# SurrealAI/surreal

Hardware: AMD Instinct MI355X
Metric: env-steps/sec (learner ingest) PPO 1024 actors×128 steps, 1/2/4/8 MI355X (higher is better)
Workload: dtype f32; 1 GPU; BASELINE configs[4]: PPO synthetic 1024 actors x 128 steps x 376-dim obs per GPU, one learn() per step, batch resident in HBM; mode=adapt, B_per_gpu=1024, n_step=128, obs_dim=376, action_dim=17, epochs=10 policy + 10 value, KL early exit disabled, hip_graph=True, parallelism=dp1, epoch_kernels=fused row-block, graph_segments=False

## Files before the change

include/surreal_amd.h:

```cpp
#ifndef SURREAL_AMD_H
#define SURREAL_AMD_H

#include <stddef.h>
#include <stdint.h>

#ifdef __cplusplus
extern "C" {
#endif

typedef void* smx_stream_t;

enum {
    SMX_OK = 0,
    SMX_E_NULL = -1,
    SMX_E_SHAPE = -2,
    SMX_E_UNSUPPORTED = -3,
    SMX_E_WORKSPACE = -4,
    SMX_E_ALIGN = -5
};

enum { SMX_ACT_NONE = 0, SMX_ACT_RELU = 1, SMX_ACT_TANH = 2 };
enum { SMX_PPO_CLIP = 0, SMX_PPO_ADAPT = 1 };

int smx_abi_version(void);
// ... 139 lines not shown
int smx_ppo_learn_epilogue_f32(const smx_learn_epilogue_t* args, smx_stream_t stream);
int smx_moments_f32(const float* x, int64_t n, float* moments, smx_stream_t stream);
int smx_moments_merge_f32(const float* parts, int32_t k, float* out, smx_stream_t stream);
int smx_adv_normalize_f32(float* x, int64_t n, const float* moments, float min_std,
                          smx_stream_t stream);

typedef struct {
    float lr_actor, lr_critic;
    float beta, eta;
    float clip_eps;
    float kl_target;
    float actor_max_norm, critic_max_norm;
    float actor_weight_decay, critic_weight_decay;
    int32_t adam_step_actor, adam_step_critic;
    int32_t stop_flag;
    int32_t epochs_done;
    int32_t reserved[2];
} smx_ppo_ctrl_t;

enum {
    SMX_PS_SURR = 0,
    SMX_PS_LOSS = 1,
    SMX_PS_ENTROPY = 2,
    SMX_PS_KL = 3,
    SMX_PS_GRADNORM = 4,
    SMX_PS_LB = 5,
    SMX_PS_ISW = 6,
    SMX_PS_REFBEH = 7,
    SMX_PS_STRIDE = 8
};
enum { SMX_VS_LOSS = 0, SMX_VS_EXPVAR = 1, SMX_VS_GRADNORM = 2, SMX_VS_STRIDE = 4 };

int32_t smx_ppo_loss_blocks(int64_t rows);
int32_t smx_ppo_loss_partial_stride(int32_t A);
int smx_ppo_policy_loss_f32(int32_t mode, const float* mean, const float* log_var,
                            const float* actions, int32_t ld_act, const float* behave,
                            int32_t ld_beh, const float* ref, int32_t ld_ref,
                            const float* adv, int64_t rows, int32_t A,
                            const smx_ppo_ctrl_t* ctrl, float* g_surr, float* g_kl,
                            float* row_partials, smx_stream_t stream);
int smx_ppo_partials_fold_f32(const float* row_partials, int32_t nblk, int32_t stride, float* out, int32_t nout,
                              const smx_ppo_ctrl_t* ctrl, smx_stream_t stream);
int smx_ppo_loss_finalize_f32(int32_t mode, const float* row_partials, int32_t nblk,
                              const float* g_surr, const float* g_kl, const float* log_var,
                              int64_t rows, int64_t n_total, int32_t A, smx_ppo_ctrl_t* ctrl,
                              int32_t check_stop, int32_t will_update, float* dz3,
                              float* dz3_t, int64_t ld_t, float* dlogvar, float* dlogvar_sumsq,
                              float* stats, smx_stream_t stream);

int32_t smx_value_loss_blocks(int64_t rows);
int smx_value_loss_f32(const float* values, const float* returns, int64_t rows,
                       int64_t n_total, float* dz3, float* partials, smx_ppo_ctrl_t* ctrl,
                       int32_t will_update, smx_stream_t stream);
typedef struct smx_ppo_losses {
    int32_t mode, A;
    const float* mean;
    const float* log_var;
    const float* actions;
    const float* behave;
    const float* ref;
    const float* adv;
    int32_t ld_act, ld_beh, ld_ref, check_stop;
    int64_t rows;
    float* g_surr;
    float* g_kl;
    float* row_partials;
    float* dz3;
    float* dz3_t;
    int64_t ld_t;
    float* dlogvar;
    float* dlogvar_sumsq;
    float* stats;
    const float* values;
    const float* returns;
    float* v_dz3;
    float* v_partials;
    int32_t will_update, v_will_update;
} smx_ppo_losses_t;
int smx_ppo_epoch_losses_f32(const smx_ppo_losses_t* args, smx_ppo_ctrl_t* ctrl,
                             smx_stream_t stream);
int smx_ppo_epoch_losses_dp_f32(const smx_ppo_losses_t* args, int64_t n_total, float* g_surr_t,
                                float* g_kl_t, smx_ppo_ctrl_t* ctrl, smx_stream_t stream);
typedef struct smx_ppo_combine {
    int32_t mode, A;
    const float* row_partials;
    int32_t nblk;
    int32_t check_stop;
    int64_t n_total;
    const float* log_var;
    float* stats;
    float* grads_a;
    const float* grads_kl;
    int64_t n_mlp, n_a;
    float* sumsq_a;
    const float* grads_c;
    int64_t n_c;
    float* sumsq_c;
    int32_t will_update, reserved;
} smx_ppo_combine_t;
int smx_ppo_epoch_combine_f32(const smx_ppo_combine_t* args, smx_ppo_ctrl_t* ctrl,
                              smx_stream_t stream);
int smx_mlp3_wgrad_multi_f32(const smx_mlp3_job_t* jobs, int32_t njobs, smx_stream_t stream);

enum { SMX_EPOCH_LOSS_NONE = 0, SMX_EPOCH_LOSS_POLICY = 1, SMX_EPOCH_LOSS_VALUE = 2, SMX_EPOCH_RHS_SURR = 3,
       SMX_EPOCH_RHS_KL = 4 };
typedef struct smx_epoch_job {
    const smx_mlp3_t* net;
    const float* x;
    int64_t rows;
    float* h1T;
    float* h2T;
    int64_t ldT;
    float* out;
    int32_t out_ld;
    int32_t out_act;
    int32_t loss;
    int32_t reserved;
    const int32_t* stop_flag;
    const float* dz3;
    float* dz3T;
    float* dz2T;
    float* dz1T;
    const float* packed;
} smx_epoch_job_t;
typedef struct smx_epoch_pack {
    const smx_mlp3_t* net;
    float* packed;
} smx_epoch_pack_t;
int64_t smx_epoch_packed_floats(int32_t D, int32_t H1, int32_t H2, int32_t OUT);
int smx_epoch_pack_f32(const smx_epoch_pack_t* items, int32_t n, smx_stream_t stream);
typedef struct smx_epoch_prep {
    const float* obs0; int64_t ld_obs0; int64_t rows; int32_t D; int32_t A;
    const float* zmean; const float* zstd;
    float* xn; float* xnT; int64_t ldT;
    const float* ref_sum; const float* ref_sumsq; const float* ref_count; float ref_eps; int32_t ref_filter;
    float* xr;
    const float* obs_next; int64_t ld_next; float* xnext;
    const float* ref_log_var; float* ref_std; int64_t ld_ref;
    int32_t* zero_words; int32_t n_zero; int32_t n_pack;
    smx_epoch_pack_t pack[4];
} smx_epoch_prep_t;
int smx_epoch_prepare_f32(const smx_epoch_prep_t* args, smx_stream_t stream);
struct smx_ppo_losses;
int32_t smx_epoch_blocks(int64_t rows);
int32_t smx_epoch_supported(int32_t D, int32_t H1, int32_t H2, int32_t OUT);
int smx_epoch_forward_f32(const smx_epoch_job_t* jobs, int32_t njobs, const struct smx_ppo_losses* loss,
                          smx_ppo_ctrl_t* ctrl, int64_t n_total, smx_stream_t stream);
int smx_epoch_backward_f32(const smx_epoch_job_t* jobs, int32_t njobs, const struct smx_ppo_losses* loss,
                           smx_ppo_ctrl_t* ctrl, int64_t n_total, smx_stream_t stream);
int32_t smx_epoch_fwdbwd_supported(int32_t D, int32_t H1, int32_t H2, int32_t OUT);
int smx_epoch_fwdbwd_f32(const smx_epoch_job_t* jobs, int32_t njobs, const struct smx_ppo_losses* loss,
                         smx_ppo_ctrl_t* ctrl, int64_t n_total, int32_t* sync_word, uint64_t* kl_slots,
                         smx_stream_t stream);
int smx_device_occupy(int32_t blocks, int64_t microseconds, smx_stream_t stream);

int smx_diaggauss_sample_f32(const float* mean, int64_t ld_mean, const float* log_var,
                             const float* noise_scale, const float* eps, int64_t ld_eps,
                             int64_t rows, int32_t A, float* actions, int64_t ld_act, float* pd,
                             int64_t ld_pd, smx_stream_t stream);
int smx_ppo_final_stats_f32(const float* log_var, int32_t A, const float* running_sum,
                            const float* running_sumsq, const float* count, int32_t D, float* out4,
                            smx_stream_t stream);
int smx_value_loss_finalize_f32(const float* partials, int32_t count, int32_t nblk,
                                float* stats, int32_t stats_stride, smx_stream_t stream);

int smx_clip_adam_step_f32(float* theta, const float* grads, float* exp_avg,
                           float* exp_avg_sq, int64_t n, const float* sumsq_partials,
                           int32_t npart, const smx_ppo_ctrl_t* ctrl, int32_t which,
                           int32_t honour_stop, float* grad_norm_out, smx_stream_t stream);
typedef struct smx_adam_group {
    float* theta;
    const float* grads;
    float* exp_avg;
    float* exp_avg_sq;
    int64_t n;
    const float* sumsq_partials;
    int32_t npart;
    int32_t honour_stop;
    float* grad_norm_out;
    const smx_mlp3_t* pack_net;
    float* packed;
} smx_adam_group_t;
int smx_clip_adam_step_group_f32(const smx_adam_group_t* group, int32_t which, const smx_ppo_ctrl_t* ctrl,
                                 smx_stream_t stream);
int smx_clip_adam_step_pair_f32(const smx_adam_group_t* actor, const smx_adam_group_t* critic,
                                const smx_ppo_ctrl_t* ctrl, smx_stream_t stream);
int32_t smx_sumsq_blocks(int64_t n);
int smx_sumsq_partials_f32(const float* x, int64_t n, float* partials, smx_stream_t stream);

int smx_ring_insert_f32(float* table, int64_t capacity, int32_t width, int64_t cursor,
                        const float* src, int64_t n, smx_stream_t stream);
int smx_gather_rows_f32(const float* table, int64_t capacity, int32_t width,
                        const int64_t* idx, int64_t n, float* dst, smx_stream_t stream);
int smx_uniform_indices(int64_t* idx, int64_t n, int64_t len, uint64_t seed,
                        uint64_t offset, smx_stream_t stream);
int smx_philox4x32_10(const uint32_t* ctr_key, int64_t n, uint32_t* out, smx_stream_t stream);
typedef struct {
    const void* table;
    void* dst;
    int64_t row_bytes;
} smx_gather_job_t;
int smx_uniform_gather_multi(const smx_gather_job_t* jobs, int32_t njobs, int64_t capacity, int64_t rows,
                             const int64_t* idx, int64_t len, uint64_t seed, uint64_t offset, int64_t* idx_out,
                             smx_stream_t stream);

int smx_ring_insert_bytes(void* table, int64_t capacity, int64_t row_bytes, int64_t cursor,
                          const void* src, int64_t n, smx_stream_t stream);
int smx_gather_rows_bytes(const void* table, int64_t capacity, int64_t row_bytes, const int64_t* idx,
                          int64_t n, void* dst, smx_stream_t stream);

int smx_window_emit_f32(const float* src, int32_t actors, int32_t T, int32_t width,
                        int32_t start, int32_t n_step, int32_t stride, int32_t W, float* dst,
                        smx_stream_t stream);
int smx_window_emit_bytes(const void* src, int32_t actors, int32_t T, int64_t row_bytes, int32_t start,
                          int32_t n_step, int32_t stride, int32_t W, void* dst, smx_stream_t stream);

int smx_frame_stack_u8(const void* frames, int32_t actors, int32_t R, int64_t frame_bytes, int32_t n_stack,
                       const int32_t* episode_first, int32_t start, int32_t n_step, int32_t stride, int32_t W,
                       void* dst, smx_stream_t stream);
int smx_synth_frame_u8(const float* s0, int64_t ld_s0, int32_t n, int32_t C, int32_t H, int32_t W, int32_t t,
                       void* dst, int64_t ld_dst, smx_stream_t stream);


struct smx_episode_monitor {
    double* ep_reward;
    int32_t* ep_steps;
    int64_t* ep_count;
    double* done_reward;
    int32_t* done_steps;
    int32_t capacity, reserved;
};

struct smx_noise_stream {
    uint64_t seed;
    int64_t actor_base;
    int64_t step;
    int32_t enabled, reserved;
};
int smx_noise_fill_f32(const struct smx_noise_stream* noise, int32_t steps, int32_t n, int32_t A, float* out,
                       smx_stream_t stream);

int smx_synth_env_step_f32(float* state, const float* init_state, const float* actions,
                           int32_t n, int32_t D, int32_t A, int32_t t, int32_t episode_len,
                           int32_t slot, int32_t T, float* obs_roll, float* act_roll,
                           float* rew_roll, float* done_roll, const struct smx_episode_monitor* mon,
                           smx_stream_t stream);

typedef struct smx_synth_act_step {
    float* state;
    const float* init_state;
    const float* mean;
    const float* log_var;
    const float* noise_scale;
    const float* eps;
    int64_t ld_mean, ld_eps;
    int32_t n, D, A, t, episode_len, slot, T, reserved;
    float* obs_roll;
    float* act_roll;
    float* rew_roll;
    float* done_roll;
    float* pd_roll;
    const float* zsum;
    const float* zsumsq;
    const float* zcount;
    float zeps, reserved_f;
    float* xn_out;
    struct smx_noise_stream noise;
    struct smx_episode_monitor mon;
} smx_synth_act_step_t;
int smx_synth_act_env_step_f32(const smx_synth_act_step_t* args, smx_stream_t stream);
int smx_synth_act_env_step_head_f32(const smx_synth_act_step_t* args, const float* W3, const float* b3,
                                    const float* h2, int64_t ld_h2, int32_t H2, int32_t out_act,
                                    smx_stream_t stream);


int smx_ddpg_critic_loss_f32(const float* q, const float* q_next_target, const float* rewards,
                             const float* dones, float gamma_n, int64_t rows, float* y,
                             float* dz3, smx_stream_t stream);
int smx_tanh_backward_f32(const float* da, const float* a, int64_t n, float* out,
                          smx_stream_t stream);
int smx_fill_f32(float* x, int64_t n, float value, smx_stream_t stream);
int smx_layernorm_forward_f32(const float* x, int64_t ldx, int64_t rows, int32_t F, const float* gamma, const float* beta,
                              float eps, float* y, int64_t ldy, float* mean, float* rstd, smx_stream_t stream);
int64_t smx_layernorm_backward_ws_floats(int64_t rows, int32_t F);
int smx_layernorm_backward_f32(const float* dy, int64_t lddy, const float* x, int64_t ldx, const float* mean,
                               const float* rstd, const float* gamma, int64_t rows, int32_t F, int32_t relu_mask, float* dx,
                               int64_t lddx, float* dgamma, float* dbeta, float* ws, int64_t ws_floats, smx_stream_t stream);
int smx_adam_step_f32(float* theta, const float* grads, float* exp_avg, float* exp_avg_sq,
                      int64_t n, double lr, int32_t step, double weight_decay,
                      double clip_value, smx_stream_t stream);
int smx_ddpg_critic_loss_step_f32(const float* q, const float* q_next_target, const float* rewards,
                                  const float* dones, float gamma_n, int64_t rows, float* y,
                                  float* dz3, int32_t* step_counter, smx_stream_t stream);
int smx_adam_step_dev_f32(float* theta, const float* grads, float* exp_avg, float* exp_avg_sq,
                          int64_t n, const float* lr, const int32_t* step, double weight_decay,
                          double clip_value, smx_stream_t stream);
int smx_hard_update_every_f32(float* target, const float* source, int64_t n, const int32_t* step,
                              int32_t interval, smx_stream_t stream);
int smx_soft_update_f32(float* target, const float* source, float tau, int64_t n,
                        smx_stream_t stream);
int smx_ddpg_stats_f32(const float* q, const float* y, const float* rewards,
                       const float* actions, int32_t ld_act, int32_t A, const float* q_actor,
                       int64_t rows, float* stats, smx_stream_t stream);

typedef struct smx_ddpg_net {
    const float *W1, *b1, *W2, *b2, *W3, *b3;
// ... 323 lines not shown
```

surreal_amd/_lib.py:

```python
import ctypes
import os
from ctypes import (POINTER, Structure, c_char_p, c_double, c_float, c_int32, c_int64, c_size_t,
                    c_uint64, c_void_p)

_HERE = os.path.dirname(os.path.abspath(__file__))
LIB_PATH = os.environ.get('SMX_LIB_PATH') or os.path.join(_HERE, 'libsurreal_amd.so')

SMX_ACT_NONE, SMX_ACT_RELU, SMX_ACT_TANH = 0, 1, 2
SMX_PPO_CLIP, SMX_PPO_ADAPT = 0, 1
SMX_E_UNSUPPORTED = -3
PS_SURR, PS_LOSS, PS_ENTROPY, PS_KL, PS_GRADNORM, PS_LB, PS_ISW, PS_REFBEH, PS_STRIDE = range(9)
VS_LOSS, VS_EXPVAR, VS_GRADNORM = 0, 1, 2
VS_STRIDE = 4


class Mlp3(Structure):
    _fields_ = [('W1', c_void_p), ('b1', c_void_p), ('W2', c_void_p), ('b2', c_void_p),
                ('W3', c_void_p), ('b3', c_void_p),
                ('D', c_int32), ('H1', c_int32), ('H2', c_int32), ('OUT', c_int32)]


class Mlp3Job(Structure):
    _fields_ = [('net', POINTER(Mlp3)), ('x', c_void_p), ('rows', c_int64), ('h1', c_void_p),
                ('h2', c_void_p), ('out', c_void_p), ('out_act', c_int32), ('out_ld', c_int32),
# ... 104 lines not shown
                [(n, c_void_p) for n in ('c_a1', 'cm1', 'cr1', 'c_a2', 'cm2', 'cr2', 'dn2', 'dz1c', 'a1', 'am1', 'ar1', 'a2',
                                         'am2', 'ar2', 'dn2a', 'dn1a')] + [('second', POINTER(DdpgRowsLnSecond))])


class DdpgRows(Structure):
    _fields_ = ([('rows', c_int64)] + [(n, c_int32) for n in ('D', 'A', 'H1', 'H2', 'c1', 'c2')] +
                [(n, DdpgNet) for n in ('actor', 'critic', 'target_actor', 'target_critic')] +
                [(n, c_void_p) for n in ('packed', 'x', 'x_next', 'actions', 'rewards', 'dones')] +
                [('gamma_n', c_float)] +
                [(n, c_void_p) for n in ('xcat', 'h2c', 'q', 'q_next', 'y', 'dz3', 'dz2', 'dxcat', 'h1a', 'h2a', 'act',
                                         'q_actor', 'dz3a', 'dz2a', 'dz1a', 'step')] +
                [('second', POINTER(DdpgRowsSecond)), ('ln', POINTER(DdpgRowsLn))])


class GatherJob(Structure):
    _fields_ = [('table', c_void_p), ('dst', c_void_p), ('row_bytes', c_int64)]


class EpisodeMonitor(Structure):
    _fields_ = [('ep_reward', c_void_p), ('ep_steps', c_void_p), ('ep_count', c_void_p), ('done_reward', c_void_p),
                ('done_steps', c_void_p), ('capacity', c_int32), ('reserved', c_int32)]


class NoiseStream(Structure):
    _fields_ = [('seed', c_uint64), ('actor_base', c_int64), ('step', c_int64), ('enabled', c_int32),
                ('reserved', c_int32)]


class SynthRollout(Structure):
    _fields_ = [('net', POINTER(Mlp3)), ('packed', c_void_p), ('out_act', c_int32), ('n', c_int32),
                ('log_var', c_void_p), ('noise_scale', c_void_p), ('eps', c_void_p), ('zsum', c_void_p),
                ('zsumsq', c_void_p), ('zcount', c_void_p), ('zeps', c_float), ('t', c_int32),
                ('episode_len', c_int32), ('steps', c_int32), ('rows_per_actor', c_int32), ('slot', c_int32),
                ('state', c_void_p), ('init_state', c_void_p), ('obs_roll', c_void_p), ('act_roll', c_void_p),
                ('rew_roll', c_void_p), ('done_roll', c_void_p), ('pd_roll', c_void_p), ('obs_last', c_void_p),
                ('actors_per_workgroup', c_int32), ('noise', NoiseStream), ('mon', EpisodeMonitor)]


class SynthLstmRollout(Structure):
    _fields_ = [('roll', SynthRollout), ('lstm', POINTER(Lstm)), ('lstm_packed', c_void_p), ('hidden', c_int32),
                ('reserved', c_int32), ('h0', c_void_p), ('c0', c_void_p), ('hN', c_void_p), ('cN', c_void_p),
                ('h_before', c_void_p), ('c_before', c_void_p), ('cell_roll', c_void_p)]


class SynthPpoWindowRollout(Structure):
    _fields_ = [('base', SynthLstmRollout), ('n_step', c_int32), ('advance', c_int32), ('carry_obs', c_void_p),
                ('carry_act', c_void_p), ('carry_rew', c_void_p), ('carry_pd', c_void_p), ('carry_cells', c_void_p),
                ('obs', c_void_p), ('obs_next', c_void_p), ('actions', c_void_p), ('rewards', c_void_p),
                ('dones', c_void_p), ('pds', c_void_p), ('cells', c_void_p), ('cursor', c_int64),
                ('capacity', c_int64)]


class DdpgRollout(Structure):
    _fields_ = [('net', POINTER(Mlp3)), ('packed', c_void_p), ('n', c_int32), ('D', c_int32), ('A', c_int32),
                ('steps', c_int32), ('t', c_int32), ('episode_len', c_int32), ('n_step', c_int32),
                ('noise_type', c_int32), ('actors_per_workgroup', c_int32), ('reserved', c_int32),
                ('eps', c_void_p), ('sigmas', c_void_p), ('theta', c_double), ('dt', c_double), ('root_dt', c_double),
                ('gpow', c_void_p), ('ou', c_void_p), ('state', c_void_p), ('init_state', c_void_p),
                ('carry_obs', c_void_p), ('carry_act', c_void_p), ('carry_rew', c_void_p), ('obs', c_void_p),
                ('obs_next', c_void_p), ('actions', c_void_p), ('rewards', c_void_p), ('dones', c_void_p),
                ('cursor', c_int64), ('capacity', c_int64), ('noise', NoiseStream), ('mon', EpisodeMonitor)]


class DdpgActorVariant(Structure):
    _fields_ = [('ln', c_void_p), ('ln_eps', c_float), ('reserved', c_int32), ('packed_pop', c_void_p),
                ('packed_stride', c_int64), ('actors_per_agent', c_int32), ('agents', c_int32),
                ('measure_step', c_int32), ('reserved2', c_int32), ('dist', c_void_p)]


class ParamNoise(Structure):
    _fields_ = [('net', POINTER(Mlp3)), ('seed', c_uint64), ('agent_base', c_int64), ('generation', c_int64),
                ('agents', c_int32), ('adaptive', c_int32), ('acts', c_int64), ('alpha', c_double), ('target', c_double),
                ('sigma', c_void_p), ('dist', c_void_p), ('packed_pop', c_void_p), ('packed_stride', c_int64),
                ('ln', c_void_p)]


class DdpgPixelStep(Structure):
    _fields_ = [('base', DdpgRollout), ('C', c_int32), ('H', c_int32), ('W', c_int32), ('frame_stacks', c_int32),
                ('hist_len', c_int32), ('hist_pos', c_int32), ('hist', c_void_p), ('pixel', c_void_p),
                ('pixel_next', c_void_p), ('obs_pixel', c_void_p)]


class SynthPpoPixelWindowStep(Structure):
    _fields_ = ([(n, c_int32) for n in ('n', 'D', 'A', 'hidden', 't', 'episode_len', 'n_step', 'advance')] +
                [(n, c_void_p) for n in ('log_var', 'noise_scale', 'eps', 'state', 'init_state', 'h_before', 'c_before',
                                         'carry_obs', 'carry_act', 'carry_rew', 'carry_pd', 'carry_cells', 'obs',
                                         'obs_next', 'actions', 'rewards', 'dones', 'pds', 'cells')] +
                [('cursor', c_int64), ('capacity', c_int64)] +
                [(n, c_int32) for n in ('C', 'H', 'W', 'frame_stacks', 'hist_len', 'hist_pos', 'copy_workgroups',
                                        'reserved')] +
                [(n, c_void_p) for n in ('hist', 'pixel', 'pixel_next', 'obs_pixel')] + [('noise', NoiseStream),
                                                                                   ('mon', EpisodeMonitor)])


SMX_DDPG_NOISE_NONE, SMX_DDPG_NOISE_GAUSSIAN, SMX_DDPG_NOISE_OU = 0, 1, 2
SMX_PPO_PIXEL_STEP_MAX_A = 64


class Xchg(Structure):
    _fields_ = [('world', c_int32), ('rank', c_int32), ('capacity', c_int64), ('peer', c_void_p * 8)]


class SynthActStep(Structure):
    _fields_ = [('state', c_void_p), ('init_state', c_void_p), ('mean', c_void_p), ('log_var', c_void_p),
                ('noise_scale', c_void_p), ('eps', c_void_p), ('ld_mean', c_int64), ('ld_eps', c_int64),
                ('n', c_int32), ('D', c_int32), ('A', c_int32), ('t', c_int32), ('episode_len', c_int32),
                ('slot', c_int32), ('T', c_int32), ('reserved', c_int32),
                ('obs_roll', c_void_p), ('act_roll', c_void_p), ('rew_roll', c_void_p),
                ('done_roll', c_void_p), ('pd_roll', c_void_p), ('zsum', c_void_p), ('zsumsq', c_void_p),
                ('zcount', c_void_p), ('zeps', c_float), ('reserved_f', c_float), ('xn_out', c_void_p),
                ('noise', NoiseStream), ('mon', EpisodeMonitor)]


CTRL_WORDS = 16
(C_LR_ACTOR, C_LR_CRITIC, C_BETA, C_ETA, C_CLIP_EPS, C_KL_TARGET, C_ACTOR_MAX_NORM,
 C_CRITIC_MAX_NORM, C_ACTOR_WD, C_CRITIC_WD, C_STEP_ACTOR, C_STEP_CRITIC, C_STOP,
 C_EPOCHS_DONE) = range(14)
C_XCHG_ERR = 14
C_SYNC_ERR = 15

_P = c_void_p
_SIGS = {
    'smx_abi_version': (c_int32, []),
    'smx_error_string': (c_char_p, [c_int32]),
    'smx_zfilter_stats_f32': (c_int32, [_P, _P, _P, c_int32, c_float, _P, _P, _P]),
    'smx_zfilter_forward_f32': (c_int32, [_P, c_int64, c_int64, c_int32, _P, _P, _P, _P]),
    'smx_zfilter_forward_sums_f32': (c_int32, [_P, c_int64, c_int64, c_int32, _P, _P, _P, c_float, _P, _P]),
    'smx_diaggauss_sample_f32': (c_int32, [_P, c_int64, _P, _P, _P, c_int64, c_int64, c_int32, _P,
                                           c_int64, _P, c_int64, _P]),
    'smx_zfilter_update_f32': (c_int32, [_P, c_int64, c_int64, c_int32, _P, _P, _P, c_float, _P]),
    'smx_mlp3_packed_bytes': (c_size_t, [c_int32, c_int32, c_int32, c_int32]),
    'smx_mlp3_pack_f32': (c_int32, [POINTER(Mlp3), _P, c_size_t, _P]),
    'smx_mlp3_pack_zstats_f32': (c_int32, [POINTER(Mlp3), _P, c_size_t, _P, _P, _P, c_int32, c_float, _P, _P, _P]),
    'smx_mlp3_fused_exact_zfilter': (c_int32, [c_int32]),
    'smx_mlp3_forward_fused_f32': (c_int32, [_P, c_int32, c_int32, c_int32, c_int32, _P, _P,
                                             c_int64, c_int32, c_int32, _P, _P, _P, c_int32, _P]),
    'smx_linear_f32': (c_int32, [_P, c_int32, c_int32, _P, c_int32, c_int32, _P, _P, c_int32,
                                 c_int32, c_int32, c_int32, c_int32, _P, _P, _P]),
    'smx_linear_wgrad_f32': (c_int32, [_P, c_int32, _P, c_int32, _P, c_int32, _P, c_int32, c_int32,
                                       c_int32, _P]),
    'smx_mlp3_forward_f32': (c_int32, [POINTER(Mlp3), _P, c_int64, _P, _P, _P, c_int32, _P, _P]),
    'smx_mlp3_forward_multi_f32': (c_int32, [POINTER(Mlp3Job), c_int32, _P]),
    'smx_mlp3_backward_multi_f32': (c_int32, [POINTER(Mlp3Job), c_int32, _P]),
    'smx_mlp3_wgrad_multi_f32': (c_int32, [POINTER(Mlp3Job), c_int32, _P]),
    'smx_epoch_blocks': (c_int32, [c_int64]),
    'smx_epoch_supported': (c_int32, [c_int32, c_int32, c_int32, c_int32]),
    'smx_epoch_packed_floats': (c_int64, [c_int32, c_int32, c_int32, c_int32]),
    'smx_epoch_pack_f32': (c_int32, [POINTER(EpochPack), c_int32, _P]),
    'smx_epoch_prepare_f32': (c_int32, [POINTER(EpochPrep), _P]),
    'smx_epoch_forward_f32': (c_int32, [POINTER(EpochJob), c_int32, POINTER(PpoLosses), _P, c_int64, _P]),
    'smx_epoch_backward_f32': (c_int32, [POINTER(EpochJob), c_int32, POINTER(PpoLosses), _P, c_int64, _P]),
    'smx_epoch_fwdbwd_supported': (c_int32, [c_int32, c_int32, c_int32, c_int32]),
    'smx_epoch_fwdbwd_f32': (c_int32, [POINTER(EpochJob), c_int32, POINTER(PpoLosses), _P, c_int64, _P, _P, _P]),
    'smx_device_occupy': (c_int32, [c_int32, c_int64, _P]),
    'smx_layernorm_forward_f32': (c_int32, [_P, c_int64, c_int64, c_int32, _P, _P, c_float, _P, c_int64, _P, _P, _P]),
    'smx_layernorm_backward_ws_floats': (c_int64, [c_int64, c_int32]),
    'smx_layernorm_backward_f32': (c_int32, [_P, c_int64, _P, c_int64, _P, _P, _P, c_int64, c_int32, c_int32, _P, c_int64, _P, _P,
                                             _P, c_int64, _P]),
    'smx_zfilter_update_ws_floats': (c_int64, [c_int64, c_int32]),
    'smx_zfilter_update_ws_f32': (c_int32, [_P, c_int64, c_int64, c_int32, _P, _P, _P, c_float, _P, c_int64, _P]),
    'smx_ppo_partials_fold_f32': (c_int32, [_P, c_int32, c_int32, _P, c_int32, _P, _P]),
    'smx_mlp3_forward_rows_supported': (c_int32, [c_int32, c_int32, c_int32, c_int32]),
    'smx_mlp3_forward_rows_f32': (c_int32, [POINTER(Mlp3), _P, c_int64, _P, _P, _P, c_int32, c_int32, _P, c_size_t, _P, _P]),
    'smx_mlp3_backward_partials': (c_int32, [c_int32, c_int32, c_int32, c_int32]),
    'smx_mlp3_backward_f32': (c_int32, [POINTER(Mlp3), _P, _P, _P, _P, c_int64, _P, _P, _P, _P,
                                        _P, _P]),
    'smx_mlp3_backward_ws_floats': (c_int64, [c_int32, c_int32, c_int32, c_int32, c_int64]),
    'smx_mlp3_backward_splitk_f32': (c_int32, [POINTER(Mlp3), _P, _P, _P, _P, c_int64, _P, _P, _P, _P, c_int64, _P, _P]),
    'smx_mlp3_dgrad_rows_supported': (c_int32, [c_int32, c_int32, c_int32, c_int32]),
    'smx_mlp3_dgrad_rows_ws_floats': (c_int64, [c_int32, c_int32, c_int32, c_int32]),
    'smx_mlp3_backward_rows_f32': (c_int32, [POINTER(Mlp3), _P, _P, _P, _P, c_int64, _P, _P, _P, _P, _P, c_int64, _P, c_int64,
                                             _P, _P]),
    'smx_windowed_gae_returns_f32': (c_int32, [_P, _P, _P, _P, _P, _P, c_float, c_float, c_int32,
                                               c_int32, c_int32, _P, _P, _P]),
    'smx_windowed_gae_norm_f32': (c_int32, [_P, _P, _P, _P, _P, _P, c_float, c_float, c_int32, c_int32, c_int32, _P, _P, _P,
                                            c_float, _P, _P]),
    'smx_ppo_learn_epilogue_f32': (c_int32, [POINTER(LearnEpilogue), _P]),
    'smx_reward_filter_f32': (c_int32, [_P, c_int64, c_float, c_int32, _P, c_float, c_int32, _P, _P, _P, _P, _P]),
    'smx_reward_filter_partials': (c_int32, []),
    'smx_moments_f32': (c_int32, [_P, c_int64, _P, _P]),
    'smx_moments_merge_f32': (c_int32, [_P, c_int32, _P, _P]),
    'smx_adv_normalize_f32': (c_int32, [_P, c_int64, _P, c_float, _P]),
    'smx_ppo_loss_blocks': (c_int32, [c_int64]),
    'smx_ppo_loss_partial_stride': (c_int32, [c_int32]),
    'smx_ppo_policy_loss_f32': (c_int32, [c_int32, _P, _P, _P, c_int32, _P, c_int32, _P, c_int32,
                                          _P, c_int64, c_int32, _P, _P, _P, _P, _P]),
    'smx_ppo_loss_finalize_f32': (c_int32, [c_int32, _P, c_int32, _P, _P, _P, c_int64, c_int64,
                                            c_int32, _P, c_int32, c_int32, _P, _P, c_int64, _P, _P,
                                            _P, _P]),
    'smx_ppo_epoch_losses_f32': (c_int32, [POINTER(PpoLosses), _P, _P]),
    'smx_ppo_epoch_losses_dp_f32': (c_int32, [POINTER(PpoLosses), c_int64, _P, _P, _P, _P]),
    'smx_ppo_epoch_combine_f32': (c_int32, [POINTER(PpoCombine), _P, _P]),
    'smx_ppo_final_stats_f32': (c_int32, [_P, c_int32, _P, _P, _P, c_int32, _P, _P]),
    'smx_value_loss_blocks': (c_int32, [c_int64]),
    'smx_value_loss_f32': (c_int32, [_P, _P, c_int64, c_int64, _P, _P, _P, c_int32, _P]),
    'smx_value_loss_finalize_f32': (c_int32, [_P, c_int32, c_int32, _P, c_int32, _P]),
    'smx_clip_adam_step_f32': (c_int32, [_P, _P, _P, _P, c_int64, _P, c_int32, _P, c_int32,
                                         c_int32, _P, _P]),
    'smx_clip_adam_step_group_f32': (c_int32, [POINTER(AdamGroup), c_int32, _P, _P]),
    'smx_clip_adam_step_pair_f32': (c_int32, [POINTER(AdamGroup), POINTER(AdamGroup), _P, _P]),
    'smx_sumsq_blocks': (c_int32, [c_int64]),
    'smx_sumsq_partials_f32': (c_int32, [_P, c_int64, _P, _P]),
    'smx_synth_act_env_step_head_f32': (c_int32, [POINTER(SynthActStep), _P, _P, _P, c_int64, c_int32, c_int32, _P]),
    'smx_conv_u8_forward_f32': (c_int32, [_P, c_int64, c_int32, c_int32, c_int32, c_int32, c_int32, _P, _P, c_int32,
                                          _P, _P, _P]),
    'smx_conv_u8_wgrad_ws_floats': (c_int64, [c_int32, c_int32]),
    'smx_conv_u8_wgrad_f32': (c_int32, [_P, c_int64, c_int32, c_int32, c_int32, c_int32, c_int32, _P, c_int32, _P, _P, _P,
                                        c_int64, _P, _P]),
    'smx_conv_cl_forward_f32': (c_int32, [_P, c_int64, c_int32, c_int32, c_int32, c_int32, c_int32, _P, _P, c_int32,
                                          _P, _P, _P]),
    'smx_conv_cl_wgrad_ws_floats': (c_int64, [c_int32, c_int32]),
    'smx_conv_cl_wgrad_f32': (c_int32, [_P, c_int64, c_int32, c_int32, c_int32, c_int32, c_int32, _P, c_int32, _P, _P, _P,
                                        c_int64, _P, _P]),
    'smx_conv_cl_dgrad_f32': (c_int32, [_P, c_int64, c_int32, c_int32, c_int32, c_int32, c_int32, _P, c_int32, _P, _P,
                                        _P, _P]),
    'smx_ring_insert_bytes': (c_int32, [_P, c_int64, c_int64, c_int64, _P, c_int64, _P]),
    'smx_gather_rows_bytes': (c_int32, [_P, c_int64, c_int64, _P, c_int64, _P, _P]),
    'smx_window_emit_bytes': (c_int32, [_P, c_int32, c_int32, c_int64, c_int32, c_int32, c_int32, c_int32, _P, _P]),
    'smx_ring_insert_f32': (c_int32, [_P, c_int64, c_int32, c_int64, _P, c_int64, _P]),
    'smx_gather_rows_f32': (c_int32, [_P, c_int64, c_int32, _P, c_int64, _P, _P]),
    'smx_philox4x32_10': (c_int32, [_P, c_int64, _P, _P]),
    'smx_noise_fill_f32': (c_int32, [POINTER(NoiseStream), c_int32, c_int32, c_int32, _P, _P]),
    'smx_uniform_indices': (c_int32, [_P, c_int64, c_int64, c_uint64, c_uint64, _P]),
    'smx_uniform_gather_multi': (c_int32, [POINTER(GatherJob), c_int32, c_int64, c_int64, _P, c_int64, c_uint64, c_uint64,
                                           _P, _P]),
    'smx_window_emit_f32': (c_int32, [_P, c_int32, c_int32, c_int32, c_int32, c_int32, c_int32,
                                      c_int32, _P, _P]),
    'smx_synth_act_env_step_f32': (c_int32, [POINTER(SynthActStep), _P]),
    'smx_synth_env_step_f32': (c_int32, [_P, _P, _P, c_int32, c_int32, c_int32, c_int32, c_int32,
                                         c_int32, c_int32, _P, _P, _P, _P, POINTER(EpisodeMonitor), _P]),
    'smx_ddpg_critic_loss_f32': (c_int32, [_P, _P, _P, _P, c_float, c_int64, _P, _P, _P]),
    'smx_tanh_backward_f32': (c_int32, [_P, _P, c_int64, _P, _P]),
    'smx_fill_f32': (c_int32, [_P, c_int64, c_float, _P]),
    'smx_adam_step_f32': (c_int32, [_P, _P, _P, _P, c_int64, c_double, c_int32, c_double, c_double,
                                    _P]),
    'smx_soft_update_f32': (c_int32, [_P, _P, c_float, c_int64, _P]),
    'smx_ddpg_critic_loss_step_f32': (c_int32, [_P, _P, _P, _P, c_float, c_int64, _P, _P, _P, _P]),
    'smx_adam_step_dev_f32': (c_int32, [_P, _P, _P, _P, c_int64, _P, _P, c_double, c_double, _P]),
    'smx_hard_update_every_f32': (c_int32, [_P, _P, c_int64, _P, c_int32, _P]),
    'smx_ddpg_rows_supported': (c_int32, [c_int32] * 6),
    'smx_ddpg_rows_supported_at': (c_int32, [c_int32] * 6 + [c_int64]),
    'smx_ddpg_rows_packed_floats': (c_int64, [c_int32] * 6),
    'smx_ddpg_rows_pack_f32': (c_int32, [_P, c_int32, _P]),
    'smx_ddpg_rows_critic_f32': (c_int32, [_P, _P]),
    'smx_ddpg_rows_actor_f32': (c_int32, [_P, _P]),
    'smx_ddpg_rows_second_supported': (c_int32, [c_int32] * 6 + [c_int64]),
    'smx_ddpg_rows_second_packed_floats': (c_int64, [c_int32] * 6),
    'smx_ddpg_rows_critic_td3_f32': (c_int32, [_P, _P]),
    'smx_ddpg_rows_ln_supported': (c_int32, [c_int32] * 6 + [c_int64]),
    'smx_ddpg_rows_ln_second_supported': (c_int32, [c_int32] * 6 + [c_int64]),
    'smx_ddpg_rows_update_f32': (c_int32, [_P, c_int32, _P, _P]),
    'smx_ddpg_rows_wgrad_update_f32': (c_int32, [_P, c_int32, _P, _P]),
    'smx_ddpg_stats_f32': (c_int32, [_P, _P, _P, _P, c_int32, c_int32, _P, c_int64, _P, _P]),
    'smx_lstm_param_count': (c_int64, [c_int32, c_int32]),
    'smx_lstm_forward_f32': (c_int32, [POINTER(Lstm), _P, c_int64, c_int32, _P, _P, _P, _P, _P, _P,
                                       _P, _P, _P, _P]),
    'smx_lstm_backward_f32': (c_int32, [POINTER(Lstm), _P, c_int64, c_int32, _P, _P, _P, _P, _P, _P,
                                        _P, _P, _P, c_int64, _P]),
    'smx_lstm_backward_ws_floats': (c_int64, [c_int32, c_int32, c_int64, c_int32]),
    'smx_linear_wgrad_ws_floats': (c_int64, [c_int32, c_int32, c_int32]),
    'smx_linear_wgrad_splitk_f32': (c_int32, [_P, c_int32, _P, c_int32, _P, c_int32, _P, c_int32,
                                              c_int32, c_int32, _P, c_int64, _P]),
    'smx_linear_wgrad_splitk_pair_f32': (c_int32, [_P, c_int32, c_int32, c_int32, _P, c_int32, _P, _P, c_int32, _P,
                                                    c_int32, _P, _P, c_int32, _P, c_int64, _P]),
    'smx_im2col_f32': (c_int32, [_P, c_int32, c_int32, c_int64, c_int32, c_int32, c_int32, c_int32,
                                 c_int32, c_int32, c_float, _P, _P]),
    'smx_col2im_f32': (c_int32, [_P, c_int64, c_int32, c_int32, c_int32, c_int32, c_int32, c_int32,
                                 _P, _P, _P]),
    'smx_flatten_order_f32': (c_int32, [_P, c_int32, c_int32, c_int32, c_int32, _P, _P]),
    'smx_linear_multi_f32': (c_int32, [POINTER(LinearJob), c_int32, _P]),
    'smx_frame_stack_u8': (c_int32, [_P, c_int32, c_int32, c_int64, c_int32, _P, c_int32, c_int32, c_int32, c_int32, _P, _P]),
    'smx_synth_frame_u8': (c_int32, [_P, c_int64, c_int32, c_int32, c_int32, c_int32, c_int32, _P, c_int64, _P]),
    'smx_synth_rollout_supported': (c_int32, [c_int32, c_int32, c_int32, c_int32]),
    'smx_synth_rollout_f32': (c_int32, [POINTER(SynthRollout), _P]),
    'smx_synth_lstm_rollout_supported': (c_int32, [c_int32] * 5),
    'smx_lstm_rollout_packed_floats': (c_int64, [c_int32, c_int32]),
    'smx_lstm_rollout_pack_f32': (c_int32, [POINTER(Lstm), _P, _P]),
    'smx_synth_lstm_rollout_f32': (c_int32, [POINTER(SynthLstmRollout), _P]),
    'smx_synth_ppo_window_rollout_supported': (c_int32, [c_int32] * 5),
    'smx_synth_ppo_window_rollout_f32': (c_int32, [POINTER(SynthPpoWindowRollout), _P]),
    'smx_synth_ddpg_rollout_supported': (c_int32, [c_int32, c_int32, c_int32, c_int32, c_int32]),
    'smx_synth_ddpg_rollout_f32': (c_int32, [POINTER(DdpgRollout), POINTER(DdpgActorVariant), _P]),
    'smx_synth_ddpg_population_block': (c_int32, [c_int32, c_int32, c_int32]),
    'smx_synth_ddpg_step_f32': (c_int32, [POINTER(DdpgRollout), _P, c_int64, _P]),
    'smx_synth_ddpg_pixel_step': (c_int32, [POINTER(DdpgPixelStep), _P, c_int64, _P]),
    'smx_param_noise_copy_floats': (c_int64, [c_int32, c_int32, c_int32, c_int32, c_int32]),
    'smx_param_noise_fill_f32': (c_int32, [POINTER(ParamNoise), c_int32, _P, _P]),
    'smx_param_noise_refresh_f32': (c_int32, [POINTER(ParamNoise), _P]),
    'smx_synth_ppo_pixel_window_step': (c_int32, [POINTER(SynthPpoPixelWindowStep), _P, c_int64, _P]),
    'smx_xchg_bytes': (c_int64, [c_int64, c_int32]),
    'smx_xchg_alloc': (c_int32, [c_int64, c_double, POINTER(c_void_p), POINTER(c_int32), _P]),
    'smx_xchg_free': (c_int32, [_P]),
    'smx_xchg_export': (c_int32, [_P, _P]),
    'smx_xchg_open': (c_int32, [_P, POINTER(c_void_p)]),
    'smx_xchg_close': (c_int32, [_P]),
    'smx_xchg_allreduce_f32': (c_int32, [POINTER(Xchg), _P, _P, c_int64, _P, _P]),
    'smx_xchg_allgather_f32': (c_int32, [POINTER(Xchg), _P, c_int64, _P, _P, _P]),
    'smx_xchg_status': (c_int32, [POINTER(Xchg), _P, _P]),
}

EXPORTED_SYMBOLS = tuple(sorted(_SIGS))


class SmxError(RuntimeError):
    pass

# ... 58 lines not shown
```

surreal_amd/csrc/smx_epoch.hip:

```cpp
#include "smx_common.h"
#include <string.h>

#define SMX_LDS_BARRIER() asm volatile("s_waitcnt lgkmcnt(0)\n\ts_barrier" ::: "memory")

namespace {
#include "smx_ppo_loss.inc.h"
#include "smx_epoch_pack.inc.h"
#include "smx_epoch_mma.inc.h"

constexpr int TB = 3;
constexpr int MAX_EJOBS = 4;
constexpr int XV = 7;
constexpr int LIN = 6;
constexpr int LINF = 3;
constexpr int EXCLUSIVE_LDS = 84 * 1024;
constexpr int LDZ = 68;
constexpr int LDO = 36;
static_assert(ER == LOSS_ROWS_PER_BLOCK, "a row block is a loss block");
static_assert(NTH == 256, "the shared loss code strides by 256 threads");

#ifdef SMX_EPOCH_TIMING
#define TSTAMP(i) do { if (G.tbuf && threadIdx.x == 0) G.tbuf[(size_t)ts_blk * 32 + (i)] = (long long)__builtin_readcyclecounter(); } while (0)
#else
#define TSTAMP(i) do { } while (0)
#endif
struct EJob {
    const float *W1, *b1, *W2, *b2, *W3, *b3;
    int D, H1, H2, OUT;
    const float* x;
    int rows;
    float *h1T, *h2T;
    long ldT;
    float* out;
    int out_ld, out_act, loss, blk_base;
    const int* stop;
    const float* dz3;
    float *dz3T, *dz2T, *dz1T;
    const float *P1, *P2, *P3, *P2T, *P3T;
};

struct PolArgs {
    int mode, A;
    const float *log_var, *actions, *behave, *ref, *adv;
    int ld_act, ld_beh, ld_ref, check_stop, will_update;
    float *g_surr, *g_kl, *row_partials;
    float *dlogvar, *dlogvar_sumsq, *stats;
};

struct ValArgs {
    const float* returns;
    float *v_dz3, *v_partials;
    int will_update;
};

struct EArgs {
    EJob j[MAX_EJOBS];
    int n;
    PolArgs pl;
    ValArgs vl;
    long n_total;
    int ldx, ldh1, ldh2, off_h1, off_h2, off_out, off_red, off_loss;
    int off_g;
    int* sync;
    int nb_pol;
    const int* pol_stop;
    unsigned long long* kl_slots;
    int fsplit;
    int xsplit;
    long long* tbuf;
};

__device__ __forceinline__ int xcd_job_order(const EArgs& G, int raw) {
    const int nb = G.xsplit;
    if (nb == 0) return raw;
    const int xcd = raw & 7, slot = raw >> 3;
    return (xcd >> 2) * nb + slot * 4 + (xcd & 3);
}

__device__ __forceinline__ EJob select_job(const EArgs& G, int bid) {
    int pi = 0;
#pragma unroll
    for (int k = 1; k < MAX_EJOBS; ++k) pi += (k < G.n && bid >= G.j[k].blk_base) ? 1 : 0;
    EJob J = G.j[pi];
    asm volatile("" :: "s"(J.W1), "s"(J.b1), "s"(J.W2), "s"(J.b2), "s"(J.W3), "s"(J.b3), "s"(J.D), "s"(J.H1),
                 "s"(J.H2), "s"(J.OUT), "s"(J.x), "s"(J.rows), "s"(J.h1T), "s"(J.h2T), "s"(J.ldT), "s"(J.out),
                 "s"(J.out_ld), "s"(J.out_act), "s"(J.loss), "s"(J.blk_base), "s"(J.stop), "s"(J.dz3),
                 "s"(J.dz3T), "s"(J.dz2T), "s"(J.dz1T));
    return J;
}

constexpr int FNWV = 8;
constexpr int FNTH = 64 * FNWV;
constexpr int FTG = 3;

__device__ __forceinline__ void fb_reduce_partials(const float* __restrict__ partials, int nblk, int stride, float* S,
                                                   float* buf) {
    const int tid = threadIdx.x;
    float t0 = 0.f, t1 = 0.f, t2 = 0.f, t3 = 0.f;
    for (int b0 = 0; b0 < nblk; b0 += FIN_CH) {
        const int nb = min(FIN_CH, nblk - b0);
        const int cnt = nb * stride;
        const float* src = partials + (size_t)b0 * stride;
        for (int i0 = tid; i0 < cnt; i0 += 8 * FNTH) {
            float v[8];
#pragma unroll
            for (int u = 0; u < 8; ++u)
                v[u] = __hip_atomic_load(src + min(i0 + FNTH * u, cnt - 1), __ATOMIC_RELAXED, __HIP_MEMORY_SCOPE_AGENT);
#pragma unroll
            for (int u = 0; u < 8; ++u)
                if (i0 + FNTH * u < cnt) buf[i0 + FNTH * u] = v[u];
        }
        SMX_LDS_BARRIER();
        if (tid < stride) {
            int b = 0;
            for (; b + 4 <= nb; b += 4) {
                t0 += buf[b * stride + tid];
                t1 += buf[(b + 1) * stride + tid];
                t2 += buf[(b + 2) * stride + tid];
                t3 += buf[(b + 3) * stride + tid];
            }
            for (; b < nb; ++b) t0 += buf[b * stride + tid];
        }
        SMX_LDS_BARRIER();
    }
    if (tid < stride) S[tid] = (t0 + t1) + (t2 + t3);
    SMX_LDS_BARRIER();
}

template <bool FB>
__device__ __forceinline__ void epoch_fwd_body(const EArgs& G, smx_ppo_ctrl_t* __restrict__ ctrl) {
    extern __shared__ float sm[];
    const int bid = xcd_job_order(G, (int)blockIdx.x);
    const int ts_blk = bid;
    (void)ts_blk;
    TSTAMP(0);
    const EJob J = select_job(G, bid);
    const int stopv = J.stop ? __builtin_nontemporal_load(J.stop) : 0;
    const int blk = bid - J.blk_base;
    const long row0 = (long)blk * ER;
    int nrows = J.rows - (int)row0;
    if (nrows > ER) nrows = ER;
    const int tid = threadIdx.x, lane = tid & 63;
    const int wv = __builtin_amdgcn_readfirstlane(tid >> 6);
    const int fm = lane & 15, kq = lane >> 4;
    TSTAMP(12);

    float* xs = sm;
    float* h1s = sm + G.off_h1;
    float* h2s = sm + G.off_h2;
    float* outs = sm + G.off_out;
    const int ldx = G.ldx, ldh1 = G.ldh1, ldh2 = G.ldh2;

    const rsrc_t rx = make_rsrc(J.x, (unsigned)J.rows * (unsigned)J.D * 4u);
    const bool lo = tid < NTH;
    const int xr = (tid & (NTH - 1)) >> 4, xj = tid & 15;
    const unsigned xrow = (unsigned)(row0 + xr) * (unsigned)J.D * 4u;
    const bool xvec = (J.D & 3) == 0;
    float4 xv[XV];
    if (xvec) {
#pragma unroll
        for (int i = 0; i < XV; ++i) {
            const int k = 4 * (xj + 16 * i);
            xv[i] = ld16(rx, (lo && k < J.D && xr < nrows) ? xrow + 4u * k : OOB);
        }
    }
    const PolArgs& pa = G.pl;
    const int LW = 5 * pa.A + 1;
    float lin[LINF];
    float vret = 0.f;
    unsigned lin_ok = 0u;
    auto loss_word = [&](int n, int c, bool& ok) -> float {
        const int A = pa.A;
        ok = n < nrows;
        n = ok ? n : 0;
        const long gr = row0 + n;
        const float* q = c < A ? pa.actions + gr * pa.ld_act + c
                       : c < 3 * A ? pa.behave + gr * pa.ld_beh + (c - A)
                       : c < 5 * A ? pa.ref + gr * pa.ld_ref + (c - 3 * A) : pa.adv + gr;
        return *q;
    };
    if (J.loss == SMX_EPOCH_LOSS_POLICY) {
        const int lq = FNTH / LW, lr = FNTH - lq * LW;
        int n = tid / LW, c = tid - n * LW;
#pragma unroll
        for (int i = 0; i < LINF; ++i) {
            const bool in = tid + FNTH * i < ER * LW;
            bool ok;
            lin[i] = loss_word(in ? n : 0, in ? c : 0, ok);
            lin_ok |= (ok && in) ? (1u << i) : 0u;
            n += lq;
            c += lr;
            if (c >= LW) { c -= LW; ++n; }
        }
    } else if (lo && J.loss == SMX_EPOCH_LOSS_VALUE && tid < nrows) {
        vret = G.vl.returns[row0 + tid];
    }
    TSTAMP(13);
    for (int idx = tid; idx < (G.off_red - G.off_h1) >> 2; idx += FNTH)
        *(float4*)(h1s + 4 * idx) = make_float4(0.f, 0.f, 0.f, 0.f);
    TSTAMP(14);
    if (xvec && lo) {
#pragma unroll
        for (int i = 0; i < XV; ++i) {
            const int k = 4 * (xj + 16 * i);
            if (k < ldx) *(float4*)(xs + xr * ldx + k) = xv[i];
        }
        for (int k = 4 * (xj + 16 * XV); k < ldx; k += 64) {
            const float4 v = ld16(rx, (k < J.D && xr < nrows) ? xrow + 4u * k : OOB);
            *(float4*)(xs + xr * ldx + k) = v;
        }
    } else if (!xvec) {
        for (int idx = tid; idx < ER * ldx; idx += FNTH) {
            const int n = idx / ldx, j = idx - n * ldx;
            xs[idx] = (j < J.D && n < nrows) ? J.x[(size_t)(row0 + n) * J.D + j] : 0.f;
        }
    }
    TSTAMP(15);
    float* lin_s = sm + G.off_loss + loss_scratch_floats(pa.A);
    if (J.loss == SMX_EPOCH_LOSS_POLICY) {
#pragma unroll
        for (int i = 0; i < LINF; ++i) {
            const int idx = tid + FNTH * i;
            if (idx < ER * LW) lin_s[idx] = ((lin_ok >> i) & 1u) ? lin[i] : 0.f;
        }
        for (int idx = tid + FNTH * LINF; idx < ER * LW; idx += FNTH) {
            const int n = idx / LW;
            bool ok;
            const float v = loss_word(n, idx - n * LW, ok);
            lin_s[idx] = ok ? v : 0.f;
        }
    }
    if (__builtin_amdgcn_readfirstlane(stopv) != 0) return;
    TSTAMP(1);
    SMX_LDS_BARRIER();
    TSTAMP(2);

#pragma unroll 1
    for (int l = 0; l < 3; ++l) {
        const float* Wp = l == 0 ? J.P1 : (l == 1 ? J.P2 : J.P3);
        const float* bias = l == 0 ? J.b1 : (l == 1 ? J.b2 : J.b3);
        const int H = l == 0 ? J.H1 : (l == 1 ? J.H2 : J.OUT);
        const int K = l == 0 ? J.D : (l == 1 ? J.H1 : J.H2);
        const float* in_lds = l == 0 ? xs : (l == 1 ? h1s : h2s);
        const int ldi = l == 0 ? ldx : (l == 1 ? ldh1 : ldh2);
        float* out_lds = l == 0 ? h1s : (l == 1 ? h2s : outs);
        const int ldo = l == 0 ? ldh1 : (l == 1 ? ldh2 : LDO);
        float* hT = l == 0 ? J.h1T : (l == 1 ? J.h2T : nullptr);
        const int tiles = (H + 15) >> 4;
        const int C2 = (((K + 31) >> 5) + 1) & ~1;
        const rsrc_t rw = make_rsrc(Wp, (unsigned)tiles * (unsigned)C2 * 2048u);
        const rsrc_t rbias = make_rsrc(bias, (unsigned)H * 4u);
        float* stp = l == 2 ? J.out : hT;
        const bool st_ok = stp != nullptr;
        const rsrc_t rst = make_rsrc(stp ? stp : Wp, l == 2 ? (unsigned)J.rows * (unsigned)J.out_ld * 4u
                                                             : (unsigned)H * (unsigned)J.ldT * 4u);
#pragma unroll 1
        for (int tb = 0; tb < tiles; tb += FNWV * FTG) {
            const int t0 = tb + wv;
            int nt = (tiles - t0 + FNWV - 1) / FNWV;
            nt = nt < 0 ? 0 : (nt > FTG ? FTG : nt);
            float bs[FTG][4];
#pragma unroll
            for (int g = 0; g < FTG; ++g) {
                const int f0 = 16 * (t0 + FNWV * g) + 4 * kq;
#pragma unroll
                for (int r = 0; r < 4; ++r) bs[g][r] = ld4(rbias, (g < nt) ? (unsigned)(f0 + r) * 4u : OOB);
            }
            f32x4 acc[TG];
#pragma unroll
            for (int g = 0; g < TG; ++g) acc[g] = (f32x4){0.f, 0.f, 0.f, 0.f};
            TSTAMP(16 + 4 * l);
            if (nt > 2) fwd_tiles<3>(acc, rw, tiles, C2, in_lds, ldi, t0, FNWV, lane);
            else if (nt > 1) fwd_tiles<2>(acc, rw, tiles, C2, in_lds, ldi, t0, FNWV, lane);
            else if (nt > 0) fwd_tiles<1>(acc, rw, tiles, C2, in_lds, ldi, t0, FNWV, lane);
            TSTAMP(17 + 4 * l);
            const unsigned sstep = l == 2 ? 4u : (unsigned)J.ldT * 4u;
            const unsigned srow = l == 2 ? (unsigned)(row0 + fm) * (unsigned)J.out_ld * 4u
                                         : (unsigned)(row0 + fm) * 4u;
#pragma unroll
            for (int g = 0; g < FTG; ++g) {
                if (g < nt) {
                    const int f0 = 16 * (t0 + FNWV * g) + 4 * kq;
                    float v[4];
#pragma unroll
                    for (int r = 0; r < 4; ++r) {
                        float z = acc[g][r] + bs[g][r];
                        if (g == 0 && l == 2) z = act_f(z, J.out_act);
                        else z = (z < 0.f) ? 0.f : z;
                        v[r] = (f0 + r < H) ? z : 0.f;
                    }
                    *(float4*)(out_lds + fm * ldo + f0) = make_float4(v[0], v[1], v[2], v[3]);
#pragma unroll
                    for (int r = 0; r < 4; ++r) {
                        const bool ok = st_ok && fm < nrows && f0 + r < H;
                        __builtin_amdgcn_raw_buffer_store_b32(__float_as_uint(v[r]), rst,
                                                              ok ? srow + (unsigned)(f0 + r) * sstep : OOB, 0, 0);
                    }
                }
            }
        }
        TSTAMP(18 + 4 * l);
        SMX_LDS_BARRIER();
        TSTAMP(3 + l);
    }

    if constexpr (!FB) {
    if (!lo) return;
    if (J.loss == SMX_EPOCH_LOSS_POLICY) {
        const PolArgs& p = G.pl;
        policy_loss_body(blk, sm + G.off_loss, p.mode, outs, LDO, p.log_var, lin_s, LW, lin_s + p.A, LW,
                         lin_s + 3 * p.A, LW, lin_s + 5 * p.A, (long)J.rows, p.A, ctrl, p.g_surr, p.g_kl,
                         p.row_partials, 1.0f, false, nullptr, nullptr, 0, row0, LW);
    } else if (J.loss == SMX_EPOCH_LOSS_VALUE && tid < 64) {
        const ValArgs& q = G.vl;
        const bool ok = tid < nrows;
        const float v = ok ? outs[tid * LDO] : 0.f, g = ok ? vret : 0.f;
        const float d = g - v, e = v - g;
        if (ok) q.v_dz3[row0 + tid] = (2.0f * e) / (float)G.n_total;
        const float cnt = (float)nrows;
        const float md = smx_wave_sum(ok ? d : 0.f) / cnt;
        const float mg = smx_wave_sum(ok ? g : 0.f) / cnt;
        const float m2d = smx_wave_sum(ok ? (d - md) * (d - md) : 0.f);
        const float m2g = smx_wave_sum(ok ? (g - mg) * (g - mg) : 0.f);
        const float sq = smx_wave_sum(ok ? e * e : 0.f);
        if (tid == 0) {
            float* P = q.v_partials + (size_t)blk * 8;
            P[0] = cnt; P[1] = md; P[2] = m2d; P[3] = mg; P[4] = m2g; P[5] = sq; P[6] = 0.f; P[7] = 0.f;
            if (blk == 0 && q.will_update) ctrl->adam_step_critic += 1;
        }
    }
    TSTAMP(6);
    } else {
    __shared__ __attribute__((aligned(16))) float S[8 + 2 * MAX_A + 8];
    float& s_kl = S[8 + 2 * MAX_A];
    int& wait_ok = *(int*)&S[8 + 2 * MAX_A + 1];
    static_assert(sizeof(S) % 16 == 0, "static LDS is a multiple of 16 bytes");
    const PolArgs& p = G.pl;
    const bool policy = J.loss == SMX_EPOCH_LOSS_POLICY;
    const bool adapt = policy && p.mode == SMX_PPO_ADAPT;
    const int A = p.A;
    const int pstride = 8 + 2 * A;
    float* gss = sm + G.off_g;
    float* gks = gss + ER * LDZ;
    float* dz2s = gks + ER * LDZ;
    const float nf = (float)G.n_total;
    const float inv_n = 1.0f / nf;
    const int pol_stopped = (G.pol_stop && blockIdx.x == gridDim.x - 1) ? __builtin_nontemporal_load(G.pol_stop) : 0;
    const int tiles2 = (J.H2 + 15) >> 4;
    float4 wa[FTG], wb[FTG];
    {
        const rsrc_t rw3 = make_rsrc(J.P3T, (unsigned)tiles2 * (unsigned)pack_chunks(J.OUT) * 2048u);
#pragma unroll
        for (int g = 0; g < FTG; ++g) {
            const int t = wv + FNWV * g;
            const unsigned o = t < tiles2 ? ((unsigned)t * (unsigned)pack_chunks(J.OUT) * 512u + (unsigned)lane * 4u) * 4u : OOB;
            wa[g] = ld16(rw3, o);
            wb[g] = ld16(rw3, t < tiles2 ? o + 1024u : OOB);
        }
    }
    if (policy) {
        if (lo) {
            policy_loss_body<true>(blk, sm + G.off_loss, p.mode, outs, LDO, p.log_var, lin_s, LW, lin_s + p.A, LW,
                                   lin_s + 3 * p.A, LW, lin_s + 5 * p.A, (long)J.rows, p.A, ctrl, nullptr, nullptr,
                                   p.row_partials, 1.0f, false, nullptr, nullptr, 0, row0, LW, G.kl_slots);
        } else {
#pragma unroll
            for (int i = 0; i < POLICY_LOSS_BARRIERS; ++i) SMX_LDS_BARRIER();
        }
    } else if (tid < 64) {
        const ValArgs& q = G.vl;
        const bool ok = tid < nrows;
        const float v = ok ? outs[tid * LDO] : 0.f, g = ok ? vret : 0.f;
        const float d = g - v, e = v - g;
        const float dz = (2.0f * e) / nf;
        if (ok) q.v_dz3[row0 + tid] = dz;
        if (tid < ER) gss[tid * LDZ] = ok ? dz : 0.f;
        const float cnt = (float)nrows;
        const float md = smx_wave_sum(ok ? d : 0.f) / cnt;
        const float mg = smx_wave_sum(ok ? g : 0.f) / cnt;
        const float m2d = smx_wave_sum(ok ? (d - md) * (d - md) : 0.f);
        const float m2g = smx_wave_sum(ok ? (g - mg) * (g - mg) : 0.f);
        const float sq = smx_wave_sum(ok ? e * e : 0.f);
        if (tid == 0) {
            float* P = q.v_partials + (size_t)blk * 8;
            P[0] = cnt; P[1] = md; P[2] = m2d; P[3] = mg; P[4] = m2g; P[5] = sq; P[6] = 0.f; P[7] = 0.f;
            if (blk == 0 && q.will_update) ctrl->adam_step_critic += 1;
        }
    }
    SMX_LDS_BARRIER();
    TSTAMP(6);
    if (policy) {
        const float* sc = sm + G.off_loss;
        const float* e_dmu = loss_elem_dmu(sc, A);
        const float* e_dkl = loss_elem_dkl(sc, A);
        const float* r_dll = loss_row_dll(sc, A);
        for (int idx = tid; idx < ER * 32; idx += FNTH) {
            const int n = idx >> 5, a = idx & 31;
            const bool ok = n < nrows && a < A;
            const int i = ok ? n * A + a : 0;
            const float gs = r_dll[ok ? n : 0] * e_dmu[i];
            gss[n * LDZ + a] = ok ? gs * inv_n : 0.f;
            if (adapt) gks[n * LDZ + a] = ok ? e_dkl[i] * inv_n : 0.f;
        }
    }
    SMX_LDS_BARRIER();
    f32x4 aS[FTG], aK[FTG];
#pragma unroll
    for (int g = 0; g < FTG; ++g) { aS[g] = (f32x4){0.f, 0.f, 0.f, 0.f}; aK[g] = (f32x4){0.f, 0.f, 0.f, 0.f}; }
    {
        const float* bs = gss + (lane & 15) * LDZ + 8 * (lane >> 4);
        const float4 s0 = *(const float4*)bs, s1 = *(const float4*)(bs + 4);
        float4 k0 = make_float4(0.f, 0.f, 0.f, 0.f), k1 = k0;
        if (adapt) {
            const float* bk = gks + (lane & 15) * LDZ + 8 * (lane >> 4);
            k0 = *(const float4*)bk; k1 = *(const float4*)(bk + 4);
        }
#pragma unroll
        for (int g = 0; g < FTG; ++g) {
            if (wv + FNWV * g < tiles2) {
                aS[g] = MFMA16(wa[g].x, s0.x, aS[g]); aS[g] = MFMA16(wa[g].y, s0.y, aS[g]);
                aS[g] = MFMA16(wa[g].z, s0.z, aS[g]); aS[g] = MFMA16(wa[g].w, s0.w, aS[g]);
                aS[g] = MFMA16(wb[g].x, s1.x, aS[g]); aS[g] = MFMA16(wb[g].y, s1.y, aS[g]);
                aS[g] = MFMA16(wb[g].z, s1.z, aS[g]); aS[g] = MFMA16(wb[g].w, s1.w, aS[g]);
                if (adapt) {
                    aK[g] = MFMA16(wa[g].x, k0.x, aK[g]); aK[g] = MFMA16(wa[g].y, k0.y, aK[g]);
                    aK[g] = MFMA16(wa[g].z, k0.z, aK[g]); aK[g] = MFMA16(wa[g].w, k0.w, aK[g]);
                    aK[g] = MFMA16(wb[g].x, k1.x, aK[g]); aK[g] = MFMA16(wb[g].y, k1.y, aK[g]);
                    aK[g] = MFMA16(wb[g].z, k1.z, aK[g]); aK[g] = MFMA16(wb[g].w, k1.w, aK[g]);
                }
            }
        }
    }
    TSTAMP(7);
    const int nbp = G.nb_pol;
    auto wait_count = [&]() {
        if (tid == 0) {
            const long long t0 = (long long)wall_clock64();
            int okw = 1;
            while (__hip_atomic_load(G.sync, __ATOMIC_RELAXED, __HIP_MEMORY_SCOPE_AGENT) < nbp) {
                if ((long long)wall_clock64() - t0 > 25000000LL) { okw = 0; break; }
                __builtin_amdgcn_s_sleep(1);
            }
            wait_ok = wait_ok & okw;
            if (!okw) atomicOr(&ctrl->reserved[1], 1);
        }
        __syncthreads();
    };
    auto kl_total = [&]() -> float {
        if (tid < 64) {
            float t = 0.f;
            int okw = 1;
            const long long t0 = (long long)wall_clock64();
            for (int b = tid; b < nbp; b += 64) {
                unsigned long long w;
                while (((w = __hip_atomic_load(G.kl_slots + b, __ATOMIC_RELAXED, __HIP_MEMORY_SCOPE_AGENT)) >> 32) == 0ull) {
                    if ((long long)wall_clock64() - t0 > 25000000LL) { okw = 0; break; }
                    __builtin_amdgcn_s_sleep(1);
                }
                t += __uint_as_float((unsigned)w);
            }
            t = smx_wave_sum(t);
            okw = __all(okw);
            if (tid == 0) {
                s_kl = t;
                wait_ok = wait_ok & okw;
                if (!okw) atomicOr(&ctrl->reserved[1], 1);
            }
        }
        SMX_LDS_BARRIER();
        return s_kl;
    };
    auto kl_coef = [&](float klsum, float& ck, bool& stop) {
        float S3[3] = {0.f, 0.f, klsum}, ls;
        loss_and_kl_coef(p.mode, S3, nf, ctrl, ls, ck);
        stop = (p.check_stop && (double)(klsum / nf) > 4.0 * (double)ctrl->kl_target) || wait_ok == 0;
    };
    float c_kl = 0.f;
    bool stop_now = false;
    if (tid == 0) wait_ok = 1;
    if (adapt) kl_coef(kl_total(), c_kl, stop_now);
    if (policy && tid < 128) asm volatile("s_waitcnt vmcnt(0)" ::: "memory");
    SMX_LDS_BARRIER();
    if (policy && tid == 0) __hip_atomic_fetch_add(G.sync, 1, __ATOMIC_RELAXED, __HIP_MEMORY_SCOPE_AGENT);
    TSTAMP(8);
    if (!stop_now) {
        {
            const rsrc_t rout = make_rsrc(J.dz2T, (unsigned)J.H2 * (unsigned)J.ldT * 4u);
#pragma unroll
            for (int g = 0; g < FTG; ++g) {
                const int t = wv + FNWV * g;
                if (t < tiles2) {
                    const int f0 = 16 * t + 4 * kq;
                    const float4 m = *(const float4*)(h2s + fm * ldh2 + f0);
                    float4 v;
                    v.x = (m.x > 0.f) ? aS[g][0] + c_kl * aK[g][0] : 0.f;
                    v.y = (m.y > 0.f) ? aS[g][1] + c_kl * aK[g][1] : 0.f;
                    v.z = (m.z > 0.f) ? aS[g][2] + c_kl * aK[g][2] : 0.f;
                    v.w = (m.w > 0.f) ? aS[g][3] + c_kl * aK[g][3] : 0.f;
                    *(float4*)(dz2s + fm * ldh2 + f0) = v;
                    const bool ok = fm < nrows;
                    const unsigned o = ((unsigned)f0 * (unsigned)J.ldT + (unsigned)(row0 + fm)) * 4u, st = (unsigned)J.ldT * 4u;
                    __builtin_amdgcn_raw_buffer_store_b32(__float_as_uint(v.x), rout, ok && f0 < J.H2 ? o : OOB, 0, 0);
                    __builtin_amdgcn_raw_buffer_store_b32(__float_as_uint(v.y), rout, ok && f0 + 1 < J.H2 ? o + st : OOB, 0, 0);
                    __builtin_amdgcn_raw_buffer_store_b32(__float_as_uint(v.z), rout, ok && f0 + 2 < J.H2 ? o + 2 * st : OOB, 0, 0);
                    __builtin_amdgcn_raw_buffer_store_b32(__float_as_uint(v.w), rout, ok && f0 + 3 < J.H2 ? o + 3 * st : OOB, 0, 0);
                }
            }
        }
        if (policy) {
            for (int idx = tid; idx < ER * A; idx += FNTH) {
                const int a = idx / ER, n = idx - a * ER;
                const float v = gss[n * LDZ + a] + c_kl * gks[n * LDZ + a];
                if (n < nrows) J.dz3T[(size_t)a * J.ldT + row0 + n] = v;
            }
        }
        SMX_LDS_BARRIER();
        TSTAMP(9);
        {
            const int tiles1 = (J.H1 + 15) >> 4;
            const int C2h = pack_chunks(J.H2);
            const rsrc_t rw2 = make_rsrc(J.P2T, (unsigned)tiles1 * (unsigned)C2h * 2048u);
            const rsrc_t rout = make_rsrc(J.dz1T, (unsigned)J.H1 * (unsigned)J.ldT * 4u);
#pragma unroll 1
            for (int tb = 0; tb < tiles1; tb += FNWV * FTG) {
                const int t0 = tb + wv;
                int nt = (tiles1 - t0 + FNWV - 1) / FNWV;
                nt = nt < 0 ? 0 : (nt > FTG ? FTG : nt);
                f32x4 acc[TG];
#pragma unroll
                for (int g = 0; g < TG; ++g) acc[g] = (f32x4){0.f, 0.f, 0.f, 0.f};
                if (nt > 2) fwd_tiles<3>(acc, rw2, tiles1, C2h, dz2s, ldh2, t0, FNWV, lane);
                else fwd_tiles<2>(acc, rw2, tiles1, C2h, dz2s, ldh2, t0, FNWV, lane);
#pragma unroll
                for (int g = 0; g < FTG; ++g) {
                    if (g < nt) {
                        const int f0 = 16 * (t0 + FNWV * g) + 4 * kq;
                        const float4 m = *(const float4*)(h1s + fm * ldh1 + f0);
                        const float vx = (m.x > 0.f) ? acc[g][0] : 0.f, vy = (m.y > 0.f) ? acc[g][1] : 0.f;
                        const float vz = (m.z > 0.f) ? acc[g][2] : 0.f, vw = (m.w > 0.f) ? acc[g][3] : 0.f;
                        const bool ok = fm < nrows;
                        const unsigned o = ((unsigned)f0 * (unsigned)J.ldT + (unsigned)(row0 + fm)) * 4u, st = (unsigned)J.ldT * 4u;
                        __builtin_amdgcn_raw_buffer_store_b32(__float_as_uint(vx), rout, ok && f0 < J.H1 ? o : OOB, 0, 0);
                        __builtin_amdgcn_raw_buffer_store_b32(__float_as_uint(vy), rout, ok && f0 + 1 < J.H1 ? o + st : OOB, 0, 0);
                        __builtin_amdgcn_raw_buffer_store_b32(__float_as_uint(vz), rout, ok && f0 + 2 < J.H1 ? o + 2 * st : OOB, 0, 0);
                        __builtin_amdgcn_raw_buffer_store_b32(__float_as_uint(vw), rout, ok && f0 + 3 < J.H1 ? o + 3 * st : OOB, 0, 0);
                    }
                }
            }
        }
    }
    TSTAMP(10);
    if (nbp > 0 && blockIdx.x == gridDim.x - 1 && pol_stopped == 0) {
        wait_count();
        fb_reduce_partials(p.row_partials, nbp, pstride, S, sm + G.off_loss);
        const float klsum = kl_total();
        float loss = 0.f, ck = 0.f;
        if (tid == 0) S[2] = klsum;
        SMX_LDS_BARRIER();
        loss_and_kl_coef(p.mode, S, nf, ctrl, loss, ck);
        for (int a = tid; a < A; a += FNTH) p.dlogvar[a] = (S[8 + a] + ck * S[8 + A + a]) * inv_n;
        if (tid == 0 && wait_ok)
            write_policy_scalars(S, nf, loss, ck, p.log_var, A, ctrl, p.check_stop, p.will_update, p.dlogvar_sumsq,
                                 p.stats);
    }
    TSTAMP(11);
    }
}

__global__ __launch_bounds__(FNTH) void epoch_fwd_kernel(EArgs G, smx_ppo_ctrl_t* __restrict__ ctrl) {
    epoch_fwd_body<false>(G, ctrl);
}

__global__ __launch_bounds__(FNTH) void epoch_fb_kernel(EArgs G, smx_ppo_ctrl_t* __restrict__ ctrl) {
    epoch_fwd_body<true>(G, ctrl);
}

__global__ __launch_bounds__(NTH) void epoch_bwd_kernel(EArgs G, smx_ppo_ctrl_t* __restrict__ ctrl) {
    extern __shared__ float sm[];
    __shared__ float S[8 + 2 * MAX_A];
    const int ts_blk = blockIdx.x;
    (void)ts_blk;
    TSTAMP(0);
    const EJob J = select_job(G, (int)blockIdx.x);
    const int fs = G.fsplit;
    const int wg = blockIdx.x - J.blk_base;
    const int nb = (J.rows + ER - 1) / ER;
    int blk, half;
    if ((nb & 7) == 0 && (J.blk_base & 7) == 0) {
        const int s = wg >> 3;
        half = s % fs;
        blk = (s / fs) * 8 + (wg & 7);
    } else {
        blk = wg / fs;
        half = wg - blk * fs;
    }
    const long row0 = (long)blk * ER;
    int nrows = J.rows - (int)row0;
    if (nrows > ER) nrows = ER;
    const int tid = threadIdx.x, lane = tid & 63;
    const int wv = __builtin_amdgcn_readfirstlane(tid >> 6);
    const int fm = lane & 15, kq = lane >> 4;
    float* dz3s = sm;
    float* dz2s = sm + G.off_h2;
    const int ldh2 = G.ldh2;
    const bool policy = J.loss == SMX_EPOCH_LOSS_POLICY;
    const bool dp_surr = J.loss == SMX_EPOCH_RHS_SURR, dp_kl = J.loss == SMX_EPOCH_RHS_KL;
    const bool actor = policy || dp_surr || dp_kl;
    const PolArgs& p = G.pl;

    const int A = p.A;
    float gs0 = 0.f, gk0 = 0.f, gs1 = 0.f, gk1 = 0.f, vd = 0.f;
    if (actor) {
        const int last = ER * A - 1;
        const int i0 = tid < last ? tid : last, i1 = tid + NTH < last ? tid + NTH : last;
        const int a0 = i0 / ER, n0 = i0 - a0 * ER, a1 = i1 / ER, n1 = i1 - a1 * ER;
        const size_t e0 = (size_t)(row0 + (n0 < nrows ? n0 : 0)) * A + a0;
        const size_t e1 = (size_t)(row0 + (n1 < nrows ? n1 : 0)) * A + a1;
        gs0 = p.g_surr[e0]; gk0 = p.g_kl[e0];
        gs1 = p.g_surr[e1]; gk1 = p.g_kl[e1];
    } else {
        vd = J.dz3[row0 + (tid < nrows ? tid : 0)];
    }
    for (int idx = tid; idx < (G.off_red >> 2); idx += NTH) *(float4*)(sm + 4 * idx) = make_float4(0.f, 0.f, 0.f, 0.f);
    if (tid == 0) S[0] = (actor && ctrl->stop_flag) ? 1.f : 0.f;
    SMX_LDS_BARRIER();
    const bool stopped = S[0] != 0.f;
    SMX_LDS_BARRIER();
    if (stopped) return;
    TSTAMP(1);

    if (policy) {
        const int nblk = nb;
        reduce_row_partials(p.row_partials, nblk, 8 + 2 * A, S, sm + G.off_loss);
        const float n = (float)G.n_total;
        float c_kl, loss;
        loss_and_kl_coef(p.mode, S, n, ctrl, loss, c_kl);
        const float inv_n = 1.0f / n;
        const bool stop_now = p.check_stop && (double)(S[2] / n) > 4.0 * (double)ctrl->kl_target;
        if (wg == 0) {
            for (int a = tid; a < A; a += NTH) p.dlogvar[a] = (S[8 + a] + c_kl * S[8 + A + a]) * inv_n;
            if (tid == 0)
                write_policy_scalars(S, n, loss, c_kl, p.log_var, A, ctrl, p.check_stop, p.will_update,
                                     p.dlogvar_sumsq, p.stats);
        }
        TSTAMP(2);
        if (stop_now || !p.will_update) return;
#pragma unroll
        for (int i = 0; i < 2; ++i) {
            const int idx = tid + NTH * i;
            if (idx < ER * A) {
                const int a = idx / ER, nn = idx - a * ER;
                const float v = nn < nrows ? ((i ? gs1 : gs0) + c_kl * (i ? gk1 : gk0)) * inv_n : 0.f;
                if (nn < nrows && half == 0 && J.dz3T) J.dz3T[(size_t)a * J.ldT + row0 + nn] = v;
                dz3s[nn * LDZ + a] = v;
            }
        }
    } else if (actor) {
        const float inv_n = 1.0f / (float)G.n_total;
#pragma unroll
        for (int i = 0; i < 2; ++i) {
            const int idx = tid + NTH * i;
            if (idx < ER * A) {
                const int a = idx / ER, nn = idx - a * ER;
                const float v = nn < nrows ? (dp_surr ? (i ? gs1 : gs0) : (i ? gk1 : gk0)) * inv_n : 0.f;
                if (nn < nrows && half == 0 && J.dz3T) J.dz3T[(size_t)a * J.ldT + row0 + nn] = v;
                dz3s[nn * LDZ + a] = v;
            }
        }
    } else {
        if (tid < ER) dz3s[tid * LDZ] = tid < nrows ? vd : 0.f;
    }
    SMX_LDS_BARRIER();
    TSTAMP(3);
#pragma unroll 1
    for (int l = 0; l < 2; ++l) {
        const float* Wp = l == 0 ? J.P3T : J.P2T;
        const int M = l == 0 ? J.H2 : J.H1, K = l == 0 ? J.OUT : J.H2;
        const float* in_lds = l == 0 ? dz3s : dz2s;
        const int ldi = l == 0 ? LDZ : ldh2;
        const float* hT = l == 0 ? J.h2T : J.h1T;
        float* out_lds = l == 0 ? dz2s : nullptr;
        float* outT = l == 0 ? (half == 0 ? J.dz2T : nullptr) : J.dz1T;
        const int first = l == 0 ? 0 : half, step = l == 0 ? 1 : fs;
        const int tiles = (M + 15) >> 4;
        const int C2 = (((K + 31) >> 5) + 1) & ~1;
        const rsrc_t rw = make_rsrc(Wp, (unsigned)tiles * (unsigned)C2 * 2048u);
        const rsrc_t rmask = make_rsrc(hT, (unsigned)M * (unsigned)J.ldT * 4u);
        const rsrc_t rout = make_rsrc(outT ? outT : hT, (unsigned)M * (unsigned)J.ldT * 4u);
#pragma unroll 1
        for (int tb = first; tb < tiles; tb += step * NWV * TB) {
            const int t0 = tb + step * wv, ts = step * NWV;
            int nt = (tiles - t0 + ts - 1) / ts;
            nt = nt < 0 ? 0 : (nt > TB ? TB : nt);
            float mk[TB][4];
#pragma unroll
            for (int g = 0; g < TB; ++g) {
                const int f0 = 16 * (t0 + ts * g) + 4 * kq;
                const bool ok = g < nt && f0 < M && fm < nrows;
#pragma unroll
                for (int r = 0; r < 4; ++r)
                    mk[g][r] = ld4(rmask, ok ? ((unsigned)(f0 + r) * (unsigned)J.ldT + (unsigned)(row0 + fm)) * 4u : OOB);
            }
            f32x4 acc[TG];
#pragma unroll
            for (int g = 0; g < TG; ++g) acc[g] = (f32x4){0.f, 0.f, 0.f, 0.f};
            TSTAMP(8 + 4 * l);
            if (nt > 1) fwd_tiles<TB>(acc, rw, tiles, C2, in_lds, ldi, t0, ts, lane);
            else if (nt > 0) fwd_tiles<1>(acc, rw, tiles, C2, in_lds, ldi, t0, ts, lane);
            TSTAMP(9 + 4 * l);
#pragma unroll
            for (int g = 0; g < TB; ++g) {
                if (g < nt) {
                    const int f0 = 16 * (t0 + ts * g) + 4 * kq;
                    float4 v;
                    v.x = (mk[g][0] > 0.f) ? acc[g][0] : 0.f;
                    v.y = (mk[g][1] > 0.f) ? acc[g][1] : 0.f;
                    v.z = (mk[g][2] > 0.f) ? acc[g][2] : 0.f;
                    v.w = (mk[g][3] > 0.f) ? acc[g][3] : 0.f;
                    if (out_lds) *(float4*)(out_lds + fm * ldh2 + f0) = v;
                    const bool ok = outT != nullptr && f0 < M && fm < nrows;
                    const unsigned o = ((unsigned)f0 * (unsigned)J.ldT + (unsigned)(row0 + fm)) * 4u, st = (unsigned)J.ldT * 4u;
                    __builtin_amdgcn_raw_buffer_store_b32(__float_as_uint(v.x), rout, ok ? o : OOB, 0, 0);
                    __builtin_amdgcn_raw_buffer_store_b32(__float_as_uint(v.y), rout, ok ? o + st : OOB, 0, 0);
                    __builtin_amdgcn_raw_buffer_store_b32(__float_as_uint(v.z), rout, ok ? o + 2 * st : OOB, 0, 0);
                    __builtin_amdgcn_raw_buffer_store_b32(__float_as_uint(v.w), rout, ok ? o + 3 * st : OOB, 0, 0);
                }
            }
// ... 145 lines not shown
    SMX_REQUIRE((a->zmean == nullptr) == (a->zstd == nullptr), SMX_E_NULL);
    SMX_REQUIRE(!a->xnT || a->ldT >= a->rows, SMX_E_SHAPE);
    SMX_REQUIRE(!a->ref_filter || (a->ref_sum && a->ref_sumsq && a->ref_count), SMX_E_NULL);
    SMX_REQUIRE(!a->xnext || (a->obs_next && a->ld_next >= a->D), SMX_E_SHAPE);
    SMX_REQUIRE(!a->ref_std || (a->ref_log_var && a->A > 0 && a->ld_ref >= a->A), SMX_E_SHAPE);
    SMX_REQUIRE(a->n_zero >= 0 && a->n_zero <= (1 << 20) && (a->n_zero == 0 || a->zero_words), SMX_E_SHAPE);
    PrepArgs P;
    memset(&P, 0, sizeof(P));
    P.obs0 = a->obs0; P.ld_obs0 = (long)a->ld_obs0; P.rows = (long)a->rows; P.D = a->D;
    P.zmean = a->zmean; P.zstd = a->zstd; P.xn = a->xn; P.xnT = a->xnT; P.ldT = (long)a->ldT;
    P.rsum = a->ref_sum; P.rsumsq = a->ref_sumsq; P.rcount = a->ref_count; P.reps = a->ref_eps;
    P.ref_filter = a->ref_filter; P.xr = a->xr;
    P.obs_next = a->obs_next; P.ld_next = (long)a->ld_next; P.xnext = a->xnext;
    P.ref_log_var = a->ref_log_var; P.A = a->A; P.ref_std = a->ref_std; P.ld_ref = (long)a->ld_ref;
    P.zero_words = a->zero_words; P.n_zero = a->n_zero;
    P.n_x = P.rows * P.D;
    P.n_std = a->ref_std ? P.rows * a->A : 0;
    P.pack.count = 0; P.pack.total = 0;
    if (a->n_pack > 0) {
        const int rc = fill_pack(P.pack, a->pack, a->n_pack);
        if (rc) return rc;
    }
    const long total = 2 * P.n_x + (P.xnext ? P.n_x : 0) + P.n_std + P.pack.total;
    long blocks = (total + 255) / 256;
    if (blocks > 4096) blocks = 4096;
    hipLaunchKernelGGL(epoch_prepare_kernel, dim3((unsigned)blocks), dim3(256), 0, smx_s(stream), P);
    SMX_LAUNCH_CHECK();
    return SMX_OK;
}

extern "C" void smx_epoch_debug_tbuf(void* p) { g_tbuf = (long long*)p; }

extern "C" int32_t smx_epoch_blocks(int64_t rows) { return (int32_t)((rows + ER - 1) / ER); }

static int fwd_lds_bytes(int D, int H1, int H2, int A) {
    const int floats = ER * (r64(D) + 4) + ER * (r64(H1) + 4) + ER * (r64(H2) + 4) + ER * LDO + NWV * 2 * 256 +
                       loss_scratch_floats(A) + ER * (5 * A + 1);
    return floats * (int)sizeof(float);
}
static int fb_loss_floats(int A) {
    const int a = loss_scratch_floats(A) + ER * (5 * A + 1), b = FIN_CH * (8 + 2 * A);
    return a > b ? a : b;
}
static int fb_lds_bytes(int D, int H1, int H2, int A) {
    const int floats = ER * (r64(D) + 4) + ER * (r64(H1) + 4) + ER * (r64(H2) + 4) + ER * LDO + 2 * ER * LDZ +
                       ER * (r64(H2) + 4) + NWV * 2 * 256 + fb_loss_floats(A);
    return floats * (int)sizeof(float);
}
constexpr int MAX_LDS = 128 * 1024;

extern "C" int32_t smx_epoch_supported(int32_t D, int32_t H1, int32_t H2, int32_t OUT) {
    return D > 0 && H1 > 0 && H2 > 0 && OUT > 0 && H1 % 4 == 0 && H2 % 4 == 0 && OUT <= 32 &&
           D <= 2048 && H1 <= 16 * NWV * TG * 2 && H2 <= 16 * NWV * TG * 2 &&
           fwd_lds_bytes(D, H1, H2, OUT) <= MAX_LDS;
}

extern "C" int32_t smx_epoch_fwdbwd_supported(int32_t D, int32_t H1, int32_t H2, int32_t OUT) {
    return smx_epoch_supported(D, H1, H2, OUT) && H2 <= 16 * FNWV * FTG && fb_lds_bytes(D, H1, H2, OUT) <= MAX_LDS;
}

enum { KIND_FWD = 0, KIND_BWD = 1, KIND_FB = 2 };

static int fill_args(EArgs& G, const smx_epoch_job_t* jobs, int32_t njobs, const smx_ppo_losses_t* loss,
                     int64_t n_total, int fsplit, int kind) {
    const bool backward = kind == KIND_BWD;
    SMX_REQUIRE(jobs, SMX_E_NULL);
    SMX_REQUIRE(njobs >= 1 && njobs <= MAX_EJOBS, SMX_E_SHAPE);
    memset(&G, 0, sizeof(G));
    G.n = njobs;
    G.n_total = n_total;
    G.fsplit = fsplit;
    G.tbuf = g_tbuf;
    int base = 0, maxD = 0, maxH1 = 0, maxH2 = 0, A = 0;
    for (int k = 0; k < njobs; ++k) {
        const smx_epoch_job_t& s = jobs[k];
        SMX_REQUIRE(s.net && s.x, SMX_E_NULL);
        const smx_mlp3_t& n = *s.net;
        SMX_REQUIRE(smx_epoch_supported(n.D, n.H1, n.H2, n.OUT), SMX_E_UNSUPPORTED);
        SMX_REQUIRE(s.rows > 0 && s.rows < (1 << 30), SMX_E_SHAPE);
        SMX_REQUIRE(((n.D & 3) || ((uintptr_t)s.x & 15) == 0) && ((uintptr_t)n.W1 & 3) == 0 &&
                        ((uintptr_t)n.W2 & 15) == 0 && ((uintptr_t)n.W3 & 15) == 0 && ((uintptr_t)n.b1 & 15) == 0 &&
                        ((uintptr_t)n.b2 & 15) == 0,
                    SMX_E_ALIGN);
        SMX_REQUIRE((!s.h1T && !s.h2T) || (s.h1T && s.h2T && s.ldT >= s.rows), SMX_E_SHAPE);
        EJob& J = G.j[k];
        J.W1 = n.W1; J.b1 = n.b1; J.W2 = n.W2; J.b2 = n.b2; J.W3 = n.W3; J.b3 = n.b3;
        J.D = n.D; J.H1 = n.H1; J.H2 = n.H2; J.OUT = n.OUT;
        J.x = s.x; J.rows = (int)s.rows; J.h1T = s.h1T; J.h2T = s.h2T; J.ldT = (long)s.ldT;
        J.out = s.out; J.out_ld = s.out_ld ? s.out_ld : n.OUT; J.out_act = s.out_act; J.loss = s.loss;
        J.stop = s.stop_flag;
        J.dz3 = s.dz3; J.dz3T = s.dz3T; J.dz2T = s.dz2T; J.dz1T = s.dz1T;

        {
            SMX_REQUIRE(s.packed, SMX_E_NULL);
            SMX_REQUIRE(((uintptr_t)s.packed & 15) == 0, SMX_E_ALIGN);
            J.P1 = s.packed;
            J.P2 = s.packed + 4 * pack_off(n.D, n.H1, n.H2, n.OUT, 1);
            J.P3 = s.packed + 4 * pack_off(n.D, n.H1, n.H2, n.OUT, 2);
            J.P2T = s.packed + 4 * pack_off(n.D, n.H1, n.H2, n.OUT, 3);
            J.P3T = s.packed + 4 * pack_off(n.D, n.H1, n.H2, n.OUT, 4);
        }
        J.blk_base = base;
        base += smx_epoch_blocks(s.rows) * fsplit;
        if (s.loss == SMX_EPOCH_RHS_SURR || s.loss == SMX_EPOCH_RHS_KL) {
            SMX_REQUIRE(backward, SMX_E_UNSUPPORTED);
            SMX_REQUIRE(loss && loss->g_surr && loss->g_kl && s.dz3T, SMX_E_NULL);
        }
        if (s.loss == SMX_EPOCH_LOSS_POLICY || s.loss == SMX_EPOCH_RHS_SURR || s.loss == SMX_EPOCH_RHS_KL) {
            SMX_REQUIRE(loss, SMX_E_NULL);
            SMX_REQUIRE(loss->A == n.OUT && loss->A <= MAX_A, SMX_E_SHAPE);
            SMX_REQUIRE(loss->rows == s.rows, SMX_E_SHAPE);
            A = loss->A;
        }
        if (s.loss == SMX_EPOCH_LOSS_VALUE) {
            SMX_REQUIRE(loss && n.OUT == 1, SMX_E_SHAPE);
            SMX_REQUIRE(backward ? s.dz3 != nullptr : (loss->returns && loss->v_dz3 && loss->v_partials), SMX_E_NULL);
        }
        if (backward || kind == KIND_FB) SMX_REQUIRE(s.h1T && s.h2T && s.dz2T && s.dz1T, SMX_E_NULL);
        if (kind == KIND_FB) {
            SMX_REQUIRE(s.loss == SMX_EPOCH_LOSS_POLICY || s.loss == SMX_EPOCH_LOSS_VALUE, SMX_E_UNSUPPORTED);
            SMX_REQUIRE(smx_epoch_fwdbwd_supported(n.D, n.H1, n.H2, n.OUT), SMX_E_UNSUPPORTED);
            SMX_REQUIRE(s.loss != SMX_EPOCH_LOSS_POLICY || s.dz3T, SMX_E_NULL);
        }
        maxD = n.D > maxD ? n.D : maxD; maxH1 = n.H1 > maxH1 ? n.H1 : maxH1; maxH2 = n.H2 > maxH2 ? n.H2 : maxH2;
    }
    if (loss) {
        const smx_ppo_losses_t& a = *loss;
        G.pl.mode = a.mode; G.pl.A = a.A; G.pl.log_var = a.log_var; G.pl.actions = a.actions; G.pl.behave = a.behave;
        G.pl.ref = a.ref; G.pl.adv = a.adv; G.pl.ld_act = a.ld_act; G.pl.ld_beh = a.ld_beh; G.pl.ld_ref = a.ld_ref;
        G.pl.check_stop = a.check_stop; G.pl.will_update = a.will_update; G.pl.g_surr = a.g_surr; G.pl.g_kl = a.g_kl;
        G.pl.row_partials = a.row_partials; G.pl.dlogvar = a.dlogvar; G.pl.dlogvar_sumsq = a.dlogvar_sumsq;
        G.pl.stats = a.stats;
        G.vl.returns = a.returns; G.vl.v_dz3 = a.v_dz3; G.vl.v_partials = a.v_partials;
        G.vl.will_update = a.v_will_update;
    }
    if (!backward && njobs == 2 && fsplit == 1) {
        const int nb0 = smx_epoch_blocks(jobs[0].rows), nb1 = smx_epoch_blocks(jobs[1].rows);
        if (nb0 == nb1 && (nb0 & 3) == 0) G.xsplit = nb0;
    }
    G.ldx = r64(maxD) + 4; G.ldh1 = r64(maxH1) + 4; G.ldh2 = r64(maxH2) + 4;
    if (backward) { G.ldx = 0; G.ldh1 = 0; }
    G.off_h1 = backward ? ER * LDZ : ER * G.ldx;
    G.off_h2 = G.off_h1 + ER * G.ldh1;
    G.off_out = G.off_h2 + ER * G.ldh2;
    G.off_g = G.off_out + ER * LDO;
    G.off_red = G.off_out + (backward ? 0 : ER * LDO) + (kind == KIND_FB ? 2 * ER * LDZ + ER * G.ldh2 : 0);
    G.off_loss = G.off_red + (backward ? 0 : NWV * 2 * 256);
    const int loss_floats = backward ? FIN_CH * (8 + 2 * MAX_A)
                                     : (kind == KIND_FB ? fb_loss_floats(A) : loss_scratch_floats(A) + ER * (5 * A + 1));
    const int bytes = (G.off_loss + loss_floats) * (int)sizeof(float);
    return bytes > EXCLUSIVE_LDS ? bytes : EXCLUSIVE_LDS;
}

extern "C" int smx_epoch_forward_f32(const smx_epoch_job_t* jobs, int32_t njobs, const smx_ppo_losses_t* loss,
                                     smx_ppo_ctrl_t* ctrl, int64_t n_total, smx_stream_t stream) {
    EArgs G;
    const int lds = fill_args(G, jobs, njobs, loss, n_total, 1, KIND_FWD);
    if (lds < 0) return lds;
    SMX_REQUIRE(ctrl, SMX_E_NULL);
    if (loss && loss->mode != SMX_PPO_CLIP && loss->mode != SMX_PPO_ADAPT) return SMX_E_UNSUPPORTED;
    for (int k = 0; k < njobs; ++k)
        if (jobs[k].loss == SMX_EPOCH_LOSS_POLICY)
            SMX_REQUIRE(loss->log_var && loss->actions && loss->behave && loss->ref && loss->adv && loss->g_surr &&
                            loss->g_kl && loss->row_partials, SMX_E_NULL);
    const EJob& Lj = G.j[njobs - 1];
    const int blocks = Lj.blk_base + smx_epoch_blocks(Lj.rows);
    SMX_REQUIRE(lds <= MAX_LDS, SMX_E_UNSUPPORTED);
    static bool attr_set = false;
    if (!attr_set) {
        (void)hipFuncSetAttribute((const void*)epoch_fwd_kernel, hipFuncAttributeMaxDynamicSharedMemorySize, 128 * 1024);
        attr_set = true;
    }
    hipLaunchKernelGGL(epoch_fwd_kernel, dim3(blocks), dim3(FNTH), lds, smx_s(stream), G, ctrl);
    SMX_LAUNCH_CHECK();
    return SMX_OK;
}

extern "C" int smx_epoch_backward_f32(const smx_epoch_job_t* jobs, int32_t njobs, const smx_ppo_losses_t* loss,
                                      smx_ppo_ctrl_t* ctrl, int64_t n_total, smx_stream_t stream);

extern "C" int smx_epoch_fwdbwd_f32(const smx_epoch_job_t* jobs, int32_t njobs, const smx_ppo_losses_t* loss,
                                    smx_ppo_ctrl_t* ctrl, int64_t n_total, int32_t* sync_word, uint64_t* kl_slots,
                                    smx_stream_t stream) {
    EArgs G;
    SMX_REQUIRE(loss && ctrl, SMX_E_NULL);
    const int lds = fill_args(G, jobs, njobs, loss, n_total, 1, KIND_FB);
    if (lds < 0) return lds;
    if (loss->mode != SMX_PPO_CLIP && loss->mode != SMX_PPO_ADAPT) return SMX_E_UNSUPPORTED;
    int n_policy = 0;
    for (int k = 0; k < njobs; ++k)
        if (jobs[k].loss == SMX_EPOCH_LOSS_POLICY) {
            SMX_REQUIRE(loss->will_update, SMX_E_UNSUPPORTED);
            SMX_REQUIRE(loss->log_var && loss->actions && loss->behave && loss->ref && loss->adv && loss->g_surr &&
                            loss->g_kl && loss->row_partials && loss->dlogvar && loss->stats && sync_word && kl_slots,
                        SMX_E_NULL);
            SMX_REQUIRE(((uintptr_t)kl_slots & 7) == 0, SMX_E_ALIGN);
            ++n_policy;
        }
    SMX_REQUIRE(n_policy <= 1, SMX_E_SHAPE);
    {
        const int n_cu = smx_cu_count();
        const EJob& Lj0 = G.j[njobs - 1];
        const int blocks0 = Lj0.blk_base + smx_epoch_blocks(Lj0.rows);
        if (n_policy && loss->mode == SMX_PPO_ADAPT && blocks0 > n_cu) {
            const int rc = smx_epoch_forward_f32(jobs, njobs, loss, ctrl, n_total, stream);
            if (rc) return rc;
            return smx_epoch_backward_f32(jobs, njobs, loss, ctrl, n_total, stream);
        }
    }
    G.sync = (int*)sync_word;
    G.kl_slots = (unsigned long long*)kl_slots;
    for (int k = 0; k < njobs; ++k)
        if (jobs[k].loss == SMX_EPOCH_LOSS_POLICY) {
            G.nb_pol = smx_epoch_blocks(jobs[k].rows);
            G.pol_stop = jobs[k].stop_flag;
        }
    const EJob& Lj = G.j[njobs - 1];
    const int blocks = Lj.blk_base + smx_epoch_blocks(Lj.rows);
    SMX_REQUIRE(lds <= MAX_LDS, SMX_E_UNSUPPORTED);
    static bool attr_set_fb = false;
    if (!attr_set_fb) {
        (void)hipFuncSetAttribute((const void*)epoch_fb_kernel, hipFuncAttributeMaxDynamicSharedMemorySize, 128 * 1024);
        attr_set_fb = true;
    }
    hipLaunchKernelGGL(epoch_fb_kernel, dim3(blocks), dim3(FNTH), lds, smx_s(stream), G, ctrl);
    SMX_LAUNCH_CHECK();
    return SMX_OK;
}

extern "C" int smx_epoch_backward_f32(const smx_epoch_job_t* jobs, int32_t njobs, const smx_ppo_losses_t* loss,
                                      smx_ppo_ctrl_t* ctrl, int64_t n_total, smx_stream_t stream) {
    EArgs G;
    bool update = true;
    for (int k = 0; k < njobs && jobs; ++k)
        if (jobs[k].loss == SMX_EPOCH_LOSS_POLICY && loss && !loss->will_update) update = false;
    const int fs = 2;
    const int lds = fill_args(G, jobs, njobs, loss, n_total, fs, KIND_BWD);
    if (lds < 0) return lds;
    SMX_REQUIRE(ctrl, SMX_E_NULL);
    for (int k = 0; k < njobs; ++k)
        if (jobs[k].loss == SMX_EPOCH_LOSS_POLICY) {
            SMX_REQUIRE(loss->log_var && loss->g_surr && loss->g_kl && loss->row_partials && loss->dlogvar &&
                            loss->stats, SMX_E_NULL);
            SMX_REQUIRE(!update || jobs[k].dz3T, SMX_E_NULL);
        }
    const EJob& Lj = G.j[njobs - 1];
    int blocks = Lj.blk_base + smx_epoch_blocks(Lj.rows) * fs;
    if (!update) {
        SMX_REQUIRE(njobs == 1, SMX_E_SHAPE);
        blocks = 1;
    }
    static bool attr_set_b = false;
    if (!attr_set_b) {
        (void)hipFuncSetAttribute((const void*)epoch_bwd_kernel, hipFuncAttributeMaxDynamicSharedMemorySize, 128 * 1024);
        attr_set_b = true;
    }
    hipLaunchKernelGGL(epoch_bwd_kernel, dim3(blocks), dim3(NTH), lds, smx_s(stream), G, ctrl);
    SMX_LAUNCH_CHECK();
    return SMX_OK;
}

__global__ void occupy_kernel(long long ticks, int* sink) {
    extern __shared__ float occ[];
    const long long t0 = (long long)wall_clock64();
    float acc = 0.f;
    while ((long long)wall_clock64() - t0 < ticks) {
        occ[threadIdx.x] = acc;
        acc += occ[(threadIdx.x + 1) & 63];
        __builtin_amdgcn_s_sleep(8);
    }
    if (acc == 12345.678f && sink) *sink = 1;
}

extern "C" int smx_device_occupy(int32_t blocks, int64_t microseconds, smx_stream_t stream) {
    SMX_REQUIRE(blocks > 0 && blocks <= 4096 && microseconds >= 0 && microseconds <= 2000000, SMX_E_SHAPE);
    static bool attr_set_o = false;
    if (!attr_set_o) {
        (void)hipFuncSetAttribute((const void*)occupy_kernel, hipFuncAttributeMaxDynamicSharedMemorySize, 128 * 1024);
        attr_set_o = true;
    }
    hipLaunchKernelGGL(occupy_kernel, dim3(blocks), dim3(64), EXCLUSIVE_LDS, smx_s(stream), (long long)microseconds * 100LL,
                       (int*)nullptr);
    SMX_LAUNCH_CHECK();
    return SMX_OK;
}
```

surreal_amd/csrc/smx_ppo_loss.inc.h:

```cpp
#pragma once

#ifndef SMX_LDS_BARRIER
#define SMX_LDS_BARRIER() __syncthreads()
#endif

constexpr int LOSS_ROWS_PER_BLOCK = 16;
constexpr int MAX_A = 32;

__host__ __device__ constexpr int loss_scratch_floats(int A) { return LOSS_ROWS_PER_BLOCK * (8 * A + 1) + 2 * MAX_A; }
__device__ __forceinline__ const float* loss_elem_dmu(const float* sm, int A) { return sm + 5 * LOSS_ROWS_PER_BLOCK * A; }
__device__ __forceinline__ const float* loss_elem_dkl(const float* sm, int A) { return sm + 6 * LOSS_ROWS_PER_BLOCK * A; }
__device__ __forceinline__ const float* loss_row_dll(const float* sm, int A) { return sm + 8 * LOSS_ROWS_PER_BLOCK * A; }
constexpr int POLICY_LOSS_BARRIERS = 3;

__device__ __forceinline__ float clamp_min_nan(float x, float lo) {
    return (x == x) ? fmaxf(x, lo) : x;
}

template <bool COH>
__device__ __forceinline__ void partial_store(float* p, float v) {
    if constexpr (COH) __hip_atomic_store(p, v, __ATOMIC_RELAXED, __HIP_MEMORY_SCOPE_AGENT);
    else *p = v;
}

template <bool COH = false>
__device__ __forceinline__ void policy_loss_body(
    const int blk, float* sm,
    int mode, const float* __restrict__ mean_blk, const int ld_mean, const float* __restrict__ log_var,
    const float* __restrict__ g_actions, int ld_act, const float* __restrict__ g_behave, int ld_beh,
    const float* __restrict__ g_ref, int ld_ref, const float* __restrict__ adv, long rows, int A,
    const smx_ppo_ctrl_t* __restrict__ ctrl, float* __restrict__ g_surr, float* __restrict__ g_kl,
    float* __restrict__ partials, const float gscale = 1.0f, const bool scaled = false,
    float* __restrict__ g_surr_t = nullptr, float* __restrict__ g_kl_t = nullptr, const long ld_t = 0,
    const long in_row0 = 0 ,
    const int ld_adv = 1,
    unsigned long long* __restrict__ kl_slot = nullptr ) {
    const int R = LOSS_ROWS_PER_BLOCK;
    float* e_z2 = sm;
    float* e_zb2 = e_z2 + R * A;
    float* e_lsb = e_zb2 + R * A;
    float* e_kl = e_lsb + R * A;
    float* e_klb = e_kl + R * A;
    float* e_dmu = e_klb + R * A;
    float* e_dkl = e_dmu + R * A;
    float* e_gk = e_dkl + R * A;
    float* r_dll = e_gk + R * A;
    float* s_sig = r_dll + R;
    float* s_lsig = s_sig + MAX_A;
    const long row0 = (long)blk * R;
    long nrows = rows - row0;
    if (nrows > R) nrows = R;
    const int tid = threadIdx.x;
    const int stride = 8 + 2 * A;
    float* P = partials + (size_t)blk * stride;

    if (tid < A) {
        const float sg = expf(log_var[tid]);
        s_sig[tid] = sg;
        s_lsig[tid] = logf(sg);
    }
    SMX_LDS_BARRIER();
    const int n_el = (int)nrows * A;
    for (int i0 = tid; i0 < n_el; i0 += 512) {
        float o_z2[2], o_zb2[2], o_lsb[2], o_kl[2], o_klb[2], o_dmu[2], o_dkl[2], o_gk[2];
#pragma unroll
        for (int u = 0; u < 2; ++u) {
            const int i = min(i0 + 256 * u, n_el - 1);
            const int rr = i / A, a = i - rr * A;
            const long gr = row0 + rr - in_row0;
            const float sig = s_sig[a];
            const float mu = mean_blk[rr * ld_mean + a];
            const float ac = g_actions[gr * ld_act + a];
            const float mb = g_behave[gr * ld_beh + a], sb = g_behave[gr * ld_beh + A + a];
            const float mr = g_ref[gr * ld_ref + a], sr = g_ref[gr * ld_ref + A + a];
            const float z = (ac - mu) / sig;
            const float zb = (ac - mb) / sb;
            const float s2 = sig * sig;
            const float dt = 1.0f - mu * mu;
            const float num = sr * sr + (mr - mu) * (mr - mu);
            o_z2[u] = z * z;
            o_zb2[u] = zb * zb;
            o_lsb[u] = logf(sb);
            o_kl[u] = logf(sig / sr) + num / (2.0f * s2);
            o_klb[u] = logf(sb / sr) + (sr * sr + (mr - mb) * (mr - mb)) / (2.0f * (sb * sb));
            o_dmu[u] = ((ac - mu) / s2) * dt;
            o_dkl[u] = ((mu - mr) / s2) * dt;
            o_gk[u] = 1.0f - num / s2;
        }
#pragma unroll
        for (int u = 0; u < 2; ++u) {
            const int i = i0 + 256 * u;
            if (i < n_el) {
                e_z2[i] = o_z2[u]; e_zb2[i] = o_zb2[u]; e_lsb[i] = o_lsb[u]; e_kl[i] = o_kl[u];
                e_klb[i] = o_klb[u]; e_dmu[i] = o_dmu[u]; e_dkl[i] = o_dkl[u]; e_gk[i] = o_gk[u];
            }
        }
    }
    SMX_LDS_BARRIER();

    if (tid < 64) {
        const int r = tid >> 2, q = tid & 3;
        const bool ok = r < nrows;
        const float c_ll = (float)(0.5 * 1.8378770664093453  * (double)A);
        const float half_d = (float)(0.5 * (double)A);
        float s1 = 0.f, s2 = 0.f, sb1 = 0.f, sb2 = 0.f, klr = 0.f, klbr = 0.f;
        if (ok) {
            for (int a = q; a < A; a += 4) {
                s1 += e_z2[r * A + a];
                s2 += s_lsig[a];
                sb1 += e_zb2[r * A + a];
                sb2 += e_lsb[r * A + a];
                klr += e_kl[r * A + a];
                klbr += e_klb[r * A + a];
            }
        }
#pragma unroll
        for (int off = 1; off <= 2; off <<= 1) {
            s1 += __shfl_xor(s1, off, 64);
            s2 += __shfl_xor(s2, off, 64);
            sb1 += __shfl_xor(sb1, off, 64);
            sb2 += __shfl_xor(sb2, off, 64);
            klr += __shfl_xor(klr, off, 64);
            klbr += __shfl_xor(klbr, off, 64);
        }
        const float ll = ((-0.5f * s1) - c_ll) - s2;
        const float llb = ((-0.5f * sb1) - c_ll) - sb2;
        const float el = expf(ll);
        const float Ll = clamp_min_nan(el, 1e-5f);
        const float Lb = clamp_min_nan(expf(llb), 1e-5f);
        const float kl = klr - half_d;
        const float klb = klbr - half_d;
        const float ad = ok ? adv[(row0 + r - in_row0) * ld_adv] : 0.f;
        float surr, loss_r, dLl;
        if (mode == SMX_PPO_CLIP) {
            const float eps = ctrl->clip_eps;
            const float lo = (float)(1.0 - (double)eps), hi = (float)(1.0 + (double)eps);
            const float ratio = Ll / Lb;
            float cr = ratio;
            if (cr == cr) cr = fminf(fmaxf(cr, lo), hi);
            surr = -ratio * ad;
            const float cs = -cr * ad;
            loss_r = (surr >= cs) ? surr : cs;
            dLl = (surr >= cs) ? (-ad / Lb) : 0.f;
        } else {
            const float Lbc = clamp_min_nan(Lb, 1e-2f);
            surr = -(ad * (Ll / Lbc));
            loss_r = surr;
            dLl = -ad / Lbc;
        }
        const float dll = (el >= 1e-5f) ? dLl * el : 0.f;
        if (q == 0) r_dll[r] = ok ? dll : 0.f;
        const float isw = Ll / (Lb + 1e-4f);
        const bool one = ok && q == 0;
        const float v0 = smx_wave_sum(one ? surr : 0.f);
        const float v1 = smx_wave_sum(one ? loss_r : 0.f);
        const float v2 = smx_wave_sum(one ? kl : 0.f);
        const float v3 = smx_wave_sum(one ? Lb : 0.f);
        const float v4 = smx_wave_sum(one ? isw : 0.f);
        const float v5 = smx_wave_sum(one ? klb : 0.f);
        if (tid == 0) {
            if (COH && kl_slot)
                __hip_atomic_store(kl_slot + blk, (unsigned long long)__float_as_uint(v2) | (1ull << 32), __ATOMIC_RELAXED,
                                   __HIP_MEMORY_SCOPE_AGENT);
            partial_store<COH>(P + 0, v0); partial_store<COH>(P + 1, v1); partial_store<COH>(P + 2, v2);
            partial_store<COH>(P + 3, v3); partial_store<COH>(P + 4, v4); partial_store<COH>(P + 5, v5);
            partial_store<COH>(P + 6, 0.f); partial_store<COH>(P + 7, 0.f);
        }
    }
    SMX_LDS_BARRIER();

    if (g_surr) {
        for (int i = tid; i < (int)nrows * A; i += 256) {
            const int rr = i / A;
            float gs = r_dll[rr] * e_dmu[i], gk = e_dkl[i];
            if (scaled) { gs *= gscale; gk *= gscale; }
            g_surr[row0 * A + i] = gs;
            g_kl[row0 * A + i] = gk;
            if (g_surr_t) {
                const long at = (long)(i - rr * A) * ld_t + row0 + rr;
                g_surr_t[at] = gs;
                if (g_kl_t) g_kl_t[at] = gk;
            }
        }
    }
    if (tid < 4 * A) {
        const int a = tid >> 2, q = tid & 3;
        float gs = 0.f, gk = 0.f;
        for (int rr = q; rr < (int)nrows; rr += 4) {
            gs += r_dll[rr] * (e_z2[rr * A + a] - 1.0f);
            gk += e_gk[rr * A + a];
        }
#pragma unroll
        for (int off = 1; off <= 2; off <<= 1) {
            gs += __shfl_xor(gs, off, 64);
            gk += __shfl_xor(gk, off, 64);
        }
        if (q == 0) {
            partial_store<COH>(P + 8 + a, gs);
            partial_store<COH>(P + 8 + A + a, gk);
        }
    }
}

constexpr int FIN_CH = 64;
__device__ __forceinline__ void reduce_row_partials(const float* __restrict__ partials, int nblk,
                                                    int stride, float* S, float* buf) {
    const int Q = 256 / stride;
    const int q = (int)threadIdx.x / stride, c = (int)threadIdx.x - q * stride;
    float t = 0.f;
    for (int b0 = 0; b0 < nblk; b0 += FIN_CH) {
        const int nb = min(FIN_CH, nblk - b0);
        const int cnt = nb * stride;
        const float* src = partials + (size_t)b0 * stride;
        for (int i0 = threadIdx.x; i0 < cnt; i0 += 8 * 256) {
            float v[8];
#pragma unroll
            for (int u = 0; u < 8; ++u) v[u] = src[min(i0 + 256 * u, cnt - 1)];
#pragma unroll
            for (int u = 0; u < 8; ++u)
                if (i0 + 256 * u < cnt) buf[i0 + 256 * u] = v[u];
        }
        SMX_LDS_BARRIER();
        if (q < Q)
            for (int b = q; b < nb; b += Q) t += buf[b * stride + c];
        SMX_LDS_BARRIER();
    }
    if (q < Q) buf[q * stride + c] = t;
    SMX_LDS_BARRIER();
    if ((int)threadIdx.x < stride) {
        float s = buf[threadIdx.x];
        for (int k = 1; k < Q; ++k) s += buf[k * stride + threadIdx.x];
        S[threadIdx.x] = s;
    }
    SMX_LDS_BARRIER();
}

__device__ __forceinline__ void loss_and_kl_coef(int mode, const float* S, float n,
                                                 const smx_ppo_ctrl_t* __restrict__ ctrl,
                                                 float& loss, float& c_kl) {
    const float surr_mean = S[0] / n;
    const float kl_mean = S[2] / n;
    c_kl = 0.f;
    if (mode == SMX_PPO_CLIP) {
        loss = S[1] / n;
    } else {
        const float beta = ctrl->beta, eta = ctrl->eta;
        const double kt2 = 2.0 * (double)ctrl->kl_target;
        loss = surr_mean + beta * kl_mean;
        c_kl = beta;
        if ((double)kl_mean - kt2 > 0.0) {
            const float d = kl_mean - (float)kt2;
            loss += eta * (d * d);
            c_kl += 2.0f * eta * d;
        }
    }
}

__device__ __forceinline__ void write_policy_scalars(const float* S, float n, float loss, float c_kl,
                                                     const float* __restrict__ log_var, int A,
                                                     smx_ppo_ctrl_t* __restrict__ ctrl,
                                                     int check_stop, int will_update,
                                                     float* __restrict__ dlogvar_sumsq,
                                                     float* __restrict__ stats) {
    const float inv_n = 1.0f / n;
    const float kl_mean = S[2] / n;
    float ls = 0.f, dq = 0.f;
    for (int a = 0; a < A; ++a) {
        ls += logf(expf(log_var[a]));
        const float g = (S[8 + a] + c_kl * S[8 + A + a]) * inv_n;
        dq += g * g;
    }
    if (dlogvar_sumsq) *dlogvar_sumsq = dq;
    stats[SMX_PS_SURR] = S[0] / n;
    stats[SMX_PS_LOSS] = loss;
    stats[SMX_PS_ENTROPY] = 0.5f * ls + (float)(0.5 * 2.8378770664093453 * (double)A);
    stats[SMX_PS_KL] = kl_mean;
    stats[SMX_PS_LB] = S[3] / n;
    stats[SMX_PS_ISW] = S[4] / n;
    stats[SMX_PS_REFBEH] = S[5] / n;
    int stop = 0;
    if (check_stop && (double)kl_mean > 4.0 * (double)ctrl->kl_target) stop = 1;
    if (stop) {
        ctrl->stop_flag = 1;
    } else if (will_update) {
        ctrl->adam_step_actor += 1;
        ctrl->epochs_done += 1;
    }
}
```

surreal_amd/kernels.py:

```python
import ctypes

import torch

from surreal_amd import _lib as L


def _row_stride(view, width):
    assert view.dim() == 2 and view.shape[1] == width and (width == 1 or view.stride(1) == 1), \
        (tuple(view.shape), view.stride())
    return view.stride(0) if view.shape[0] > 1 else max(view.stride(0), width)


def ddpg_rows_ln(kernels):
    return bool(getattr(kernels, 'ddpg_rows_ln', False))


def ddpg_rows_ln_td3(kernels):
    return bool(getattr(kernels, 'ddpg_rows_ln_td3', False))


def ddpg_rows_td3(kernels):
    return bool(getattr(kernels, 'ddpg_rows_td3', False))


# ... 81 lines not shown
            ld = 0 if out.dim() < 2 or out.stride(0) == out.shape[1] else out.stride(0)
            rc = L.load().smx_mlp3_forward_rows_f32(ctypes.byref(net.desc), L.ptr(x), x.shape[0], L.ptr(h1), L.ptr(h2),
                                                    L.ptr(out), act, ld, L.ptr(pack), pack.numel() * 4, L.ptr(stop), self._st())
            if rc != L.SMX_E_UNSUPPORTED:
                L.check(rc, 'smx_mlp3_forward_rows_f32')
                return
        L.call('smx_mlp3_forward_f32', ctypes.byref(net.desc), L.ptr(x), x.shape[0], L.ptr(h1),
               L.ptr(h2), L.ptr(out), act, L.ptr(stop), self._st())

    def _jobs(self, jobs):
        arr = (L.Mlp3Job * len(jobs))()
        for k, j in enumerate(jobs):
            g = lambda name: L.ptr(j.get(name)) if j.get(name) is not None else None
            arr[k].net = ctypes.pointer(j['net'].desc)
            arr[k].x = g('x')
            arr[k].rows = j['x'].shape[0]
            arr[k].h1, arr[k].h2, arr[k].out = g('h1'), g('h2'), g('out')
            arr[k].out_act = int(j.get('act', 0))
            out = j.get('out')
            arr[k].out_ld = 0 if out is None or out.dim() < 2 or out.stride(0) == out.shape[1] \
                else out.stride(0)
            arr[k].dz3, arr[k].dz2, arr[k].dz1 = g('dz3'), g('dz2'), g('dz1')
            arr[k].grads, arr[k].sumsq_partials = g('grads'), g('sumsq')
            arr[k].stop_flag = g('stop')
            arr[k].h1T, arr[k].h2T, arr[k].xT = g('h1T'), g('h2T'), g('xT')
            arr[k].dz3T, arr[k].dz2T, arr[k].dz1T = g('dz3T'), g('dz2T'), g('dz1T')
            tv = j.get('h1T')
            arr[k].ldT = 0 if tv is None else (tv.stride(0) if tv.shape[0] > 1 else tv.shape[1])
        return arr

    def mlp3_forward_multi(self, jobs):
        L.call('smx_mlp3_forward_multi_f32', self._jobs(jobs), len(jobs), self._st())

    def mlp3_backward_multi(self, jobs):
        L.call('smx_mlp3_backward_multi_f32', self._jobs(jobs), len(jobs), self._st())

    def mlp3_backward_partials(self, net):
        return self.lib.smx_mlp3_backward_partials(net.D, net.H1, net.H2, net.OUT)

    def mlp3_backward(self, net, x, h1, h2, dz3, dz2, dz1, grads, sumsq, stop=None, ws=None, packT=None, dx=None):
        if ws is not None and sumsq is None and packT is not None and x.shape[0] >= self.FUSED_ROWS_MIN and \
                dz2.is_contiguous() and dz1.is_contiguous() and (dx is None or dx.is_contiguous()):
            rc = L.load().smx_mlp3_backward_rows_f32(
                ctypes.byref(net.desc), L.ptr(x), L.ptr(h1), L.ptr(h2), L.ptr(dz3), x.shape[0], L.ptr(dz2), L.ptr(dz1),
                L.ptr(dx), L.ptr(grads), L.ptr(ws), ws.numel(), L.ptr(packT), packT.numel(), L.ptr(stop), self._st())
            if rc != L.SMX_E_UNSUPPORTED:
                L.check(rc, 'smx_mlp3_backward_rows_f32')
                return dx is not None
        if ws is not None and sumsq is None:
            L.call('smx_mlp3_backward_splitk_f32', ctypes.byref(net.desc), L.ptr(x), L.ptr(h1), L.ptr(h2),
                   L.ptr(dz3), x.shape[0], L.ptr(dz2), L.ptr(dz1), L.ptr(grads), L.ptr(ws), ws.numel(),
                   L.ptr(stop), self._st())
            return False
        L.call('smx_mlp3_backward_f32', ctypes.byref(net.desc), L.ptr(x), L.ptr(h1), L.ptr(h2),
               L.ptr(dz3), x.shape[0], L.ptr(dz2), L.ptr(dz1), L.ptr(grads), L.ptr(sumsq),
               L.ptr(stop), self._st())

    def mlp3_backward_ws_floats(self, net, rows):
        return int(self.lib.smx_mlp3_backward_ws_floats(net.D, net.H1, net.H2, net.OUT, int(rows)))

    def mlp3_dgrad_rows_ws_floats(self, net):
        return int(self.lib.smx_mlp3_dgrad_rows_ws_floats(net.D, net.H1, net.H2, net.OUT))

    def epoch_supported(self, *nets):
        ok = all(self.lib.smx_epoch_supported(n.D, n.H1, n.H2, n.OUT) for n in nets)
        return bool(ok and self.lib.smx_epoch_supported(max(n.D for n in nets), max(n.H1 for n in nets),
                                                        max(n.H2 for n in nets), max(n.OUT for n in nets)))

    def epoch_blocks(self, rows):
        return self.lib.smx_epoch_blocks(rows)

    def epoch_packed_numel(self, net):
        return self.lib.smx_epoch_packed_floats(net.D, net.H1, net.H2, net.OUT)

    def epoch_pack(self, items):
        arr = (L.EpochPack * len(items))()
        for k, (net, packed) in enumerate(items):
            arr[k].net = ctypes.pointer(net.desc)
            arr[k].packed = L.ptr(packed)
        L.call('smx_epoch_pack_f32', arr, len(items), self._st())

    def epoch_prepare(self, obs0, xn, xnT, xr, zmean=None, zstd=None, ref_filter=None, obs_next=None, xnext=None,
                      ref_log_var=None, ref_std=None, pack=(), zero_words=None):
        rows, D = obs0.shape
        a = L.EpochPrep()
        a.obs0, a.ld_obs0, a.rows, a.D = L.ptr(obs0), _row_stride(obs0, D), rows, D
        a.zmean, a.zstd = L.ptr(zmean), L.ptr(zstd)
        a.xn, a.xnT = L.ptr(xn), L.ptr(xnT)
        a.ldT = 0 if xnT is None else (xnT.stride(0) if xnT.shape[0] > 1 else xnT.shape[1])
        if ref_filter is not None:
            a.ref_sum, a.ref_sumsq, a.ref_count = L.ptr(ref_filter.running_sum), L.ptr(ref_filter.running_sumsq), \
                L.ptr(ref_filter.count)
            a.ref_eps, a.ref_filter = float(ref_filter.eps), 1
        a.xr = L.ptr(xr)
        if xnext is not None:
            a.obs_next, a.ld_next, a.xnext = L.ptr(obs_next), _row_stride(obs_next, D), L.ptr(xnext)
        if ref_std is not None:
            A = ref_std.shape[1]
            a.A, a.ref_log_var, a.ref_std, a.ld_ref = A, L.ptr(ref_log_var), L.ptr(ref_std), _row_stride(ref_std, A)
        if zero_words is not None:
            a.zero_words, a.n_zero = L.ptr(zero_words), zero_words.numel()
        a.n_pack = len(pack)
        for k, (net, packed) in enumerate(pack):
            a.pack[k].net = ctypes.pointer(net.desc)
            a.pack[k].packed = L.ptr(packed)
        L.call('smx_epoch_prepare_f32', ctypes.byref(a), self._st())

    _EPOCH_LOSS = {None: L.EPOCH_LOSS_NONE, 'policy': L.EPOCH_LOSS_POLICY, 'value': L.EPOCH_LOSS_VALUE,
                   'rhs_surr': L.EPOCH_RHS_SURR, 'rhs_kl': L.EPOCH_RHS_KL}

    def _epoch_jobs(self, jobs):
        arr = (L.EpochJob * len(jobs))()
        for k, j in enumerate(jobs):
            g = lambda name: L.ptr(j.get(name)) if j.get(name) is not None else None
            x = j['x']
            assert x.is_contiguous()
            arr[k].net = ctypes.pointer(j['net'].desc)
            arr[k].x, arr[k].rows = L.ptr(x), x.shape[0]
            arr[k].h1T, arr[k].h2T = g('h1T'), g('h2T')
            tv = j.get('h1T')
            arr[k].ldT = 0 if tv is None else (tv.stride(0) if tv.shape[0] > 1 else tv.shape[1])
            out = j.get('out')
            arr[k].out = g('out')
            arr[k].out_ld = 0 if out is None or out.dim() < 2 or out.stride(0) == out.shape[1] else out.stride(0)
            arr[k].out_act = int(j.get('act', 0))
            arr[k].loss = self._EPOCH_LOSS[j.get('loss')]
            arr[k].stop_flag = g('stop')
            arr[k].dz3, arr[k].dz3T, arr[k].dz2T, arr[k].dz1T = g('dz3'), g('dz3T'), g('dz2T'), g('dz1T')
            arr[k].packed = g('packed')
        return arr

    @staticmethod
    def _epoch_loss(loss):
        if loss is None:
            return None
        a = L.PpoLosses()
        g = lambda name: L.ptr(loss.get(name)) if loss.get(name) is not None else None
        a.mode = int(loss.get('mode', 0))
        if loss.get('log_var') is not None:
            A = loss['log_var'].numel()
            a.A, a.rows = A, int(loss['rows'])
            a.log_var, a.adv = g('log_var'), g('adv')
            if loss.get('actions') is not None:
                a.actions, a.ld_act = g('actions'), _row_stride(loss['actions'], A)
                a.behave, a.ld_beh = g('behave'), _row_stride(loss['behave'], 2 * A)
                a.ref, a.ld_ref = g('ref'), _row_stride(loss['ref'], 2 * A)
            a.g_surr, a.g_kl, a.row_partials = g('g_surr'), g('g_kl'), g('partials')
            a.check_stop, a.will_update = int(loss.get('check_stop', 0)), int(loss.get('will_update', 0))
            a.dlogvar, a.dlogvar_sumsq, a.stats = g('dlogvar'), g('dlogvar_sumsq'), g('stats')
        a.returns, a.v_dz3, a.v_partials = g('returns'), g('v_dz3'), g('v_partials')
        a.v_will_update = int(loss.get('v_will_update', 0))
        return ctypes.byref(a)

    def epoch_forward(self, jobs, loss=None, ctrl=None, n_total=0):
        L.call('smx_epoch_forward_f32', self._epoch_jobs(jobs), len(jobs), self._epoch_loss(loss),
               L.ptr(ctrl), int(n_total), self._st())

    def epoch_backward(self, jobs, loss, ctrl, n_total):
        L.call('smx_epoch_backward_f32', self._epoch_jobs(jobs), len(jobs), self._epoch_loss(loss),
               L.ptr(ctrl), int(n_total), self._st())

    def epoch_fwdbwd_supported(self, *nets):
        return bool(all(self.lib.smx_epoch_fwdbwd_supported(n.D, n.H1, n.H2, n.OUT) for n in nets) and
                    self.lib.smx_epoch_fwdbwd_supported(max(n.D for n in nets), max(n.H1 for n in nets),
                                                        max(n.H2 for n in nets), max(n.OUT for n in nets)))

    def epoch_fwdbwd(self, jobs, loss, ctrl, n_total, sync_word, kl_slots):
        L.call('smx_epoch_fwdbwd_f32', self._epoch_jobs(jobs), len(jobs), self._epoch_loss(loss),
               L.ptr(ctrl), int(n_total), L.ptr(sync_word), L.ptr(kl_slots), self._st())

    def layernorm_forward(self, x, gamma, beta, eps, y, mean=None, rstd=None):
        rows, F = x.shape
        L.call('smx_layernorm_forward_f32', L.ptr(x), x.stride(0), rows, F, L.ptr(gamma), L.ptr(beta), float(eps), L.ptr(y),
               y.stride(0), L.ptr(mean), L.ptr(rstd), self._st())

    def layernorm_backward_ws_floats(self, rows, F):
        return int(self.lib.smx_layernorm_backward_ws_floats(int(rows), int(F)))

    def layernorm_backward(self, dy, x, mean, rstd, gamma, dx, dgamma, dbeta, ws, relu_mask=False):
        rows, F = x.shape
        L.call('smx_layernorm_backward_f32', L.ptr(dy), dy.stride(0), L.ptr(x), x.stride(0), L.ptr(mean), L.ptr(rstd),
               L.ptr(gamma), rows, F, int(bool(relu_mask)), L.ptr(dx), dx.stride(0), L.ptr(dgamma), L.ptr(dbeta), L.ptr(ws),
               ws.numel(), self._st())

    def device_occupy(self, blocks, microseconds):
        L.call('smx_device_occupy', int(blocks), int(microseconds), self._st())

    def mlp3_wgrad_multi(self, jobs):
        L.call('smx_mlp3_wgrad_multi_f32', self._jobs(jobs), len(jobs), self._st())

    def gae(self, values, rewards, dones, gpow, lpow, gamma, gamma_H, B, N, H, adv, ret,
            values_tail=None):
        L.call('smx_windowed_gae_returns_f32', L.ptr(values), L.ptr(values_tail), L.ptr(rewards),
               L.ptr(dones),
               L.ptr(gpow), L.ptr(lpow), float(gamma), float(gamma_H), B, N, H, L.ptr(adv),
               L.ptr(ret), self._st())

    def gae_norm(self, values, rewards, dones, gpow, lpow, gamma, gamma_H, B, N, H, adv, ret, adv_mom, min_std, ticket,
                 values_tail=None):
        L.call('smx_windowed_gae_norm_f32', L.ptr(values), L.ptr(values_tail), L.ptr(rewards), L.ptr(dones),
               L.ptr(gpow), L.ptr(lpow), float(gamma), float(gamma_H), B, N, H, L.ptr(adv), L.ptr(ret), L.ptr(adv_mom),
               float(min_std), L.ptr(ticket), self._st())

    def reward_filter_partials(self):
        return int(self.lib.smx_reward_filter_partials())

    def reward_filter(self, rewards, scale, state, eps, out, partials, ticket, use_filter=True, update=True, sums=None):
        L.call('smx_reward_filter_f32', L.ptr(rewards), rewards.numel(), float(scale), int(use_filter), L.ptr(state),
               float(eps), int(update), L.ptr(out), L.ptr(sums), L.ptr(partials), L.ptr(ticket), self._st())

    def learn_epilogue(self, ret, ret_mom, log_var, out4, ticket, zfilter=None, x=None, count_rows=0, v_partials=None,
                       n_epochs=0, nblk=0, v_stats=None, stats_stride=0):
        a = L.LearnEpilogue()
        if zfilter is not None:
            rows, D = x.shape
            a.x, a.ldx, a.rows, a.D = L.ptr(x), _row_stride(x, D), rows, D
            a.running_sum, a.running_sumsq, a.count = L.ptr(zfilter.running_sum), L.ptr(zfilter.running_sumsq), \
                L.ptr(zfilter.count)
            a.count_rows = float(count_rows)
        a.A = log_var.numel()
        a.ret, a.n_ret, a.ret_moments = L.ptr(ret), ret.numel(), L.ptr(ret_mom)
        a.v_partials, a.n_epochs, a.nblk, a.v_stats, a.stats_stride = L.ptr(v_partials), n_epochs, nblk, L.ptr(v_stats), \
            stats_stride
        a.log_var, a.out4, a.ticket = L.ptr(log_var), L.ptr(out4), L.ptr(ticket)
        L.call('smx_ppo_learn_epilogue_f32', ctypes.byref(a), self._st())

    def moments(self, x, out):
        L.call('smx_moments_f32', L.ptr(x), x.numel(), L.ptr(out), self._st())

    def moments_merge(self, parts, out):
        L.call('smx_moments_merge_f32', L.ptr(parts), parts.numel() // 3, L.ptr(out), self._st())

    def adv_normalize(self, x, mom, min_std):
        L.call('smx_adv_normalize_f32', L.ptr(x), x.numel(), L.ptr(mom), float(min_std), self._st())

    def loss_blocks(self, rows):
        return self.lib.smx_ppo_loss_blocks(rows)

    def policy_loss(self, mode, mean, log_var, actions, behave, ref, adv, ctrl, g_surr, g_kl,
                    partials):
        rows, A = mean.shape
        L.call('smx_ppo_policy_loss_f32', mode, L.ptr(mean), L.ptr(log_var), L.ptr(actions),
               _row_stride(actions, A), L.ptr(behave), _row_stride(behave, 2 * A), L.ptr(ref),
               _row_stride(ref, 2 * A), L.ptr(adv), rows, A, L.ptr(ctrl), L.ptr(g_surr),
               L.ptr(g_kl), L.ptr(partials), self._st())

    def partials_fold(self, partials, nblk, out, ctrl=None):
        L.call('smx_ppo_partials_fold_f32', L.ptr(partials), int(nblk), partials.stride(0), L.ptr(out), out.shape[0],
               L.ptr(ctrl), self._st())

    def policy_finalize(self, mode, partials, nblk, g_surr, g_kl, log_var, n_total, ctrl,
                        check_stop, will_update, dz3, dlogvar, dlogvar_sumsq, stats, dz3_t=None):
        rows, A = g_surr.shape
        L.call('smx_ppo_loss_finalize_f32', mode, L.ptr(partials), nblk, L.ptr(g_surr),
               L.ptr(g_kl), L.ptr(log_var), rows, n_total, A, L.ptr(ctrl), int(check_stop),
               int(will_update), L.ptr(dz3), L.ptr(dz3_t),
               0 if dz3_t is None else dz3_t.stride(0), L.ptr(dlogvar), L.ptr(dlogvar_sumsq),
               L.ptr(stats), self._st())

    def _losses_args(self, mode, mean, log_var, actions, behave, ref, adv, g_surr, g_kl, partials,
                     check_stop, will_update, values, returns, v_dz3, v_partials, v_will_update):
        rows, A = mean.shape
        a = L.PpoLosses()
        a.mode, a.A, a.rows = mode, A, rows
        a.mean, a.log_var, a.adv = L.ptr(mean), L.ptr(log_var), L.ptr(adv)
        a.actions, a.ld_act = L.ptr(actions), _row_stride(actions, A)
        a.behave, a.ld_beh = L.ptr(behave), _row_stride(behave, 2 * A)
        a.ref, a.ld_ref = L.ptr(ref), _row_stride(ref, 2 * A)
        a.g_surr, a.g_kl, a.row_partials = L.ptr(g_surr), L.ptr(g_kl), L.ptr(partials)
        a.check_stop, a.will_update = int(check_stop), int(will_update)
        a.values, a.returns = L.ptr(values), L.ptr(returns)
        a.v_dz3, a.v_partials, a.v_will_update = L.ptr(v_dz3), L.ptr(v_partials), int(v_will_update)
        return a

    def epoch_losses(self, mode, mean, log_var, actions, behave, ref, adv, ctrl, g_surr, g_kl,
                     partials, check_stop, will_update, dz3, dlogvar, dlogvar_sumsq, stats, dz3_t=None,
                     values=None, returns=None, v_dz3=None, v_partials=None, v_will_update=True):
        a = self._losses_args(mode, mean, log_var, actions, behave, ref, adv, g_surr, g_kl, partials,
                              check_stop, will_update, values, returns, v_dz3, v_partials, v_will_update)
        a.dz3, a.dz3_t = L.ptr(dz3), L.ptr(dz3_t)
        a.ld_t = 0 if dz3_t is None else (dz3_t.stride(0) if dz3_t.shape[0] > 1 else dz3_t.shape[1])
        a.dlogvar, a.dlogvar_sumsq, a.stats = L.ptr(dlogvar), L.ptr(dlogvar_sumsq), L.ptr(stats)
        L.call('smx_ppo_epoch_losses_f32', ctypes.byref(a), L.ptr(ctrl), self._st())

    def epoch_losses_dp(self, mode, mean, log_var, actions, behave, ref, adv, ctrl, g_surr, g_kl,
                        partials, n_total, g_surr_t=None, g_kl_t=None, values=None, returns=None,
                        v_dz3=None, v_partials=None, v_will_update=True):
        a = self._losses_args(mode, mean, log_var, actions, behave, ref, adv, g_surr, g_kl, partials,
                              False, False, values, returns, v_dz3, v_partials, v_will_update)
        t = g_surr_t
        a.ld_t = 0 if t is None else (t.stride(0) if t.shape[0] > 1 else t.shape[1])
        L.call('smx_ppo_epoch_losses_dp_f32', ctypes.byref(a), int(n_total), L.ptr(g_surr_t),
               L.ptr(g_kl_t), L.ptr(ctrl), self._st())

    def epoch_combine(self, mode, partials, nblk, n_total, log_var, ctrl, check_stop, will_update,
                      stats, grads_a, grads_kl, n_mlp, sumsq_a, grads_c=None, sumsq_c=None):
        a = L.PpoCombine()
        a.mode, a.A, a.nblk, a.n_total = mode, log_var.numel(), nblk, int(n_total)
        a.row_partials, a.log_var, a.stats = L.ptr(partials), L.ptr(log_var), L.ptr(stats)
        a.check_stop, a.will_update = int(check_stop), int(will_update)
        a.grads_a, a.grads_kl = L.ptr(grads_a), L.ptr(grads_kl)
        a.n_mlp, a.n_a, a.sumsq_a = int(n_mlp), grads_a.numel(), L.ptr(sumsq_a)
        a.grads_c, a.sumsq_c = L.ptr(grads_c), L.ptr(sumsq_c)
        a.n_c = 0 if grads_c is None else grads_c.numel()
        L.call('smx_ppo_epoch_combine_f32', ctypes.byref(a), L.ptr(ctrl), self._st())

    def final_stats(self, log_var, zfilter, out4):
        zf = zfilter
        L.call('smx_ppo_final_stats_f32', L.ptr(log_var), log_var.numel(),
               L.ptr(zf.running_sum) if zf is not None else None,
               L.ptr(zf.running_sumsq) if zf is not None else None,
               L.ptr(zf.count) if zf is not None else None,
               zf.running_sum.numel() if zf is not None else 0, L.ptr(out4), self._st())

    def value_loss_blocks(self, rows):
        return self.lib.smx_value_loss_blocks(rows)

    def value_loss(self, values, returns, n_total, dz3, partials, ctrl, will_update):
        L.call('smx_value_loss_f32', L.ptr(values), L.ptr(returns), values.numel(), n_total,
               L.ptr(dz3), L.ptr(partials), L.ptr(ctrl), int(will_update), self._st())
# ... 696 lines not shown
```

surreal_amd/learner/ppo.py:

```python
import gc
import types

import numpy as np
import torch

from surreal_amd import _lib as L
from surreal_amd import kernels as KN
from surreal_amd.learner.aggregator import MultistepAggregatorWithInfo
from surreal_amd.learner.base import Learner, DeferredStats
from surreal_amd.learner.dist import _SegmentedGraph, _dist_info, setup_peer_exchange
from surreal_amd.model.ppo_net import DiagGauss, PPOModel


class LinearWithMinLR(object):

    def __init__(self, initial_lr, num_updates, update_freq=1, min_lr=0.0):
        self.initial_lr = float(initial_lr)
        self.num_updates = max(int(num_updates), 1)
        self.update_freq = max(int(update_freq), 1)
        self.min_lr = float(min_lr)
        self.n = 0
        self.lr = float(initial_lr)

    def get_lr(self):
        return [self.lr]

    def step(self):
        self.n += 1
        if self.n % self.update_freq == 0:
            frac = max(0.0, 1.0 - self.n / self.num_updates)
            self.lr = max(self.min_lr, self.initial_lr * frac)

    def state_dict(self):
        return {'n': self.n, 'lr': self.lr}

    def load_state_dict(self, sd):
        self.n, self.lr = int(sd['n']), float(sd['lr'])


def _stats_layout(Ep, Ev, n_sync):
    lay, o = types.SimpleNamespace(), 0
    for name, n in (('ctrl', L.CTRL_WORDS), ('pstats', (Ep + 1) * L.PS_STRIDE), ('sync', n_sync),
                    ('vstats', Ev * L.VS_STRIDE), ('adv_mom', 3), ('ret_mom', 3), ('spare', 2), ('fin', 4),
                    ('rf_state', 3), ('spare_end', 1)):
        setattr(lay, name, slice(o, o + n))
        o += n
    lay.total = o
    return lay


class PPOLearner(Learner):
    def __init__(self, learner_config, env_config, session_config):
        super().__init__(learner_config, env_config, session_config)
        self.K = KN.default_kernels()
        self.device = KN.default_device()
        self._dist, self.world_size, self.rank = _dist_info()
        self._pending_stats, self._trace, self._epochs_executed, self._kl_record = None, None, 0, []
        self.lazy_stats = self.device != 'cpu' and bool(self.session_config.learner.get('lazy_stats', True))

        self.current_iteration = 0
        self.global_step = 0
        self.gpu_option = 'cuda:all'
        self.use_cuda = True

        algo = self.learner_config.algo
        self.gamma = algo.gamma
        self.lam = algo.advantage.lam
        self.n_step = algo.n_step
        self.use_z_filter = algo.use_z_filter
        self.use_r_filter = algo.use_r_filter
        self.norm_adv = algo.advantage.norm_adv
        self.batch_size = self.learner_config.replay.batch_size
        self.action_dim = self.env_config.action_spec.dim[0]
        self.obs_spec = self.env_config.obs_spec
        self.init_log_sig = algo.consts.init_log_sig
        self.ppo_mode = algo.ppo_mode
        self.if_rnn_policy = algo.rnn.if_rnn_policy
        self.horizon = algo.rnn.horizon
        self.lr_actor = algo.network.lr_actor
        self.lr_critic = algo.network.lr_critic
        self.epoch_policy = algo.consts.epoch_policy
        self.epoch_baseline = algo.consts.epoch_baseline
        self.kl_target = algo.consts.kl_target
        self.adjust_threshold = algo.consts.adjust_threshold
        self.reward_scale = algo.advantage.reward_scale
        self.kl_cutoff_coeff = algo.adapt_consts.kl_cutoff_coeff
        self.beta_init = algo.adapt_consts.beta_init
        self.beta_range = algo.adapt_consts.beta_range
        self.clip_range = algo.clip_consts.clip_range
        self.clip_epsilon_init = algo.clip_consts.clip_epsilon_init
        if self.ppo_mode == 'adapt':
            self.beta = self.beta_init
            self.eta = self.kl_cutoff_coeff
            self.beta_upper = self.beta_range[1]
            self.beta_lower = self.beta_range[0]
            self.beta_adjust_threshold = self.adjust_threshold
        elif self.ppo_mode == 'clip':
            self.clip_epsilon = self.clip_epsilon_init
            self.clip_adjust_threshold = self.adjust_threshold
            self.clip_upper = self.clip_range[1]
            self.clip_lower = self.clip_range[0]
        else:
            raise ValueError('ppo_mode must be "adapt" or "clip", got %r' % (self.ppo_mode,))
        self._mode = L.SMX_PPO_CLIP if self.ppo_mode == 'clip' else L.SMX_PPO_ADAPT
        anneal = algo.network.anneal
        self.min_lr = anneal.min_lr
        self.lr_update_frequency = anneal.lr_update_frequency
        self.frames_to_anneal = anneal.frames_to_anneal
        num_updates = int(self.frames_to_anneal / self.learner_config.parameter_publish.exp_interval)
        if anneal.lr_scheduler != 'LinearWithMinLR':
            raise ValueError('unknown lr_scheduler %r' % (anneal.lr_scheduler,))

        self.exp_counter = 0
        self.kl_record = []

        mk = dict(obs_spec=self.obs_spec, action_dim=self.action_dim,
                  model_config=self.learner_config.model, use_cuda=True,
                  init_log_sig=self.init_log_sig, use_z_filter=self.use_z_filter,
                  if_pixel_input=self.env_config.get('pixel_input', False),
                  rnn_config=algo.rnn, device=self.device, kernels=self.K)
        self.model = PPOModel(**mk)
        self.ref_target_model = PPOModel(**mk)
        self.ref_target_model.update_target_params(self.model)

        net = algo.network
        self.clip_actor_gradient = net.clip_actor_gradient
        self.actor_gradient_clip_value = net.actor_gradient_norm_clip
        self.clip_critic_gradient = net.clip_critic_gradient
        self.critic_gradient_clip_value = net.critic_gradient_norm_clip
        self.actor_regularization = net.actor_regularization
        self.critic_regularization = net.critic_regularization
        self.actor_exp_avg = torch.zeros_like(self.model.actor_flat)
        self.actor_exp_avg_sq = torch.zeros_like(self.model.actor_flat)
        self.critic_exp_avg = torch.zeros_like(self.model.critic_flat)
        self.critic_exp_avg_sq = torch.zeros_like(self.model.critic_flat)
        self.actor_lr_scheduler = LinearWithMinLR(self.lr_actor, num_updates,
                                                  self.lr_update_frequency, self.min_lr)
        self.critic_lr_scheduler = LinearWithMinLR(self.lr_critic, num_updates,
                                                   self.lr_update_frequency, self.min_lr)
        self.aggregator = MultistepAggregatorWithInfo(self.env_config.obs_spec,
                                                      self.env_config.action_spec)
        self.pd = DiagGauss(self.action_dim)
        self.cells = None
        self.filter_rewards = bool(self.use_r_filter) or self.reward_scale != 1.0

        lcfg = self.session_config.learner
        self.use_graph = bool(lcfg.get('use_hip_graph', True)) and self.device != 'cpu' \
            and (self.world_size == 1 or bool(lcfg.get('graph_segments', True)))
        self.fused_epochs = bool(lcfg.get('fused_epochs', True))
        self._ws = None
        self._graphs = {}
        self._ctrl_host = None
        self.trace = None

    def _ensure_ctrl(self, ws):
        vals = [self.actor_lr_scheduler.get_lr()[0], self.critic_lr_scheduler.get_lr()[0],
                getattr(self, 'beta', 0.0), getattr(self, 'eta', 0.0),
                getattr(self, 'clip_epsilon', 0.0), self.kl_target,
                self.actor_gradient_clip_value if self.clip_actor_gradient else 0.0,
                self.critic_gradient_clip_value if self.clip_critic_gradient else 0.0,
                self.actor_regularization, self.critic_regularization]
        if self._ctrl_host != vals:
            ws.ctrl_f[:10].copy_(torch.tensor(vals, dtype=torch.float32))
            self._ctrl_host = vals

    def _sync_words(self):
        return (max(self.epoch_policy, self.epoch_baseline) + 1 + 3) & ~3

    def _workspace(self, B, N, D, A, pix_dtype=None):
        key = (B, N, D, A, pix_dtype)
        if self._ws is not None and self._ws.key == key:
            return self._ws
        ws = types.SimpleNamespace()
        ws.key = key
        ws.E = N - self.horizon + 1 if self.if_rnn_policy else 1
        ws.rows = B * ws.E
        ws.stem = self.if_rnn_policy or self.model.if_pixel
        self._ws_scalars(ws)
        self._ws_critic_pass(ws)
        self._ws_epochs(ws)
        self._ws_exchange(ws)
        self._ws = ws
        self._graphs = {}
        return ws

    def _f(self, *shape):
        return torch.empty(*shape, device=self.device, dtype=torch.float32)

    def _ft(self, n, rows):
        return torch.zeros(n, rows + 16, device=self.device, dtype=torch.float32)[:, :rows]

    def _ws_scalars(self, ws):
        dev, K, B = self.device, self.K, ws.key[0]
        Ep, Ev = self.epoch_policy, self.epoch_baseline
        n_slots = 0 if (ws.stem or self.world_size > 1) else \
            2 * (max(Ep, Ev) + 1) * ((B + 15) // 16)
        if n_slots > (1 << 19):
            n_slots = 0
        ws.n_slots = n_slots
        lay = ws.layout = _stats_layout(Ep, Ev, self._sync_words() + n_slots)
        ws.scal = torch.zeros(lay.total, device=dev, dtype=torch.float32)
        ws.ctrl_f = ws.scal[lay.ctrl]
        ws.ctrl_i = ws.ctrl_f.view(torch.int32)
        ws.pstats = ws.scal[lay.pstats].view(Ep + 1, L.PS_STRIDE)
        ws.sync = ws.scal[lay.sync].view(torch.int32)
        ws.kl_slots = ws.sync[self._sync_words():].view(-1, 2 * ((B + 15) // 16)) if n_slots else None
        ws.vstats = ws.scal[lay.vstats].view(Ev, L.VS_STRIDE)
        ws.adv_mom, ws.ret_mom = ws.scal[lay.adv_mom], ws.scal[lay.ret_mom]
        ws.fin = ws.scal[lay.fin]
        ws.rf_state = ws.scal[lay.rf_state]
        if self._ws is not None:
            ws.rf_state.copy_(self._ws.rf_state)
        else:
            ws.rf_state.copy_(torch.tensor([1e-5, 0.0, 0.0]))
        if self.filter_rewards:
            ws.rew = torch.empty(B, ws.key[1], device=dev, dtype=torch.float32)
            ws.rf_part = torch.zeros(K.reward_filter_partials(), device=dev, dtype=torch.float64)
            ws.rf_ticket = torch.zeros(1, device=dev, dtype=torch.int32)
            ws.rf_sums = torch.zeros(3, device=dev, dtype=torch.float32)
        ws.stop = ws.ctrl_i[L.C_STOP:L.C_STOP + 1]
        ws.xerr = ws.ctrl_i[L.C_XCHG_ERR:L.C_XCHG_ERR + 1]
        ws.zero_block = ws.scal[L.C_STOP:lay.sync.stop]
        ws.gnorm_a = ws.pstats[:, L.PS_GRADNORM:L.PS_GRADNORM + 1]
        ws.gnorm_c = ws.vstats[:, L.VS_GRADNORM:L.VS_GRADNORM + 1]
        if self._ws is not None:
            ws.ctrl_i[L.C_STEP_ACTOR:L.C_STEP_CRITIC + 1].copy_(
                self._ws.ctrl_i[L.C_STEP_ACTOR:L.C_STEP_CRITIC + 1])
        self._ctrl_host = None
        ws.ticket = torch.zeros(2, dtype=torch.int32, device=dev)

    def _ws_critic_pass(self, ws):
        f, dev, cri = self._f, self.device, self.model.critic
        B, N, D = ws.key[:3]
        ws.packed = None if ws.stem else f(self.K.mlp3_packed_numel(cri))
        ws.vals = f(B * (N + 1))
        n_cu = 256
        if dev != 'cpu':
            n_cu = torch.cuda.get_device_properties(torch.cuda.current_device()).multi_processor_count
        rounds = lambda rows: -(-(-(-rows // 128)) // n_cu)
        ws.split_tail = bool(self.session_config.learner.get('split_critic_tail', True)) and \
            rounds(B * (N + 1)) > rounds(B * N) and not ws.stem
        ws.xnext = f(B, D)
        ws.h1t, ws.h2t = f(B, cri.H1), f(B, cri.H2)
        ws.adv = f(ws.rows)
        ws.ret = f(ws.rows)
        idx = torch.tensor(range(N), dtype=torch.float32)
        ws.gpow = torch.pow(self.gamma, idx).to(dev)
        ws.lpow = torch.pow(self.lam, idx).to(dev)
        ws.mom_parts = f(self.world_size, 3)

    def _ws_epochs(self, ws):
        f, ft, K = self._f, self._ft, self.K
        act, cri = self.model.actor, self.model.critic
        B, _, D, A = ws.key[:4]
        rows = ws.rows
        Dx = self.model.stem_in
        ws.xn = f(rows, Dx)
        ws.xr = f(rows, Dx)
        ws.h1a, ws.h2a, ws.mean = f(rows, act.H1), f(rows, act.H2), f(rows, A)
        ws.h1r, ws.h2r, ws.ref_mean = f(rows, act.H1), f(rows, act.H2), f(rows, A)
        ws.ref_pol = f(rows, 2 * A)
        ws.h1c, ws.h2c, ws.vpred = f(rows, cri.H1), f(rows, cri.H2), f(rows)
        ws.g_surr, ws.g_kl, ws.dz3a = f(rows, A), f(rows, A), f(rows, A)
        ws.dz2a, ws.dz1a = f(rows, act.H2), f(rows, act.H1)
        ws.dz3c, ws.dz2c, ws.dz1c = f(rows), f(rows, cri.H2), f(rows, cri.H1)
        if ws.stem:
            self._ws_stem(ws)
        else:
            ws.xnT = ft(D, rows)
            ws.h1aT, ws.h2aT, ws.dz3aT = ft(act.H1, rows), ft(act.H2, rows), ft(A, rows)
            ws.dz2aT, ws.dz1aT = ft(act.H2, rows), ft(act.H1, rows)
            ws.h1cT, ws.h2cT, ws.dz3cT = ft(cri.H1, rows), ft(cri.H2, rows), ft(1, rows)
            ws.dz2cT, ws.dz1cT = ft(cri.H2, rows), ft(cri.H1, rows)
        ws.nblk_p = K.loss_blocks(rows)
        ws.fused = (self.fused_epochs and not ws.stem and
                    (self.world_size == 1 or self.epoch_policy == self.epoch_baseline) and
                    K.epoch_supported(act, cri))
        ws.fb = (ws.fused and self.world_size == 1 and bool(self.session_config.learner.get('fused_fwdbwd', True)) and
                 bool(self.session_config.learner.get('exclusive_device', True)) and not getattr(self, '_fb_timed_out', False) and
                 ws.n_slots > 0 and K.epoch_fwdbwd_supported(act, cri))
        ws.vblocks = K.epoch_blocks if ws.fused else K.value_loss_blocks
        ws.nblk_v = ws.vblocks(rows)
        ws.merged_tail = ws.fused and self.world_size == 1
        if ws.fused:
            assert ws.nblk_p == K.epoch_blocks(rows)
            ws.pk_actor = torch.zeros(K.epoch_packed_numel(act), device=self.device)
            ws.pk_critic = torch.zeros(K.epoch_packed_numel(cri), device=self.device)
            ws.pk_ref = torch.zeros(K.epoch_packed_numel(act), device=self.device)
        ws.pstride = 8 + 2 * A

    def _ws_stem(self, ws):
        f, dev, K = self._f, self.device, self.K
        act, cri = self.model.actor, self.model.critic
        B, N, D, A, pix_dtype = ws.key
        rows, Dx = ws.rows, self.model.stem_in
        R1 = B * (N + 1)
        ws.h0 = ws.c0 = ws.cnn_it = ws.cnn_gae = ws.frames_it = None
        ws.low_it = f(rows, D)
        ws.act_it, ws.beh_it = f(rows, A), f(rows, 2 * A)
        ws.ztmp = f(R1, D)
        ws.lcat, ws.xcat = f(B, N + 1, D), f(R1, Dx)
        ws.h1G, ws.h2G = f(R1, cri.H1), f(R1, cri.H2)
        n_sk = max(K.mlp3_backward_ws_floats(n, rows) for n in (act, cri))
        ws.mlp_sk = f(n_sk) if n_sk else None
        try:
            ws.pack_stem = f(max(K.mlp3_packed_numel(n) for n in (act, cri)))
        except Exception:
            ws.pack_stem = None
        n_z = K.zfilter_update_ws_floats(rows, D)
        ws.zscratch = f(n_z) if n_z else None
        n_pt = max(K.mlp3_dgrad_rows_ws_floats(n) for n in (act, cri))
        ws.packT_stem = f(n_pt) if n_pt else None
        if self.if_rnn_policy:
            F = self.model.rnn_hidden
            nl = self.model.rnn_layers
            ws.h0L, ws.c0L = f(nl, B, F), f(nl, B, F)
            ws.h0, ws.c0 = ws.h0L[0], ws.c0L[0]
            ws.gates, ws.lo, ws.cs, ws.hp, ws.dlo = f(rows, 4 * F), f(rows, F), f(rows, F), f(rows, F), f(rows, F)
            ws.gatesG, ws.loG, ws.csG = f(R1, 4 * F), f(R1, F), f(R1, F)
            ws.upper = [types.SimpleNamespace(gates=f(rows, 4 * F), lo=f(rows, F), cs=f(rows, F),
                                              hp=f(rows, F), dlo=f(rows, F)) for _ in range(nl - 1)]
            ws.loG2 = f(R1, F) if nl > 1 else None
            n_sk = max(K.lstm_backward_ws_floats(r, B, ws.E) for r in self.model.rnns)
            ws.lstm_sk = f(n_sk) if n_sk else None
        if self.model.if_pixel:
            from surreal_amd.model.cnn_stem import CnnStem
            cnn = self.model.cnn
            cam = (cnn.C, cnn.H, cnn.W)
            ws.frames_it = torch.empty((rows,) + cam, device=dev, dtype=pix_dtype)
            ws.fcat = torch.empty((B, N + 1) + cam, device=dev, dtype=pix_dtype)
            ws.dxn = torch.zeros(rows, Dx, device=dev)
            chunk = int(self.session_config.learner.get('cnn_chunk_frames', 2048))
            ws.cnn_it = CnnStem.workspace(cnn, rows, dev, backward=True)
            ws.cnn_it.sk = self.model._cnn_stem.splitk_workspace(cnn, rows, dev)
            ws.cnn_gae = ws.cnn_it if rows >= min(chunk, R1) else \
                CnnStem.workspace(cnn, min(chunk, R1), dev, backward=False)

    def _ws_exchange(self, ws):
        f, ft, dev, K = self._f, self._ft, self.device, self.K
        act, cri = self.model.actor, self.model.critic
        B, _, D, A = ws.key[:4]
        rows, W = ws.rows, self.world_size
        Ev = self.epoch_baseline
        n_a, n_c = self.model.actor_flat.numel(), self.model.critic_flat.numel()
        ws.n_total, ws.B_total, nblk_p_all = rows, B, ws.nblk_p
        if W > 1:
            mine = torch.tensor([rows, B], dtype=torch.int64, device=dev)
            every = torch.empty(2 * W, dtype=torch.int64, device=dev)
            self._dist.all_gather_into_tensor(every, mine)
            every = every.view(-1, 2).tolist()
            ws.n_total, ws.B_total = sum(r for r, _ in every), sum(b for _, b in every)
            ws.nblk_v = max(ws.vblocks(r) for r, _ in every)
            nblk_p_all = max(K.loss_blocks(r) for r, _ in every)
        ws.dp_epoch = W > 1 and not ws.stem
        ws.tail_deferred = ws.dp_epoch and self.epoch_policy >= self.epoch_baseline
        ws.stem_one_exchange = bool(ws.stem and W > 1 and self.ppo_mode == 'clip' and
                                    self.session_config.learner.get('stem_one_exchange', True))
        al = lambda n: (n + 3) & ~3
        if ws.dp_epoch:
            adapt = self.ppo_mode != 'clip'
            off_k = al(n_a + n_c)
            off_p = off_k + (al(act.numel) if adapt else 0)
            ws.ar = torch.zeros(off_p + nblk_p_all * ws.pstride, device=dev)
            ws.grads_all = ws.ar[:n_a + n_c]
            ws.grads_k = ws.ar[off_k:off_k + act.numel] if adapt else None
            ws.ppart_ar = ws.ar[off_p:].view(nblk_p_all, ws.pstride)
            if adapt:
                ws.dz3k, ws.dz2k, ws.dz1k = f(rows, A), f(rows, act.H2), f(rows, act.H1)
                ws.dz3kT, ws.dz2kT, ws.dz1kT = ft(A, rows), ft(act.H2, rows), ft(act.H1, rows)
                ws.sumsq_k = torch.zeros(K.mlp3_backward_partials(act), device=dev)
            nz = 2 * D + 1 if self.use_z_filter else 0
            cuts = np.cumsum([0, ws.pstride, Ev * ws.nblk_v * 8, 3, nz]).tolist()
            ws.tail_cuts = cuts
            ws.tail_pack = torch.zeros(cuts[-1], device=dev)
            ws.tail_gather = f(W, cuts[-1])
            ws.tp_ppart = ws.tail_pack[:cuts[1]].view(1, ws.pstride)
            ws.vpart_loc_all = ws.tail_pack[cuts[1]:cuts[2]].view(Ev, ws.nblk_v, 8)
            ws.tp_ret = ws.tail_pack[cuts[2]:cuts[3]]
            ws.zsum = f(nz) if nz else None
        else:
            ws.grads_all = torch.zeros(n_a + n_c, device=dev)
            ws.vpart_loc_all = torch.zeros(Ev, ws.nblk_v, 8, device=dev)
        ws.grads_a, ws.grads_c = ws.grads_all[:n_a], ws.grads_all[n_a:]
        ws.ppart = f(ws.nblk_p, ws.pstride)
        ws.ppart_sum = f(1, ws.pstride)
        ws.ppart_fold = f(64, ws.pstride)
        if ws.stem_one_exchange:
            ws.ar_pol = torch.zeros(al(n_a) + ws.pstride, device=dev)
            ws.grads_a = ws.ar_pol[:n_a]
            ws.ppart_sum = ws.ar_pol[al(n_a):].view(1, ws.pstride)
        ws.vpart = torch.zeros(Ev, W * ws.nblk_v, 8, device=dev)
        ws.vpart_local = torch.zeros(ws.nblk_v, 8, device=dev)
        ws.vgather = f(W, Ev, ws.nblk_v, 8)
        ws.np_a = K.mlp3_backward_partials(act)
        ws.np_c = K.mlp3_backward_partials(cri)
        ws.sumsq_a = torch.zeros(max(ws.np_a + 1, K.sumsq_blocks(ws.grads_a.numel())), device=dev)
        ws.sumsq_c = torch.zeros(max(ws.np_c, K.sumsq_blocks(ws.grads_c.numel())), device=dev)
        ws.dlogvar = ws.grads_a[act.numel:act.numel + A]
        ws.dlogvar_sumsq = ws.sumsq_a[ws.np_a:ws.np_a + 1]
        if self.use_z_filter:
            ws.zdelta = ws.tail_pack[ws.tail_cuts[3]:] if ws.dp_epoch else torch.zeros(2 * D + 1, device=dev)
        if W > 1:
            need = max(64, ws.ar.numel(), ws.tail_gather.numel()) if ws.dp_epoch else max(64, n_a + n_c)
            if setup_peer_exchange(self, ws.xerr, need):
                self.exchange_kind = self._dist.kind()

    def _to_dev(self, x):
        if torch.is_tensor(x):
            return x.to(self.device, torch.float32)
        return torch.as_tensor(np.asarray(x), dtype=torch.float32).to(self.device)

    def _to_dev_pixels(self, x):
        if not torch.is_tensor(x):
            x = torch.as_tensor(np.asarray(x))
        if x.dtype != torch.uint8:
            x = x.to(torch.float32)
        return x.to(self.device)

    def _preprocess_batch_ppo(self, batch):
        obs, obs_next = batch['obs'], batch['obs_next']
        for modality in obs:
            for key in obs[modality]:
                conv = self._to_dev_pixels if modality == 'pixel' else self._to_dev
                obs[modality][key] = conv(obs[modality][key])
                obs_next[modality][key] = conv(obs_next[modality][key])
        batch['actions'] = self._to_dev(batch['actions'])
        batch['rewards'] = self._to_dev(batch['rewards'])
        batch['dones'] = self._to_dev(batch['dones'])
        if batch.get('persistent_infos') is not None:
            batch['persistent_infos'] = [self._to_dev(x) for x in batch['persistent_infos']]
        if batch.get('onetime_infos') is not None:
            batch['onetime_infos'] = [self._to_dev(x) for x in batch['onetime_infos']]
        return batch

    def _flat_obs(self, obs):
        parts = [obs['low_dim'][k] for k in obs['low_dim'].keys()]
        x = parts[0] if len(parts) == 1 else torch.cat(parts, -1)
        return x.contiguous()

    def _enqueue_gae(self, ws, obs, obs_next, rewards, dones):
        tail = self._enqueue_critic_pass(ws, obs, obs_next)
        if tail is not None:
            self.K.mlp3_forward_multi([tail])
        self._enqueue_gae_from_values(ws, obs, rewards, dones)

    def _enqueue_critic_pass(self, ws, obs, obs_next, filter_tail=True):
        K, m = self.K, self.model
        B, N, D = obs.shape
        zm = zs = None
        if self.use_z_filter:
            K.mlp3_pack_zstats(m.critic, ws.packed, m.z_filter)
            zm, zs = m.z_filter._mean, m.z_filter._std
        else:
            K.mlp3_pack(m.critic, ws.packed)
        if not ws.split_tail:
            K.mlp3_forward_fused(ws.packed, m.critic, obs, obs_next, zm, zs, ws.vals, L.SMX_ACT_NONE)
            return None
        K.mlp3_forward_fused(ws.packed, m.critic, obs, None, zm, zs, ws.vals[:B * N], L.SMX_ACT_NONE)
        if not filter_tail:
            pass
        elif self.use_z_filter:
            K.zfilter_forward(obs_next[:, 0, :], zm, zs, ws.xnext)
        else:
            ws.xnext.copy_(obs_next[:, 0, :])
        return dict(net=m.critic, x=ws.xnext, h1=ws.h1t, h2=ws.h2t, out=ws.vals[B * N:].view(B, 1),
                    act=L.SMX_ACT_NONE)

    def _enqueue_gae_from_values(self, ws, obs, rewards, dones):
        K = self.K
        B, N, D = obs.shape
        vals, tail = (ws.vals[:B * N], ws.vals[B * N:]) if ws.split_tail else (ws.vals, None)
        if ws.merged_tail and self.norm_adv:
            K.gae_norm(vals, rewards, dones, ws.gpow, ws.lpow, self.gamma, self.gamma ** N, B, N, N, ws.adv, ws.ret,
                       ws.adv_mom, 1e-4, ws.ticket[0:1], values_tail=tail)
            return
        K.gae(vals, rewards, dones, ws.gpow, ws.lpow, self.gamma, self.gamma ** N, B, N, N, ws.adv, ws.ret,
              values_tail=tail)
        self._enqueue_adv_normalize(ws)

    def _enqueue_moments(self, ws, x, out):
        self.K.moments(x, out)
        if self.world_size > 1:
            self._dist.all_gather_into_tensor(ws.mom_parts.view(-1), out.clone())
            self.K.moments_merge(ws.mom_parts, out)

    def _enqueue_adv_normalize(self, ws):
        if self.norm_adv:
            self._enqueue_moments(ws, ws.adv, ws.adv_mom)
            self.K.adv_normalize(ws.adv, ws.adv_mom, 1e-4)

    def _enqueue_lockstep_epochs(self, ws, actions0, behave0, first_extra=(), after_first=None):
        K, m = self.K, self.model
        Ep, Ev = self.epoch_policy, self.epoch_baseline
        W = self.world_size
        n_total = ws.n_total
        aj = dict(net=m.actor, x=ws.xn, h1=ws.h1a, h2=ws.h2a, out=ws.mean, act=L.SMX_ACT_TANH,
                  dz3=ws.dz3a, dz2=ws.dz2a, dz1=ws.dz1a, grads=ws.grads_a, sumsq=ws.sumsq_a,
                  stop=ws.stop, xT=ws.xnT, h1T=ws.h1aT, h2T=ws.h2aT, dz3T=ws.dz3aT, dz2T=ws.dz2aT,
                  dz1T=ws.dz1aT)
        cj = dict(net=m.critic, x=ws.xn, h1=ws.h1c, h2=ws.h2c, out=ws.vpred.view(-1, 1),
                  act=L.SMX_ACT_NONE, dz3=ws.dz3c.view(-1, 1), dz2=ws.dz2c, dz1=ws.dz1c,
                  grads=ws.grads_c, sumsq=ws.sumsq_c, xT=ws.xnT, h1T=ws.h1cT, h2T=ws.h2cT,
                  dz3T=ws.dz3c, dz2T=ws.dz2cT, dz1T=ws.dz1cT)
        for e in range(max(Ep + 1, Ev)):
            pol_f, pol_u, val = e <= Ep, e < Ep, e < Ev
            K.mlp3_forward_multi(([aj] if pol_f else []) + ([cj] if val else []) +
                                 (list(first_extra) if e == 0 else []))
            if e == 0 and after_first is not None:
                after_first()
            if ws.dp_epoch and pol_u and val:
                self._enqueue_dp_epoch(ws, e, aj, cj, actions0, behave0)
                continue
            if pol_f and W == 1:
                K.epoch_losses(self._mode, ws.mean, m.log_var.view(-1), actions0, behave0, ws.ref_pol, ws.adv,
                               ws.ctrl_f, ws.g_surr, ws.g_kl, ws.ppart, e > 0, pol_u, ws.dz3a,
                               ws.dlogvar, ws.dlogvar_sumsq, ws.pstats[e], dz3_t=ws.dz3aT,
                               values=ws.vpred if val else None, returns=ws.ret, v_dz3=ws.dz3c,
                               v_partials=ws.vpart[e] if val else None)
            elif pol_f:
                K.policy_loss(self._mode, ws.mean, m.log_var.view(-1), actions0, behave0, ws.ref_pol,
                              ws.adv, ws.ctrl_f, ws.g_surr, ws.g_kl, ws.ppart)
                if ws.tail_deferred and not pol_u and not val:
                    torch.sum(ws.ppart, 0, keepdim=True, out=ws.tp_ppart)
                    continue
                part, nblk = ws.ppart, ws.nblk_p
                if W > 1:
                    torch.sum(ws.ppart, 0, keepdim=True, out=ws.ppart_sum)
                    self._dist.all_reduce(ws.ppart_sum)
                    part, nblk = ws.ppart_sum, 1
                K.policy_finalize(self._mode, part, nblk, ws.g_surr, ws.g_kl, m.log_var.view(-1), n_total,
                                  ws.ctrl_f, e > 0, pol_u, ws.dz3a,
                                  ws.dlogvar, ws.dlogvar_sumsq, ws.pstats[e], dz3_t=ws.dz3aT)
            if val and not (pol_f and W == 1):
                K.value_loss(ws.vpred, ws.ret, n_total, ws.dz3c,
                             ws.vpart_loc_all[e] if W > 1 else ws.vpart[e], ws.ctrl_f, True)
            if pol_u or val:
                K.mlp3_backward_multi(([aj] if pol_u else []) + ([cj] if val else []))
            np_a, np_c = ws.np_a + 1, ws.np_c
            if W > 1:
                if pol_u and val:
                    if self.rank != 0:
                        ws.dlogvar.zero_()
                    self._dist.all_reduce(ws.grads_all)
                elif pol_u:
                    self._dist.all_reduce(ws.grads_a[:m.actor.numel])
                elif val:
                    self._dist.all_reduce(ws.grads_c)
                if pol_u:
                    K.sumsq_partials(ws.grads_a, ws.sumsq_a)
                    np_a = K.sumsq_blocks(ws.grads_a.numel())
                if val:
                    K.sumsq_partials(ws.grads_c, ws.sumsq_c)
                    np_c = K.sumsq_blocks(ws.grads_c.numel())
            self._enqueue_adam(ws, e, pol_u, val, np_a, np_c)
        if ws.tail_deferred:
            return
        self._enqueue_value_finalize(ws)

    def _enqueue_value_finalize(self, ws, gathered=None):
        Ev, W = self.epoch_baseline, self.world_size
        if W > 1:
            if gathered is None:
                self._dist.all_gather_into_tensor(ws.vgather.view(-1), ws.vpart_loc_all.view(-1))
                gathered = ws.vgather
            ws.vpart.view(Ev, W, ws.nblk_v, 8).copy_(gathered.permute(1, 0, 2, 3))
        self.K.value_finalize(ws.vpart, Ev, ws.vpart.shape[1], ws.vstats, L.VS_STRIDE)

    def _clear_foreign_partials(self, ws):
        if ws.nblk_p < ws.ppart_ar.shape[0]:
            ws.ppart_ar[ws.nblk_p:].zero_()

    def _enqueue_fused_epochs(self, ws, actions0, behave0, ref_job, tail, gae):
        K, m = self.K, self.model
        Ep, Ev = self.epoch_policy, self.epoch_baseline
        n_total = ws.n_total
        pre = [dict(net=ref_job['net'], packed=ws.pk_ref, x=ref_job['x'], out=ref_job['out'], act=L.SMX_ACT_TANH)]
        if tail is not None:
            pre.append(dict(net=tail['net'], packed=ws.pk_critic, x=tail['x'], out=tail['out'], act=L.SMX_ACT_NONE))
        K.epoch_forward(pre, None, ws.ctrl_f, n_total)
        gae()
        aj = dict(net=m.actor, packed=ws.pk_actor, x=ws.xn, act=L.SMX_ACT_TANH, loss='policy', stop=ws.stop, h1T=ws.h1aT,
                  h2T=ws.h2aT, dz3T=ws.dz3aT, dz2T=ws.dz2aT, dz1T=ws.dz1aT, xT=ws.xnT, grads=ws.grads_a,
                  sumsq=ws.sumsq_a)
        cj = dict(net=m.critic, packed=ws.pk_critic, x=ws.xn, act=L.SMX_ACT_NONE, loss='value', h1T=ws.h1cT, h2T=ws.h2cT,
                  dz3=ws.dz3c, dz3T=ws.dz3c, dz2T=ws.dz2cT, dz1T=ws.dz1cT, xT=ws.xnT, grads=ws.grads_c,
                  sumsq=ws.sumsq_c)
        dp = ws.dp_epoch
        pack = ((m.actor, ws.pk_actor), (m.critic, ws.pk_critic))
        adapt = self.ppo_mode != 'clip'

        def loss_args(e):
            return dict(mode=self._mode, rows=ws.rows, log_var=m.log_var.view(-1), actions=actions0, behave=behave0,
                        ref=ws.ref_pol, adv=ws.adv, g_surr=ws.g_surr, g_kl=ws.g_kl,
                        partials=ws.ppart_ar if dp and e < Ep else ws.ppart,
                        check_stop=e > 0, will_update=e < Ep,
                        dlogvar=ws.dlogvar, dlogvar_sumsq=ws.dlogvar_sumsq, stats=ws.pstats[min(e, Ep)],
                        returns=ws.ret, v_dz3=ws.dz3c,
                        v_partials=(ws.vpart_loc_all if dp else ws.vpart)[min(e, Ev - 1)], v_will_update=True)

        if dp:
            assert Ep == Ev and ws.tail_deferred
            rhs = [dict(aj, loss='rhs_surr')]
            if adapt:
                rhs.append(dict(aj, loss='rhs_kl', dz3T=ws.dz3kT, dz2T=ws.dz2kT, dz1T=ws.dz1kT, grads=ws.grads_k,
                                sumsq=ws.sumsq_k))
            for e in range(Ep + 1):
                loss = loss_args(e)
                if e == Ep:
                    K.epoch_forward([aj], loss, ws.ctrl_f, n_total)
                    torch.sum(ws.ppart, 0, keepdim=True, out=ws.tp_ppart)
                    break
                self._clear_foreign_partials(ws)
                K.epoch_forward([aj, cj], loss, ws.ctrl_f, n_total)
                K.epoch_backward(rhs + [cj], loss, ws.ctrl_f, n_total)
                K.mlp3_wgrad_multi(rhs + [cj])
                self._enqueue_dp_epoch_tail(ws, e, pack=pack)
            return

        for e in range(max(Ep + 1, Ev)):
            pol_f, pol_u, val = e <= Ep, e < Ep, e < Ev
            loss = loss_args(e)
            bj = ([aj] if pol_u else []) + ([cj] if val else [])
            if ws.fb and (pol_u or not pol_f) and (pol_u or val):
                K.epoch_fwdbwd(bj, loss, ws.ctrl_f, n_total, ws.sync[e:e + 1], ws.kl_slots[e])
                K.mlp3_wgrad_multi(bj)
            else:
                K.epoch_forward(([aj] if pol_f else []) + ([cj] if val else []), loss, ws.ctrl_f, n_total)
                if pol_f and not pol_u:
                    K.epoch_backward([aj], loss, ws.ctrl_f, n_total)
                if pol_u or val:
                    K.epoch_backward(bj, loss, ws.ctrl_f, n_total)
                    K.mlp3_wgrad_multi(bj)
            self._enqueue_adam(ws, e, pol_u, val, ws.np_a + 1, ws.np_c, pack=pack)
            if pol_u != val:
                K.epoch_pack([(m.actor, ws.pk_actor)] if pol_u else [(m.critic, ws.pk_critic)])
        if not ws.merged_tail:
            self._enqueue_value_finalize(ws)

    def _enqueue_tail_exchange(self, ws, obs0, actions0, behave0):
        K, m, W = self.K, self.model, self.world_size
        Ep, Ev, D = self.epoch_policy, self.epoch_baseline, obs0.shape[1]
        c = ws.tail_cuts
        K.moments(ws.ret, ws.tp_ret)
        if self.use_z_filter:
            ws.zdelta.zero_()
            K.zfilter_update(obs0, ws.zdelta[:D], ws.zdelta[D:2 * D], ws.zdelta[2 * D:], obs0.shape[0])
        self._dist.all_gather_into_tensor(ws.tail_gather.view(-1), ws.tail_pack)
        G = ws.tail_gather
        torch.sum(G[:, :c[1]], 0, keepdim=True, out=ws.ppart_sum)
        K.policy_finalize(self._mode, ws.ppart_sum, 1, ws.g_surr, ws.g_kl, m.log_var.view(-1), ws.n_total,
                          ws.ctrl_f, Ep > 0, False, ws.dz3a,
                          ws.dlogvar, ws.dlogvar_sumsq, ws.pstats[Ep], dz3_t=ws.dz3aT)
        self._enqueue_value_finalize(ws, gathered=G[:, c[1]:c[2]].reshape(W, Ev, ws.nblk_v, 8))
        ws.mom_parts.copy_(G[:, c[2]:c[3]])
        K.moments_merge(ws.mom_parts, ws.ret_mom)
        if self.use_z_filter:
            torch.sum(G[:, c[3]:], 0, out=ws.zsum)
            self._z_add(ws.zsum)

    def _enqueue_dp_epoch(self, ws, e, aj, cj, actions0, behave0):
        K, m = self.K, self.model
        adapt = self.ppo_mode != 'clip'
        self._clear_foreign_partials(ws)
        K.epoch_losses_dp(self._mode, ws.mean, m.log_var.view(-1), actions0, behave0, ws.ref_pol, ws.adv,
                          ws.ctrl_f, ws.dz3a, ws.dz3k if adapt else ws.g_kl, ws.ppart_ar, ws.n_total,
                          g_surr_t=ws.dz3aT, g_kl_t=ws.dz3kT if adapt else None, values=ws.vpred,
                          returns=ws.ret, v_dz3=ws.dz3c, v_partials=ws.vpart_loc_all[e])
        jobs = [aj]
        if adapt:
            jobs.append(dict(aj, dz3=ws.dz3k, dz2=ws.dz2k, dz1=ws.dz1k, grads=ws.grads_k,
                             sumsq=ws.sumsq_k, dz3T=ws.dz3kT, dz2T=ws.dz2kT, dz1T=ws.dz1kT))
        K.mlp3_backward_multi(jobs + [cj])
        self._enqueue_dp_epoch_tail(ws, e)

    def _enqueue_dp_epoch_tail(self, ws, e, pack=None):
        K, m = self.K, self.model
        self._dist.all_reduce(ws.ar)
        K.epoch_combine(self._mode, ws.ppart_ar, ws.ppart_ar.shape[0], ws.n_total, m.log_var.view(-1), ws.ctrl_f,
                        e > 0, True, ws.pstats[e], ws.grads_a, ws.grads_k if self.ppo_mode != 'clip' else None,
                        m.actor.numel, ws.sumsq_a, ws.grads_c, ws.sumsq_c)
        self._enqueue_adam(ws, e, True, True, K.sumsq_blocks(ws.grads_a.numel()), K.sumsq_blocks(ws.grads_c.numel()),
                           pack=pack)

    def _enqueue_adam(self, ws, e, actor, critic, np_a, np_c, pack=None):
        K, m = self.K, self.model
        a = (m.actor_flat, ws.grads_a, self.actor_exp_avg, self.actor_exp_avg_sq, ws.sumsq_a, np_a)
        c = (m.critic_flat, ws.grads_c, self.critic_exp_avg, self.critic_exp_avg_sq, ws.sumsq_c, np_c)
        if actor and critic:
            K.clip_adam_pair(a + (True, ws.gnorm_a[e]), c + (False, ws.gnorm_c[e]), ws.ctrl_f, pack=pack)
        elif actor:
            K.clip_adam(*a, ws.ctrl_f, 0, True, ws.gnorm_a[e])
        elif critic:
            K.clip_adam(*c, ws.ctrl_f, 1, False, ws.gnorm_c[e])

    def _enqueue_reward_filter(self, ws, rewards):
        K = self.K
        if self.world_size == 1 or not self.use_r_filter:
            K.reward_filter(rewards, self.reward_scale, ws.rf_state, 1e-5, ws.rew, ws.rf_part, ws.rf_ticket,
                            use_filter=self.use_r_filter, update=self.use_r_filter)
            return ws.rew
        K.reward_filter(rewards, self.reward_scale, ws.rf_state, 1e-5, ws.rew, ws.rf_part, ws.rf_ticket,
                        use_filter=True, update=False, sums=ws.rf_sums)
        self._dist.all_reduce(ws.rf_sums)
        ws.rf_state[:2] += ws.rf_sums[:2]
        ws.rf_state[2:] = ws.rf_sums[2:]
        return ws.rew

    def _enqueue_optimize(self, ws, obs, obs_next, actions, rewards, dones, pds, pix=None,
                          pix_next=None):
        pre_zeroed = self.filter_rewards and self.use_r_filter and self.world_size > 1
        if pre_zeroed:
            ws.zero_block.zero_()
        if self.filter_rewards:
            rewards = self._enqueue_reward_filter(ws, rewards)
        if self.if_rnn_policy or self.model.if_pixel:
            return self._enqueue_optimize_stem(ws, obs, obs_next, actions, rewards, dones, pds, pix,
                                               pix_next, pre_zeroed)
        K, m, ref = self.K, self.model, self.ref_target_model
        B, N, D = obs.shape
        A = self.action_dim
        fused = ws.fused
        if not fused and not pre_zeroed:
            ws.zero_block.zero_()
        tail = self._enqueue_critic_pass(ws, obs, obs_next, filter_tail=not fused)

        obs0 = obs[:, 0, :]
        actions0 = actions[:, 0, :]
        behave0 = pds[:, 0, :]
        if fused:
            zf = m.z_filter if self.use_z_filter else None
            K.epoch_prepare(obs0, ws.xn, ws.xnT, ws.xr, zmean=zf._mean if zf else None, zstd=zf._std if zf else None,
                            ref_filter=ref.z_filter if self.use_z_filter else None,
                            obs_next=obs_next[:, 0, :] if tail is not None else None,
                            xnext=ws.xnext if tail is not None else None,
                            ref_log_var=ref.log_var.view(-1), ref_std=ws.ref_pol[:, A:],
                            pack=[(m.actor, ws.pk_actor), (m.critic, ws.pk_critic), (ref.actor, ws.pk_ref)],
                            zero_words=None if pre_zeroed else ws.zero_block.view(torch.int32))
        elif self.use_z_filter:
            zm, zs = m.z_filter._mean, m.z_filter._std
            K.zfilter_forward(obs0, zm, zs, ws.xn)
            rz = ref.z_filter
            K.zfilter_forward_sums(obs0, rz.running_sum, rz.running_sumsq, rz.count, rz.eps, ws.xr)
        else:
            ws.xn.copy_(obs0)
            ws.xr.copy_(obs0)
        ref_job = dict(net=ref.actor, x=ws.xr, h1=ws.h1r, h2=ws.h2r, out=ws.ref_pol[:, :A],
                       act=L.SMX_ACT_TANH)
        if not fused:
            ws.xnT.copy_(ws.xn.t())
            ws.ref_pol[:, A:].copy_(torch.exp(ref.log_var).expand(ws.rows, A))
        if fused:
            self._enqueue_fused_epochs(ws, actions0, behave0, ref_job, tail,
                                       lambda: self._enqueue_gae_from_values(ws, obs, rewards, dones))
        else:
            self._enqueue_lockstep_epochs(
                ws, actions0, behave0, first_extra=[ref_job] + ([tail] if tail is not None else []),
                after_first=lambda: self._enqueue_gae_from_values(ws, obs, rewards, dones))

        if ws.tail_deferred:
            self._enqueue_tail_exchange(ws, obs0, actions0, behave0)
            self._enqueue_final_stats(ws)
            return
        if fused and ws.merged_tail:
            K.learn_epilogue(ws.ret, ws.ret_mom, m.log_var.view(-1), ws.fin, ws.ticket[1:2],
                             zfilter=m.z_filter if self.use_z_filter else None, x=obs0, count_rows=B,
                             v_partials=ws.vpart, n_epochs=self.epoch_baseline, nblk=ws.vpart.shape[1],
                             v_stats=ws.vstats, stats_stride=L.VS_STRIDE)
            return
        self._enqueue_learn_stats(ws, obs0, B, None)

    def _stem_inputs(self, ws, mm, low2d, frames, xin, cnn_ws, zstats, stop=None):
        K = self.K
        D = low2d.shape[1]
        if zstats is not False:
            if self.use_z_filter:
                K.zfilter_forward(low2d, zstats[0], zstats[1], ws.ztmp[:low2d.shape[0]])
                xin[:, :D].copy_(ws.ztmp[:low2d.shape[0]])
            else:
                xin[:, :D].copy_(low2d)
        if frames is not None:
# ... 476 lines not shown
```

Measured before the change: 122.1 million env-steps/s.

## Split each epoch row-block across two paired workgroups exchanging hidden activations

Each fused forward and forward-backward row-block is now handled by two workgroups. Each computes half of the hidden-layer output tiles and passes its half to its partner through a tagged global exchange buffer that the partner spin-waits on, so twice as many workgroups share the GEMM work when the grid is small. Only the 'publishing' half writes losses, partials and outputs. The cost is cross-workgroup spin synchronisation with a timeout fallback flag, plus a risk of deadlock or stalls if the paired workgroups are not co-resident.

```diff
diff --git a/include/surreal_amd.h b/include/surreal_amd.h
--- a/include/surreal_amd.h
+++ b/include/surreal_amd.h
@@ -315,6 +315,14 @@
 int smx_epoch_fwdbwd_f32(const smx_epoch_job_t* jobs, int32_t njobs, const struct smx_ppo_losses* loss,
                          smx_ppo_ctrl_t* ctrl, int64_t n_total, int32_t* sync_word, uint64_t* kl_slots,
                          smx_stream_t stream);
+int64_t smx_epoch_pair_xchg_bytes(int32_t H1, int32_t H2);
+int32_t smx_epoch_pair_fits(int64_t blocks);
+int smx_epoch_forward_pair_f32(const smx_epoch_job_t* jobs, int32_t njobs, const struct smx_ppo_losses* loss,
+                               smx_ppo_ctrl_t* ctrl, int64_t n_total, void* xchg, int64_t xchg_bytes,
+                               smx_stream_t stream);
+int smx_epoch_fwdbwd_pair_f32(const smx_epoch_job_t* jobs, int32_t njobs, const struct smx_ppo_losses* loss,
+                              smx_ppo_ctrl_t* ctrl, int64_t n_total, int32_t* sync_word, uint64_t* kl_slots,
+                              void* xchg, int64_t xchg_bytes, smx_stream_t stream);
 int smx_device_occupy(int32_t blocks, int64_t microseconds, smx_stream_t stream);
 
 int smx_diaggauss_sample_f32(const float* mean, int64_t ld_mean, const float* log_var,
diff --git a/surreal_amd/_lib.py b/surreal_amd/_lib.py
--- a/surreal_amd/_lib.py
+++ b/surreal_amd/_lib.py
@@ -280,6 +280,11 @@
     'smx_epoch_backward_f32': (c_int32, [POINTER(EpochJob), c_int32, POINTER(PpoLosses), _P, c_int64, _P]),
     'smx_epoch_fwdbwd_supported': (c_int32, [c_int32, c_int32, c_int32, c_int32]),
     'smx_epoch_fwdbwd_f32': (c_int32, [POINTER(EpochJob), c_int32, POINTER(PpoLosses), _P, c_int64, _P, _P, _P]),
+    'smx_epoch_pair_xchg_bytes': (c_int64, [c_int32, c_int32]),
+    'smx_epoch_pair_fits': (c_int32, [c_int64]),
+    'smx_epoch_forward_pair_f32': (c_int32, [POINTER(EpochJob), c_int32, POINTER(PpoLosses), _P, c_int64, _P, c_int64, _P]),
+    'smx_epoch_fwdbwd_pair_f32': (c_int32, [POINTER(EpochJob), c_int32, POINTER(PpoLosses), _P, c_int64, _P, _P, _P,
+                                            c_int64, _P]),
     'smx_device_occupy': (c_int32, [c_int32, c_int64, _P]),
     'smx_layernorm_forward_f32': (c_int32, [_P, c_int64, c_int64, c_int32, _P, _P, c_float, _P, c_int64, _P, _P, _P]),
     'smx_layernorm_backward_ws_floats': (c_int64, [c_int64, c_int32]),
diff --git a/surreal_amd/csrc/smx_epoch.hip b/surreal_amd/csrc/smx_epoch.hip
--- a/surreal_amd/csrc/smx_epoch.hip
+++ b/surreal_amd/csrc/smx_epoch.hip
@@ -68,6 +68,10 @@
     int fsplit;
     int xsplit;
     long long* tbuf;
+    int nblocks;
+    unsigned* xflags;
+    unsigned long long* xbuf;
+    int xoff2, xhalf;
 };
 
 __device__ __forceinline__ int xcd_job_order(const EArgs& G, int raw) {
@@ -127,12 +131,22 @@
     SMX_LDS_BARRIER();
 }
 
-template <bool FB>
+template <bool FB, bool PAIR>
 __device__ __forceinline__ void epoch_fwd_body(const EArgs& G, smx_ppo_ctrl_t* __restrict__ ctrl) {
     extern __shared__ float sm[];
-    const int bid = xcd_job_order(G, (int)blockIdx.x);
-    const int ts_blk = bid;
+    int raw = (int)blockIdx.x, half = 0;
+    if constexpr (PAIR) {
+        const int xcd = raw & 7, slot = raw >> 3;
+        half = slot & 1;
+        raw = (slot >> 1) * 8 + xcd;
+        if (raw >= G.nblocks) return;
+    }
+    const int bid = xcd_job_order(G, raw);
+    const int ts_blk = PAIR ? 2 * bid + half : bid;
     (void)ts_blk;
+    const bool fin_wg = PAIR ? (raw == G.nblocks - 1 && half == 1) : (blockIdx.x == gridDim.x - 1);
+    (void)fin_wg;
+    const bool pub = half == 0;
     TSTAMP(0);
     const EJob J = select_job(G, bid);
     const int stopv = J.stop ? __builtin_nontemporal_load(J.stop) : 0;
@@ -144,6 +158,18 @@
     const int wv = __builtin_amdgcn_readfirstlane(tid >> 6);
     const int fm = lane & 15, kq = lane >> 4;
     TSTAMP(12);
+    int pair_lost = 0;
+    unsigned* xf_mine = nullptr;
+    unsigned long long* xb_mine = nullptr;
+    const unsigned long long* xb_part = nullptr;
+    unsigned xseq[2] = {0u, 0u};
+    if constexpr (PAIR) {
+        xf_mine = G.xflags + ((size_t)bid * 2 + half) * 2;
+        xb_mine = G.xbuf + ((size_t)bid * 2 + half) * (size_t)G.xhalf;
+        xb_part = G.xbuf + ((size_t)bid * 2 + (half ^ 1)) * (size_t)G.xhalf;
+        xseq[0] = __hip_atomic_load(xf_mine, __ATOMIC_RELAXED, __HIP_MEMORY_SCOPE_AGENT) + 1u;
+        xseq[1] = __hip_atomic_load(xf_mine + 1, __ATOMIC_RELAXED, __HIP_MEMORY_SCOPE_AGENT) + 1u;
+    }
 
     float* xs = sm;
     float* h1s = sm + G.off_h1;
@@ -251,18 +277,21 @@
         const rsrc_t rw = make_rsrc(Wp, (unsigned)tiles * (unsigned)C2 * 2048u);
         const rsrc_t rbias = make_rsrc(bias, (unsigned)H * 4u);
         float* stp = l == 2 ? J.out : hT;
-        const bool st_ok = stp != nullptr;
+        const bool st_ok = stp != nullptr && (l < 2 || pub);
+        const bool split = PAIR && l < 2;
+        const int tfirst = split ? 2 * wv + half : wv, tstep = split ? 2 * FNWV : FNWV;
+        unsigned long long* xb_st = split ? xb_mine + (l == 0 ? 0 : G.xoff2) : nullptr;
         const rsrc_t rst = make_rsrc(stp ? stp : Wp, l == 2 ? (unsigned)J.rows * (unsigned)J.out_ld * 4u
                                                              : (unsigned)H * (unsigned)J.ldT * 4u);
 #pragma unroll 1
-        for (int tb = 0; tb < tiles; tb += FNWV * FTG) {
-            const int t0 = tb + wv;
-            int nt = (tiles - t0 + FNWV - 1) / FNWV;
+        for (int tb = 0; tb < tiles; tb += tstep * FTG) {
+            const int t0 = tb + tfirst;
+            int nt = (tiles - t0 + tstep - 1) / tstep;
             nt = nt < 0 ? 0 : (nt > FTG ? FTG : nt);
             float bs[FTG][4];
 #pragma unroll
             for (int g = 0; g < FTG; ++g) {
-                const int f0 = 16 * (t0 + FNWV * g) + 4 * kq;
+                const int f0 = 16 * (t0 + tstep * g) + 4 * kq;
 #pragma unroll
                 for (int r = 0; r < 4; ++r) bs[g][r] = ld4(rbias, (g < nt) ? (unsigned)(f0 + r) * 4u : OOB);
             }
@@ -270,9 +299,9 @@
 #pragma unroll
             for (int g = 0; g < TG; ++g) acc[g] = (f32x4){0.f, 0.f, 0.f, 0.f};
             TSTAMP(16 + 4 * l);
-            if (nt > 2) fwd_tiles<3>(acc, rw, tiles, C2, in_lds, ldi, t0, FNWV, lane);
-            else if (nt > 1) fwd_tiles<2>(acc, rw, tiles, C2, in_lds, ldi, t0, FNWV, lane);
-            else if (nt > 0) fwd_tiles<1>(acc, rw, tiles, C2, in_lds, ldi, t0, FNWV, lane);
+            if (nt > 2) fwd_tiles<3>(acc, rw, tiles, C2, in_lds, ldi, t0, tstep, lane);
+            else if (nt > 1) fwd_tiles<2>(acc, rw, tiles, C2, in_lds, ldi, t0, tstep, lane);
+            else if (nt > 0) fwd_tiles<1>(acc, rw, tiles, C2, in_lds, ldi, t0, tstep, lane);
             TSTAMP(17 + 4 * l);
             const unsigned sstep = l == 2 ? 4u : (unsigned)J.ldT * 4u;
             const unsigned srow = l == 2 ? (unsigned)(row0 + fm) * (unsigned)J.out_ld * 4u
@@ -280,7 +309,7 @@
 #pragma unroll
             for (int g = 0; g < FTG; ++g) {
                 if (g < nt) {
-                    const int f0 = 16 * (t0 + FNWV * g) + 4 * kq;
+                    const int f0 = 16 * (t0 + tstep * g) + 4 * kq;
                     float v[4];
 #pragma unroll
                     for (int r = 0; r < 4; ++r) {
@@ -296,12 +325,63 @@
                         __builtin_amdgcn_raw_buffer_store_b32(__float_as_uint(v[r]), rst,
                                                               ok ? srow + (unsigned)(f0 + r) * sstep : OOB, 0, 0);
                     }
+                    if constexpr (PAIR) {
+                        if (split) {
+                            unsigned long long* q = xb_st + ((t0 + tstep * g) >> 1) * 256 + (4 * kq) * ER + fm;
+                            const unsigned long long tag = (unsigned long long)xseq[l] << 32;
+#pragma unroll
+                            for (int r = 0; r < 4; ++r)
+                                __hip_atomic_store(q + r * ER, tag | __float_as_uint(v[r]), __ATOMIC_RELAXED,
+                                                   __HIP_MEMORY_SCOPE_AGENT);
+                        }
+                    }
                 }
             }
         }
         TSTAMP(18 + 4 * l);
         SMX_LDS_BARRIER();
         TSTAMP(3 + l);
+        if constexpr (PAIR) {
+            if (split) {
+                if (tid == 0)
+                    __hip_atomic_store(xf_mine + l, xseq[l], __ATOMIC_RELAXED, __HIP_MEMORY_SCOPE_AGENT);
+                TSTAMP(27 + 2 * l);
+                if constexpr (!FB) {
+                    if (l == 1 && !pub) return;
+                }
+                const int nthem = ((tiles + half) >> 1) * 256;
+                const unsigned long long* src = xb_part + (l == 0 ? 0 : G.xoff2);
+                const long long t0w = (long long)wall_clock64();
+                for (int i0 = tid; i0 < nthem; i0 += 4 * FNTH) {
+                    unsigned long long w[4];
+                    for (;;) {
+                        bool there = true;
+#pragma unroll
+                        for (int u = 0; u < 4; ++u) {
+                            w[u] = __hip_atomic_load(src + min(i0 + FNTH * u, nthem - 1), __ATOMIC_RELAXED,
+                                                     __HIP_MEMORY_SCOPE_AGENT);
+                            there = there && (unsigned)(w[u] >> 32) == xseq[l];
+                        }
+                        if (there) break;
+                        if ((long long)wall_clock64() - t0w > 25000000LL) {
+                            pair_lost = 1;
+                            atomicOr(&ctrl->reserved[1], 1);
+                            break;
+                        }
+                        __builtin_amdgcn_s_sleep(1);
+                    }
+#pragma unroll
+                    for (int u = 0; u < 4; ++u) {
+                        const int i = i0 + FNTH * u;
+                        if (i < nthem)
+                            out_lds[(i & 15) * ldo + 16 * (2 * (i >> 8) + (half ^ 1)) + ((i >> 4) & 15)] =
+                                __uint_as_float((unsigned)w[u]);
+                    }
+                }
+                SMX_LDS_BARRIER();
+                TSTAMP(28 + 2 * l);
+            }
+        }
     }
 
     if constexpr (!FB) {
@@ -334,6 +414,8 @@
     __shared__ __attribute__((aligned(16))) float S[8 + 2 * MAX_A + 8];
     float& s_kl = S[8 + 2 * MAX_A];
     int& wait_ok = *(int*)&S[8 + 2 * MAX_A + 1];
+    int& pair_bad = *(int*)&S[8 + 2 * MAX_A + 2];
+    if (PAIR && tid == 0) pair_bad = 0;
     static_assert(sizeof(S) % 16 == 0, "static LDS is a multiple of 16 bytes");
     const PolArgs& p = G.pl;
     const bool policy = J.loss == SMX_EPOCH_LOSS_POLICY;
@@ -345,7 +427,7 @@
     float* dz2s = gks + ER * LDZ;
     const float nf = (float)G.n_total;
     const float inv_n = 1.0f / nf;
-    const int pol_stopped = (G.pol_stop && blockIdx.x == gridDim.x - 1) ? __builtin_nontemporal_load(G.pol_stop) : 0;
+    const int pol_stopped = (G.pol_stop && fin_wg) ? __builtin_nontemporal_load(G.pol_stop) : 0;
     const int tiles2 = (J.H2 + 15) >> 4;
     float4 wa[FTG], wb[FTG];
     {
@@ -362,7 +444,7 @@
         if (lo) {
             policy_loss_body<true>(blk, sm + G.off_loss, p.mode, outs, LDO, p.log_var, lin_s, LW, lin_s + p.A, LW,
                                    lin_s + 3 * p.A, LW, lin_s + 5 * p.A, (long)J.rows, p.A, ctrl, nullptr, nullptr,
-                                   p.row_partials, 1.0f, false, nullptr, nullptr, 0, row0, LW, G.kl_slots);
+                                   p.row_partials, 1.0f, false, nullptr, nullptr, 0, row0, LW, G.kl_slots, pub);
         } else {
 #pragma unroll
             for (int i = 0; i < POLICY_LOSS_BARRIERS; ++i) SMX_LDS_BARRIER();
@@ -373,7 +455,7 @@
         const float v = ok ? outs[tid * LDO] : 0.f, g = ok ? vret : 0.f;
         const float d = g - v, e = v - g;
         const float dz = (2.0f * e) / nf;
-        if (ok) q.v_dz3[row0 + tid] = dz;
+        if (ok && pub) q.v_dz3[row0 + tid] = dz;
         if (tid < ER) gss[tid * LDZ] = ok ? dz : 0.f;
         const float cnt = (float)nrows;
         const float md = smx_wave_sum(ok ? d : 0.f) / cnt;
@@ -381,7 +463,7 @@
         const float m2d = smx_wave_sum(ok ? (d - md) * (d - md) : 0.f);
         const float m2g = smx_wave_sum(ok ? (g - mg) * (g - mg) : 0.f);
         const float sq = smx_wave_sum(ok ? e * e : 0.f);
-        if (tid == 0) {
+        if (tid == 0 && pub) {
             float* P = q.v_partials + (size_t)blk * 8;
             P[0] = cnt; P[1] = md; P[2] = m2d; P[3] = mg; P[4] = m2g; P[5] = sq; P[6] = 0.f; P[7] = 0.f;
             if (blk == 0 && q.will_update) ctrl->adam_step_critic += 1;
@@ -389,6 +471,9 @@
     }
     SMX_LDS_BARRIER();
     TSTAMP(6);
+    if constexpr (PAIR) {
+        if (__any(pair_lost) && lane == 0) pair_bad = 1;
+    }
     if (policy) {
         const float* sc = sm + G.off_loss;
         const float* e_dmu = loss_elem_dmu(sc, A);
@@ -477,11 +562,11 @@
     };
     float c_kl = 0.f;
     bool stop_now = false;
-    if (tid == 0) wait_ok = 1;
+    if (tid == 0) wait_ok = PAIR ? (pair_bad == 0) : 1;
     if (adapt) kl_coef(kl_total(), c_kl, stop_now);
-    if (policy && tid < 128) asm volatile("s_waitcnt vmcnt(0)" ::: "memory");
+    if (policy && (PAIR || tid < 128)) asm volatile("s_waitcnt vmcnt(0)" ::: "memory");
     SMX_LDS_BARRIER();
-    if (policy && tid == 0) __hip_atomic_fetch_add(G.sync, 1, __ATOMIC_RELAXED, __HIP_MEMORY_SCOPE_AGENT);
+    if (policy && pub && tid == 0) __hip_atomic_fetch_add(G.sync, 1, __ATOMIC_RELAXED, __HIP_MEMORY_SCOPE_AGENT);
     TSTAMP(8);
     if (!stop_now) {
         {
@@ -498,7 +583,7 @@
                     v.z = (m.z > 0.f) ? aS[g][2] + c_kl * aK[g][2] : 0.f;
                     v.w = (m.w > 0.f) ? aS[g][3] + c_kl * aK[g][3] : 0.f;
                     *(float4*)(dz2s + fm * ldh2 + f0) = v;
-                    const bool ok = fm < nrows;
+                    const bool ok = fm < nrows && (!PAIR || (t & 1) == half);
                     const unsigned o = ((unsigned)f0 * (unsigned)J.ldT + (unsigned)(row0 + fm)) * 4u, st = (unsigned)J.ldT * 4u;
                     __builtin_amdgcn_raw_buffer_store_b32(__float_as_uint(v.x), rout, ok && f0 < J.H2 ? o : OOB, 0, 0);
                     __builtin_amdgcn_raw_buffer_store_b32(__float_as_uint(v.y), rout, ok && f0 + 1 < J.H2 ? o + st : OOB, 0, 0);
@@ -511,7 +596,7 @@
             for (int idx = tid; idx < ER * A; idx += FNTH) {
                 const int a = idx / ER, n = idx - a * ER;
                 const float v = gss[n * LDZ + a] + c_kl * gks[n * LDZ + a];
-                if (n < nrows) J.dz3T[(size_t)a * J.ldT + row0 + n] = v;
+                if (n < nrows && pub) J.dz3T[(size_t)a * J.ldT + row0 + n] = v;
             }
         }
         SMX_LDS_BARRIER();
@@ -521,20 +606,21 @@
             const int C2h = pack_chunks(J.H2);
             const rsrc_t rw2 = make_rsrc(J.P2T, (unsigned)tiles1 * (unsigned)C2h * 2048u);
             const rsrc_t rout = make_rsrc(J.dz1T, (unsigned)J.H1 * (unsigned)J.ldT * 4u);
+            const int tfirst = PAIR ? 2 * wv + half : wv, tstep = PAIR ? 2 * FNWV : FNWV;
 #pragma unroll 1
-            for (int tb = 0; tb < tiles1; tb += FNWV * FTG) {
-                const int t0 = tb + wv;
-                int nt = (tiles1 - t0 + FNWV - 1) / FNWV;
+            for (int tb = 0; tb < tiles1; tb += tstep * FTG) {
+                const int t0 = tb + tfirst;
+                int nt = (tiles1 - t0 + tstep - 1) / tstep;
                 nt = nt < 0 ? 0 : (nt > FTG ? FTG : nt);
                 f32x4 acc[TG];
 #pragma unroll
                 for (int g = 0; g < TG; ++g) acc[g] = (f32x4){0.f, 0.f, 0.f, 0.f};
-                if (nt > 2) fwd_tiles<3>(acc, rw2, tiles1, C2h, dz2s, ldh2, t0, FNWV, lane);
-                else fwd_tiles<2>(acc, rw2, tiles1, C2h, dz2s, ldh2, t0, FNWV, lane);
+                if (nt > 2) fwd_tiles<3>(acc, rw2, tiles1, C2h, dz2s, ldh2, t0, tstep, lane);
+                else fwd_tiles<2>(acc, rw2, tiles1, C2h, dz2s, ldh2, t0, tstep, lane);
 #pragma unroll
                 for (int g = 0; g < FTG; ++g) {
                     if (g < nt) {
-                        const int f0 = 16 * (t0 + FNWV * g) + 4 * kq;
+                        const int f0 = 16 * (t0 + tstep * g) + 4 * kq;
                         const float4 m = *(const float4*)(h1s + fm * ldh1 + f0);
                         const float vx = (m.x > 0.f) ? acc[g][0] : 0.f, vy = (m.y > 0.f) ? acc[g][1] : 0.f;
                         const float vz = (m.z > 0.f) ? acc[g][2] : 0.f, vw = (m.w > 0.f) ? acc[g][3] : 0.f;
@@ -550,7 +636,7 @@
         }
     }
     TSTAMP(10);
-    if (nbp > 0 && blockIdx.x == gridDim.x - 1 && pol_stopped == 0) {
+    if (nbp > 0 && fin_wg && pol_stopped == 0) {
         wait_count();
         fb_reduce_partials(p.row_partials, nbp, pstride, S, sm + G.off_loss);
         const float klsum = kl_total();
@@ -559,7 +645,10 @@
         SMX_LDS_BARRIER();
         loss_and_kl_coef(p.mode, S, nf, ctrl, loss, ck);
         for (int a = tid; a < A; a += FNTH) p.dlogvar[a] = (S[8 + a] + ck * S[8 + A + a]) * inv_n;
-        if (tid == 0 && wait_ok)
+        bool rows_ok = true;
+        if constexpr (PAIR)
+            rows_ok = __hip_atomic_load(&ctrl->reserved[1], __ATOMIC_RELAXED, __HIP_MEMORY_SCOPE_AGENT) == 0;
+        if (tid == 0 && wait_ok && rows_ok)
             write_policy_scalars(S, nf, loss, ck, p.log_var, A, ctrl, p.check_stop, p.will_update, p.dlogvar_sumsq,
                                  p.stats);
     }
@@ -568,11 +657,17 @@
 }
 
 __global__ __launch_bounds__(FNTH) void epoch_fwd_kernel(EArgs G, smx_ppo_ctrl_t* __restrict__ ctrl) {
-    epoch_fwd_body<false>(G, ctrl);
+    epoch_fwd_body<false, false>(G, ctrl);
+}
+__global__ __launch_bounds__(FNTH) void epoch_fwd_pair_kernel(EArgs G, smx_ppo_ctrl_t* __restrict__ ctrl) {
+    epoch_fwd_body<false, true>(G, ctrl);
 }
 
 __global__ __launch_bounds__(FNTH) void epoch_fb_kernel(EArgs G, smx_ppo_ctrl_t* __restrict__ ctrl) {
-    epoch_fwd_body<true>(G, ctrl);
+    epoch_fwd_body<true, false>(G, ctrl);
+}
+__global__ __launch_bounds__(FNTH) void epoch_fb_pair_kernel(EArgs G, smx_ppo_ctrl_t* __restrict__ ctrl) {
+    epoch_fwd_body<true, true>(G, ctrl);
 }
 
 __global__ __launch_bounds__(NTH) void epoch_bwd_kernel(EArgs G, smx_ppo_ctrl_t* __restrict__ ctrl) {
@@ -1024,8 +1119,40 @@
     return bytes > EXCLUSIVE_LDS ? bytes : EXCLUSIVE_LDS;
 }
 
-extern "C" int smx_epoch_forward_f32(const smx_epoch_job_t* jobs, int32_t njobs, const smx_ppo_losses_t* loss,
-                                     smx_ppo_ctrl_t* ctrl, int64_t n_total, smx_stream_t stream) {
+static int pair_half_tiles(int H) { return (((H + 15) >> 4) + 1) >> 1; }
+static int pair_cap_blocks() { return (smx_cu_count() / 2) & ~7; }
+static int64_t pair_flag_bytes() { return ((int64_t)pair_cap_blocks() * 16 + 255) & ~(int64_t)255; }
+
+extern "C" int64_t smx_epoch_pair_xchg_bytes(int32_t H1, int32_t H2) {
+    if (H1 <= 0 || H2 <= 0) return 0;
+    return pair_flag_bytes() + (int64_t)pair_cap_blocks() * 2 * (pair_half_tiles(H1) + pair_half_tiles(H2)) * 2048;
+}
+
+extern "C" int32_t smx_epoch_pair_fits(int64_t blocks) {
+    return blocks > 0 && 2 * ((blocks + 7) & ~(int64_t)7) <= (int64_t)smx_cu_count();
+}
+
+static bool pair_args(EArgs& G, int blocks, int njobs, void* xchg, int64_t xchg_bytes) {
+    if (!xchg || !smx_epoch_pair_fits(blocks) || ((uintptr_t)xchg & 15) != 0) return false;
+    int H1 = 0, H2 = 0;
+    for (int k = 0; k < njobs; ++k) {
+        H1 = G.j[k].H1 > H1 ? G.j[k].H1 : H1;
+        H2 = G.j[k].H2 > H2 ? G.j[k].H2 : H2;
+    }
+    const int64_t share = ((xchg_bytes - pair_flag_bytes()) / (2 * (int64_t)pair_cap_blocks())) & ~(int64_t)2047;
+    if (share < (int64_t)(pair_half_tiles(H1) + pair_half_tiles(H2)) * 2048) return false;
+    G.nblocks = blocks;
+    G.xflags = (unsigned*)xchg;
+    G.xbuf = (unsigned long long*)((char*)xchg + pair_flag_bytes());
+    G.xoff2 = pair_half_tiles(H1) * 256;
+    G.xhalf = (int)(share / 8);
+    return true;
+}
+static int pair_grid(int blocks) { return 2 * ((blocks + 7) & ~7); }
+
+static int epoch_forward_launch(const smx_epoch_job_t* jobs, int32_t njobs, const smx_ppo_losses_t* loss,
+                                smx_ppo_ctrl_t* ctrl, int64_t n_total, void* xchg, int64_t xchg_bytes,
+                                smx_stream_t stream) {
     EArgs G;
     const int lds = fill_args(G, jobs, njobs, loss, n_total, 1, KIND_FWD);
     if (lds < 0) return lds;
@@ -1041,19 +1168,35 @@
     static bool attr_set = false;
     if (!attr_set) {
         (void)hipFuncSetAttribute((const void*)epoch_fwd_kernel, hipFuncAttributeMaxDynamicSharedMemorySize, 128 * 1024);
+        (void)hipFuncSetAttribute((const void*)epoch_fwd_pair_kernel, hipFuncAttributeMaxDynamicSharedMemorySize, 128 * 1024);
         attr_set = true;
     }
-    hipLaunchKernelGGL(epoch_fwd_kernel, dim3(blocks), dim3(FNTH), lds, smx_s(stream), G, ctrl);
+    if (pair_args(G, blocks, njobs, xchg, xchg_bytes))
+        hipLaunchKernelGGL(epoch_fwd_pair_kernel, dim3(pair_grid(blocks)), dim3(FNTH), lds, smx_s(stream), G, ctrl);
+    else
+        hipLaunchKernelGGL(epoch_fwd_kernel, dim3(blocks), dim3(FNTH), lds, smx_s(stream), G, ctrl);
     SMX_LAUNCH_CHECK();
     return SMX_OK;
 }
 
+extern "C" int smx_epoch_forward_f32(const smx_epoch_job_t* jobs, int32_t njobs, const smx_ppo_losses_t* loss,
+                                     smx_ppo_ctrl_t* ctrl, int64_t n_total, smx_stream_t stream) {
+    return epoch_forward_launch(jobs, njobs, loss, ctrl, n_total, nullptr, 0, stream);
+}
+
+extern "C" int smx_epoch_forward_pair_f32(const smx_epoch_job_t* jobs, int32_t njobs, const smx_ppo_losses_t* loss,
+                                          smx_ppo_ctrl_t* ctrl, int64_t n_total, void* xchg, int64_t xchg_bytes,
+                                          smx_stream_t stream) {
+    SMX_REQUIRE(xchg && xchg_bytes > 0, SMX_E_NULL);
+    return epoch_forward_launch(jobs, njobs, loss, ctrl, n_total, xchg, xchg_bytes, stream);
+}
+
 extern "C" int smx_epoch_backward_f32(const smx_epoch_job_t* jobs, int32_t njobs, const smx_ppo_losses_t* loss,
                                       smx_ppo_ctrl_t* ctrl, int64_t n_total, smx_stream_t stream);
 
-extern "C" int smx_epoch_fwdbwd_f32(const smx_epoch_job_t* jobs, int32_t njobs, const smx_ppo_losses_t* loss,
-                                    smx_ppo_ctrl_t* ctrl, int64_t n_total, int32_t* sync_word, uint64_t* kl_slots,
-                                    smx_stream_t stream) {
+static int epoch_fwdbwd_launch(const smx_epoch_job_t* jobs, int32_t njobs, const smx_ppo_losses_t* loss,
+                               smx_ppo_ctrl_t* ctrl, int64_t n_total, int32_t* sync_word, uint64_t* kl_slots,
+                               void* xchg, int64_t xchg_bytes, smx_stream_t stream) {
     EArgs G;
     SMX_REQUIRE(loss && ctrl, SMX_E_NULL);
     const int lds = fill_args(G, jobs, njobs, loss, n_total, 1, KIND_FB);
@@ -1093,11 +1236,28 @@
     static bool attr_set_fb = false;
     if (!attr_set_fb) {
         (void)hipFuncSetAttribute((const void*)epoch_fb_kernel, hipFuncAttributeMaxDynamicSharedMemorySize, 128 * 1024);
+        (void)hipFuncSetAttribute((const void*)epoch_fb_pair_kernel, hipFuncAttributeMaxDynamicSharedMemorySize, 128 * 1024);
         attr_set_fb = true;
     }
-    hipLaunchKernelGGL(epoch_fb_kernel, dim3(blocks), dim3(FNTH), lds, smx_s(stream), G, ctrl);
+    if (pair_args(G, blocks, njobs, xchg, xchg_bytes))
+        hipLaunchKernelGGL(epoch_fb_pair_kernel, dim3(pair_grid(blocks)), dim3(FNTH), lds, smx_s(stream), G, ctrl);
+    else
+        hipLaunchKernelGGL(epoch_fb_kernel, dim3(blocks), dim3(FNTH), lds, smx_s(stream), G, ctrl);
     SMX_LAUNCH_CHECK();
     return SMX_OK;
+}
+
+extern "C" int smx_epoch_fwdbwd_f32(const smx_epoch_job_t* jobs, int32_t njobs, const smx_ppo_losses_t* loss,
+                                    smx_ppo_ctrl_t* ctrl, int64_t n_total, int32_t* sync_word, uint64_t* kl_slots,
+                                    smx_stream_t stream) {
+    return epoch_fwdbwd_launch(jobs, njobs, loss, ctrl, n_total, sync_word, kl_slots, nullptr, 0, stream);
+}
+
+extern "C" int smx_epoch_fwdbwd_pair_f32(const smx_epoch_job_t* jobs, int32_t njobs, const smx_ppo_losses_t* loss,
+                                         smx_ppo_ctrl_t* ctrl, int64_t n_total, int32_t* sync_word, uint64_t* kl_slots,
+                                         void* xchg, int64_t xchg_bytes, smx_stream_t stream) {
+    SMX_REQUIRE(xchg && xchg_bytes > 0, SMX_E_NULL);
+    return epoch_fwdbwd_launch(jobs, njobs, loss, ctrl, n_total, sync_word, kl_slots, xchg, xchg_bytes, stream);
 }
 
 extern "C" int smx_epoch_backward_f32(const smx_epoch_job_t* jobs, int32_t njobs, const smx_ppo_losses_t* loss,
diff --git a/surreal_amd/csrc/smx_ppo_loss.inc.h b/surreal_amd/csrc/smx_ppo_loss.inc.h
--- a/surreal_amd/csrc/smx_ppo_loss.inc.h
+++ b/surreal_amd/csrc/smx_ppo_loss.inc.h
@@ -34,7 +34,8 @@
     float* __restrict__ g_surr_t = nullptr, float* __restrict__ g_kl_t = nullptr, const long ld_t = 0,
     const long in_row0 = 0 ,
     const int ld_adv = 1,
-    unsigned long long* __restrict__ kl_slot = nullptr ) {
+    unsigned long long* __restrict__ kl_slot = nullptr ,
+    const bool publish = true ) {
     const int R = LOSS_ROWS_PER_BLOCK;
     float* e_z2 = sm;
     float* e_zb2 = e_z2 + R * A;
@@ -158,7 +159,7 @@
         const float v3 = smx_wave_sum(one ? Lb : 0.f);
         const float v4 = smx_wave_sum(one ? isw : 0.f);
         const float v5 = smx_wave_sum(one ? klb : 0.f);
-        if (tid == 0) {
+        if (tid == 0 && publish) {
             if (COH && kl_slot)
                 __hip_atomic_store(kl_slot + blk, (unsigned long long)__float_as_uint(v2) | (1ull << 32), __ATOMIC_RELAXED,
                                    __HIP_MEMORY_SCOPE_AGENT);
@@ -195,7 +196,7 @@
             gs += __shfl_xor(gs, off, 64);
             gk += __shfl_xor(gk, off, 64);
         }
-        if (q == 0) {
+        if (q == 0 && publish) {
             partial_store<COH>(P + 8 + a, gs);
             partial_store<COH>(P + 8 + A + a, gk);
         }
diff --git a/surreal_amd/kernels.py b/surreal_amd/kernels.py
--- a/surreal_amd/kernels.py
+++ b/surreal_amd/kernels.py
@@ -257,7 +257,18 @@
         a.v_will_update = int(loss.get('v_will_update', 0))
         return ctypes.byref(a)
 
-    def epoch_forward(self, jobs, loss=None, ctrl=None, n_total=0):
+    def epoch_pair_fits(self, blocks):
+        return bool(self.lib.smx_epoch_pair_fits(int(blocks)))
+
+    def epoch_pair_xchg(self, *nets, device=None):
+        n = self.lib.smx_epoch_pair_xchg_bytes(max(t.H1 for t in nets), max(t.H2 for t in nets))
+        return torch.zeros(n, dtype=torch.uint8, device=device if device is not None else 'cuda')
+
+    def epoch_forward(self, jobs, loss=None, ctrl=None, n_total=0, xchg=None):
+        if xchg is not None:
+            L.call('smx_epoch_forward_pair_f32', self._epoch_jobs(jobs), len(jobs), self._epoch_loss(loss),
+                   L.ptr(ctrl), int(n_total), L.ptr(xchg), xchg.numel(), self._st())
+            return
         L.call('smx_epoch_forward_f32', self._epoch_jobs(jobs), len(jobs), self._epoch_loss(loss),
                L.ptr(ctrl), int(n_total), self._st())
 
@@ -270,7 +281,11 @@
                     self.lib.smx_epoch_fwdbwd_supported(max(n.D for n in nets), max(n.H1 for n in nets),
                                                         max(n.H2 for n in nets), max(n.OUT for n in nets)))
 
-    def epoch_fwdbwd(self, jobs, loss, ctrl, n_total, sync_word, kl_slots):
+    def epoch_fwdbwd(self, jobs, loss, ctrl, n_total, sync_word, kl_slots, xchg=None):
+        if xchg is not None:
+            L.call('smx_epoch_fwdbwd_pair_f32', self._epoch_jobs(jobs), len(jobs), self._epoch_loss(loss),
+                   L.ptr(ctrl), int(n_total), L.ptr(sync_word), L.ptr(kl_slots), L.ptr(xchg), xchg.numel(), self._st())
+            return
         L.call('smx_epoch_fwdbwd_f32', self._epoch_jobs(jobs), len(jobs), self._epoch_loss(loss),
                L.ptr(ctrl), int(n_total), L.ptr(sync_word), L.ptr(kl_slots), self._st())
 
diff --git a/surreal_amd/learner/ppo.py b/surreal_amd/learner/ppo.py
--- a/surreal_amd/learner/ppo.py
+++ b/surreal_amd/learner/ppo.py
@@ -10,6 +10,8 @@
 from surreal_amd.learner.base import Learner, DeferredStats
 from surreal_amd.learner.dist import _SegmentedGraph, _dist_info, setup_peer_exchange
 from surreal_amd.model.ppo_net import DiagGauss, PPOModel
+
+EPOCH_PAIR_SPLIT_DEFAULT = True
 
 
 class LinearWithMinLR(object):
@@ -279,6 +281,11 @@
         ws.fb = (ws.fused and self.world_size == 1 and bool(self.session_config.learner.get('fused_fwdbwd', True)) and
                  bool(self.session_config.learner.get('exclusive_device', True)) and not getattr(self, '_fb_timed_out', False) and
                  ws.n_slots > 0 and K.epoch_fwdbwd_supported(act, cri))
+        ws.xchg = None
+        if (ws.fb and bool(self.session_config.learner.get('epoch_pair_split', EPOCH_PAIR_SPLIT_DEFAULT)) and
+                hasattr(K, 'epoch_pair_xchg')):
+            if K.epoch_pair_fits(K.epoch_blocks(rows)):
+                ws.xchg = K.epoch_pair_xchg(act, cri, device=self.device)
         ws.vblocks = K.epoch_blocks if ws.fused else K.value_loss_blocks
         ws.nblk_v = ws.vblocks(rows)
         ws.merged_tail = ws.fused and self.world_size == 1
@@ -577,7 +584,8 @@
         pre = [dict(net=ref_job['net'], packed=ws.pk_ref, x=ref_job['x'], out=ref_job['out'], act=L.SMX_ACT_TANH)]
         if tail is not None:
             pre.append(dict(net=tail['net'], packed=ws.pk_critic, x=tail['x'], out=tail['out'], act=L.SMX_ACT_NONE))
-        K.epoch_forward(pre, None, ws.ctrl_f, n_total)
+        px = {} if ws.xchg is None else dict(xchg=ws.xchg)
+        K.epoch_forward(pre, None, ws.ctrl_f, n_total, **px)
         gae()
         aj = dict(net=m.actor, packed=ws.pk_actor, x=ws.xn, act=L.SMX_ACT_TANH, loss='policy', stop=ws.stop, h1T=ws.h1aT,
                   h2T=ws.h2aT, dz3T=ws.dz3aT, dz2T=ws.dz2aT, dz1T=ws.dz1aT, xT=ws.xnT, grads=ws.grads_a,
@@ -622,10 +630,10 @@
             loss = loss_args(e)
             bj = ([aj] if pol_u else []) + ([cj] if val else [])
             if ws.fb and (pol_u or not pol_f) and (pol_u or val):
-                K.epoch_fwdbwd(bj, loss, ws.ctrl_f, n_total, ws.sync[e:e + 1], ws.kl_slots[e])
+                K.epoch_fwdbwd(bj, loss, ws.ctrl_f, n_total, ws.sync[e:e + 1], ws.kl_slots[e], **px)
                 K.mlp3_wgrad_multi(bj)
             else:
-                K.epoch_forward(([aj] if pol_f else []) + ([cj] if val else []), loss, ws.ctrl_f, n_total)
+                K.epoch_forward(([aj] if pol_f else []) + ([cj] if val else []), loss, ws.ctrl_f, n_total, **px)
                 if pol_f and not pol_u:
                     K.epoch_backward([aj], loss, ws.ctrl_f, n_total)
                 if pol_u or val:
```

Result: faster. 125.4 million env-steps/s (median of 6 runs) (+2.8%).
